# WHB139426/Grounded-Video-LLM

Measured on AMD Instinct MI355X. Metric: clips/sec + grounding tokens/sec, 96-frame Phi3.5-3.8B @1/2/4/8 MI355X, higher is better.
Workload: dtype bf16; 1 GPU; Phi-3.5-3.8B, 96 frames (12 segs x 8), 336^2 spatial + 224^2 temporal, prompts of 60..140 tokens (ragged), 12 greedy tokens, 8 clips per GPU per step (16 clips in flight per GPU: the vision encode of the next 8 overlaps the ragged prefill + batched greedy decode of the current 8; CLIP tower batched over the 96 key frames of a step); prefill_len_max=3559, distinct_clips_resident=16, parallelism=1 GPU

## Files before the change

### grounded-video-llm_amd/csrc/gvl_attn.hip

```cpp
#include "gvl_internal.h"
#include "gvl_attn_plan.h"
#include <cstdlib>

template <int D> struct KSwz;
template <> struct KSwz<64> {
  static __device__ __forceinline__ int phys(int row, int lc) { return lc ^ ((row >> 1) & 7); }
  static __device__ __forceinline__ int logical(int row, int pc) { return pc ^ ((row >> 1) & 7); }
};
template <> struct KSwz<96> {
  static __device__ __forceinline__ int phys(int row, int lc) { int p = lc + 3 * ((row >> 2) & 3); return p >= 12 ? p - 12 : p; }
  static __device__ __forceinline__ int logical(int row, int pc) { int l = pc - 3 * ((row >> 2) & 3); return l < 0 ? l + 12 : l; }
};
template <> struct KSwz<128> {
  static __device__ __forceinline__ int phys(int row, int lc) { return lc ^ (row & 15); }
  static __device__ __forceinline__ int logical(int row, int pc) { return pc ^ (row & 15); }
};

template <int D> struct VSwz;
template <> struct VSwz<64> { static __device__ __forceinline__ int phys(int row, int c) { return c ^ (((row >> 1) & 1) << 2); } };
template <> struct VSwz<96> { static __device__ __forceinline__ int phys(int, int c) { return c; } };
template <> struct VSwz<128> { static __device__ __forceinline__ int phys(int row, int c) { return c ^ ((row & 3) << 2); } };
typedef __attribute__((ext_vector_type(4))) short s16x4_t;
typedef __attribute__((ext_vector_type(8))) short s16x8_t;
__device__ __forceinline__ bf16x8_t lds_tr8(const char* p0, const char* p1) {
  typedef __attribute__((address_space(3))) s16x4_t* lp;
  const s16x4_t lo = __builtin_amdgcn_ds_read_tr16_b64_v4i16((lp)p0), hi = __builtin_amdgcn_ds_read_tr16_b64_v4i16((lp)p1);
  const s16x8_t v = {lo[0], lo[1], lo[2], lo[3], hi[0], hi[1], hi[2], hi[3]};
  return __builtin_bit_cast(bf16x8_t, v);
}
__device__ __forceinline__ void glds16s(const void* sbase, unsigned voff, unsigned lds_dst) {
  unsigned keep;
  asm volatile("s_mov_b32 %0, m0\n\ts_mov_b32 m0, %3\n\ts_nop 0\n\tglobal_load_lds_dwordx4 %1, %2\n\ts_mov_b32 m0, %0"
               : "=&s"(keep) : "v"(voff), "s"(sbase), "s"(lds_dst) : "memory");
}

__device__ __forceinline__ float vmax3(float a, float b, float c) {
  float r;
  asm("v_max3_f32 %0, %1, %2, %3" : "=v"(r) : "v"(a), "v"(b), "v"(c));
  return r;
}

__device__ __forceinline__ int kperm(int i) {
  const int c = i & 3, hh = (i >> 2) & 1, b = i >> 3;
  return (b >> 1) * 16 + 8 * hh + 4 * (b & 1) + c;
}

template <int D, int NWAVES, int NS, int ONES = 0, int VROW = 0, int VL = 0>
__global__ __launch_bounds__(NWAVES * 64) void attn_fwd_kernel(const AttnArgs a) {
  constexpr int NT = NWAVES * 64;
  constexpr int DK = D / 16;
  constexpr int DB = D / 32;
  constexpr int CPR = D / 8;
  constexpr int KCH = 64 * CPR;
  constexpr int NIK = KCH / NT;
  constexpr int TILE_BYTES = 64 * D * 2;
  constexpr int STAGE_BYTES = 2 * TILE_BYTES;
  static_assert(KCH % NT == 0, "tile/threads mismatch");

  extern __shared__ __attribute__((aligned(16))) char smem[];

  const int tid = threadIdx.x, lane = tid & 63;
  const int wave = __builtin_amdgcn_readfirstlane(tid >> 6);
  const int l31 = lane & 31, h = lane >> 5;
  int S_ = a.S;
  const bf16_t* Qp_ = a.Q; bf16_t* Op_ = a.O; const int* tbl_ = a.block_table;
  int nq = (a.S + NWAVES * 32 - 1) / (NWAVES * 32);
  const int rep = a.H / a.KV;
  if constexpr (VL) { nq = 0; for (int u = 0; u < a.vl_n; ++u) nq += (a.vl_rows[u + 1] - a.vl_rows[u] + NWAVES * 32 - 1) / (NWAVES * 32); }
  const int xcd = blockIdx.x & 7, j = blockIdx.x >> 3;
  const int qb_ = j % nq, t_ = j / nq, member = t_ % rep, grp = (t_ / rep) * 8 + xcd;
  int qb = a.causal ? nq - 1 - qb_ : qb_;
  if (grp >= a.KV * a.B) return;
  const int b = grp / a.KV, head = (grp - b * a.KV) * rep + member;
  if constexpr (VL) {
    int u = 0, nqu = (a.vl_rows[1] - a.vl_rows[0] + NWAVES * 32 - 1) / (NWAVES * 32);
    while (qb >= nqu && u + 1 < a.vl_n) { qb -= nqu; ++u; nqu = (a.vl_rows[u + 1] - a.vl_rows[u] + NWAVES * 32 - 1) / (NWAVES * 32); }
    const int r0 = a.vl_rows[u];
    S_ = a.vl_rows[u + 1] - r0;
    Qp_ = a.Q + (size_t)r0 * a.H * D;
    Op_ = a.O + (size_t)r0 * (size_t)(a.H * a.Dout);
    tbl_ = a.vl_tables[u];
  }
  const int hkv = head / (a.H / a.KV);
  const int q0 = qb * (NWAVES * 32);
  const int qw = q0 + wave * 32;
  const int Sk = a.Sk > 0 ? a.Sk : S_, qpos0 = a.qpos0;
  const int n_tiles_all = (Sk + 63) >> 6;
  int last_q = q0 + NWAVES * 32 - 1; if (last_q > S_ - 1) last_q = S_ - 1;
  const int n_tiles = a.causal ? ((qpos0 + last_q) >> 6) + 1 : n_tiles_all;

  unsigned koff[NIK], voff[NIK];
#pragma unroll
  for (int i = 0; i < NIK; ++i) {
    const int pos = i * NT + tid;
    const int kr = pos / CPR, kpc = pos - kr * CPR;
    koff[i] = VROW == 2 ? (unsigned)(kr * a.k_ld + KSwz<D>::logical(kr, kpc) * 8) * 2 : (unsigned)(kr * D + KSwz<D>::logical(kr, kpc) * 8) * 2;
    if constexpr (VROW) {
      const int vr = pos / CPR, lc = VSwz<D>::phys(vr, pos - vr * CPR);
      voff[i] = lc * 8 < a.Dout ? (unsigned)(vr * a.v_ld + lc * 8) * 2 : 0xffffffffu;
    } else {
      const int vr = pos >> 3, vpc = pos & 7;
      voff[i] = (unsigned)(vr * 64 + (vpc ^ ((vr >> 1) & 7)) * 8) * 2;
    }
  }
  const float sc = a.scale * 1.4426950408889634f;
  constexpr bool FOLD = VROW == 3;
  u32x4_t qf[DK];
  u32x4_t qraw[DK], qw_[VROW == 3 ? DK : 1];
  float q_rs = 1.f;
  {
    int qi = qw + l31; if (qi > S_ - 1) qi = S_ - 1;
    if constexpr (VROW == 3) {
      const bf16_t* qp = a.Qrows + ((size_t)b * S_ + qi) * a.q_ld + head * a.Dout + 8 * h;
      const bf16_t* wp = a.q_nw + head * a.Dout + 8 * h;
      q_rs = a.q_rs[(size_t)b * S_ + qi];
#pragma unroll
      for (int kk = 0; kk < DK; ++kk) {
        const bool real = kk * 16 + 8 * h < a.Dout;
        qraw[kk] = real ? *(const u32x4_t*)(qp + kk * 16) : u32x4_t{0u, 0u, 0u, 0u};
        qw_[kk] = real ? *(const u32x4_t*)(wp + kk * 16) : u32x4_t{0u, 0u, 0u, 0u};
      }
    } else {
      const bf16_t* qp = VROW == 2 ? a.Qrows + ((size_t)b * S_ + qi) * a.q_ld + head * D + 8 * h : Qp_ + (((size_t)b * a.H + head) * S_ + qi) * D + 8 * h;
#pragma unroll
      for (int kk = 0; kk < DK; ++kk) qraw[kk] = *(const u32x4_t*)(qp + kk * 16);
    }
  }

  int* pages_s = (int*)(smem + NS * STAGE_BYTES);
  for (int i = tid; i < n_tiles; i += NT) pages_s[i] = tbl_ ? tbl_[b * a.max_pages + i] : b * n_tiles_all + i;
  if constexpr (VROW) {
    const int npc = CPR - (a.Dout >> 3);
    for (int i = tid; i < NS * 64 * npc; i += NT) {
      const int slot = i / (64 * npc), r = (i / npc) & 63, lc = (a.Dout >> 3) + i % npc;
      u32x4_t v = {0u, 0u, 0u, 0u};
      if (ONES && lc * 8 == a.Dout) v[0] = 0x3F80u;
      *(u32x4_t*)(smem + slot * STAGE_BYTES + TILE_BYTES + (r * CPR + VSwz<D>::phys(r, lc)) * 16) = v;
    }
  }
  __syncthreads();
  const unsigned smem_base = __builtin_amdgcn_readfirstlane(lds_addr(smem));
  auto stage = [&](int buf, int t) {
    const int pg = __builtin_amdgcn_readfirstlane(pages_s[t]);
    const size_t pb = ((size_t)pg * a.KV + hkv) * (size_t)(64 * D);
    const bf16_t* kp = a.Kt + pb;
    const bf16_t* vp = a.Vt + pb;
    const unsigned base = smem_base + buf * STAGE_BYTES + wave * 1024;
    if constexpr (VROW) {
      const int rows_left = S_ - t * 64;
      if constexpr (VROW == 2) {
        const bf16_t* kr_ = a.Krows + ((size_t)b * S_ + (size_t)t * 64) * a.k_ld + hkv * D;
        if (rows_left >= 64) {
          if constexpr (NIK == 2 || NIK == 3) glds16xn<NIK>(kr_, koff, base, NT * 16);
          else {
#pragma unroll
            for (int i = 0; i < NIK; ++i) glds16s(kr_, koff[i], base + i * NT * 16);
          }
        } else {
#pragma unroll
          for (int i = 0; i < NIK; ++i) {
            const int r = (i * NT + tid) / CPR;
            glds16s(kr_, r >= rows_left ? koff[i] - (unsigned)((r - rows_left + 1) * a.k_ld * 2) : koff[i], base + i * NT * 16);
          }
        }
      } else {
        glds16xn<NIK>(kp, koff, base, NT * 16);
      }
      const bf16_t* vr_ = a.Vrows + ((size_t)b * S_ + (size_t)t * 64) * a.v_ld + hkv * a.Dout;
      if (rows_left >= 64) {
#pragma unroll
        for (int i = 0; i < NIK; ++i)
          if (voff[i] != 0xffffffffu) glds16s(vr_, voff[i], base + TILE_BYTES + i * NT * 16);
      } else {
#pragma unroll
        for (int i = 0; i < NIK; ++i) {
          const int r = (i * NT + tid) / CPR;
          const unsigned off = r >= rows_left ? voff[i] - (unsigned)((r - rows_left + 1) * a.v_ld * 2) : voff[i];
          if (voff[i] != 0xffffffffu) glds16s(vr_, off, base + TILE_BYTES + i * NT * 16);
        }
      }
    } else if constexpr (NIK == 2 || NIK == 3) {
      glds16xn<NIK>(kp, koff, base, NT * 16);
      glds16xn<NIK>(vp, voff, base + TILE_BYTES, NT * 16);
    } else {
#pragma unroll
      for (int i = 0; i < NIK; ++i) glds16((const char*)kp + koff[i], base + i * NT * 16);
#pragma unroll
      for (int i = 0; i < NIK; ++i) glds16((const char*)vp + voff[i], base + TILE_BYTES + i * NT * 16);
    }
  };

  f32x16_t o[DB];
#pragma unroll
  for (int i = 0; i < DB; ++i)
#pragma unroll
    for (int e = 0; e < 16; ++e) o[i][e] = 0.f;
  float m_run = -1e30f, l_run = 0.f;

  const int krow0 = kperm(l31);
  const int vswz = (l31 >> 1) & 7;
  const int my_q = qw + l31;
  unsigned vtr[DB];
  if constexpr (VROW) {
    const int i16 = lane & 15, g4 = (lane >> 4) & 1, r0 = 8 * h + (i16 >> 2);
#pragma unroll
    for (int db = 0; db < DB; ++db) vtr[db] = (unsigned)(r0 * (D * 2) + VSwz<D>::phys(r0, db * 4 + 2 * g4 + ((i16 & 3) >> 1)) * 16 + (i16 & 1) * 8);
  }

  stage(0, 0);
  if (NS == 3 && n_tiles > 1) stage(1, 1);
#pragma unroll
  for (int kk = 0; kk < DK; ++kk) {
    if constexpr (VROW == 3) {
      u32x4_t o;
#pragma unroll
      for (int e = 0; e < 4; ++e) o[e] = pack2bf(lo_bf(qw_[kk][e]) * rbf(lo_bf(qraw[kk][e]) * q_rs) * sc, hi_bf(qw_[kk][e]) * rbf(hi_bf(qraw[kk][e]) * q_rs) * sc);
      qf[kk] = o;
    } else {
      qf[kk] = qraw[kk];
    }
  }
#pragma unroll
  for (int kk = 0; kk < DK; ++kk) asm volatile("" ::"v"(qf[kk]));
  int cur = 0;
  int first_tile = 1;
  if constexpr (FOLD) m_run = 0.f;
  for (int t = 0; t < n_tiles; ++t) {
    if (NS == 3 && t + 1 < n_tiles) asm volatile("s_waitcnt vmcnt(%0)" ::"n"(2 * NIK) : "memory");
    else asm volatile("s_waitcnt vmcnt(0)" ::: "memory");
    __builtin_amdgcn_s_barrier();
    asm volatile("" ::: "memory");
#ifdef GVL_ATTN_LAB
    if (!(GVL_ATTN_LAB & 1))
#endif
    if (t + NS - 1 < n_tiles) { int nb = cur + NS - 1; if (nb >= NS) nb -= NS; stage(nb, t + NS - 1); }
    const int tb = cur;
    cur = cur + 1 == NS ? 0 : cur + 1;
    if (a.causal && t * 64 > qpos0 + qw + 31) continue;
    const char* kb_ = smem + tb * STAGE_BYTES;
    const char* vb_ = kb_ + TILE_BYTES;

    f32x16_t s[2];
#pragma unroll
    for (int kb = 0; kb < 2; ++kb)
#pragma unroll
      for (int e = 0; e < 16; ++e) s[kb][e] = 0.f;
#ifdef GVL_ATTN_LAB
    if (GVL_ATTN_LAB & 4) { s[0][0] = (float)t; s[1][3] = qf[0][0]; } else
#endif
#ifdef GVL_ATTN_PRIO
    if (GVL_ATTN_PRIO & 1) __builtin_amdgcn_s_setprio(1);
#endif
#pragma unroll
    for (int kk = 0; kk < DK; ++kk) {
#pragma unroll
      for (int kb = 0; kb < 2; ++kb) {
        const int row = kb * 32 + krow0;
        const bf16x8_t kf = *(const bf16x8_t*)(kb_ + row * (D * 2) + (KSwz<D>::phys(row, kk * 2 + h) << 4));
        s[kb] = __builtin_amdgcn_mfma_f32_32x32x16_bf16(kf, __builtin_bit_cast(bf16x8_t, qf[kk]), s[kb], 0, 0, 0);
      }
    }
#ifdef GVL_ATTN_PRIO
    if (GVL_ATTN_PRIO & 1) __builtin_amdgcn_s_setprio(0);
#endif
    const bool need_mask = (t == n_tiles_all - 1 && (Sk & 63)) || (a.causal && t * 64 + 63 > qpos0 + qw);
    if (need_mask) {
#pragma unroll
      for (int kb = 0; kb < 2; ++kb)
#pragma unroll
        for (int r = 0; r < 16; ++r) {
          const int key = t * 64 + kb * 32 + (r >> 3) * 16 + 8 * h + (r & 7);
          const bool dead = key >= Sk || (a.causal && key > qpos0 + my_q);
          s[kb][r] = dead ? -1e30f : s[kb][r];
        }
    }
    float mx;
    {
      asm volatile("s_nop 11" : "+v"(s[0]), "+v"(s[1]));
      float l1[11];
#pragma unroll
      for (int i = 0; i < 5; ++i) { l1[i] = vmax3(s[0][3 * i], s[0][3 * i + 1], s[0][3 * i + 2]); l1[5 + i] = vmax3(s[1][3 * i], s[1][3 * i + 1], s[1][3 * i + 2]); }
      l1[10] = vmax3(s[0][15], s[1][15], l1[0]);
      const float a2 = vmax3(l1[1], l1[2], l1[3]), b2 = vmax3(l1[4], l1[5], l1[6]), c2 = vmax3(l1[7], l1[8], l1[9]);
      mx = vmax3(vmax3(a2, b2, c2), l1[10], l1[10]);
    }
    {
      const auto sw = __builtin_amdgcn_permlane32_swap(__float_as_uint(mx), __float_as_uint(mx), false, false);
      mx = fmaxf(__uint_as_float(sw[0]), __uint_as_float(sw[1]));
    }
    float alpha = 1.f;
    if constexpr (FOLD) {
      if (first_tile || !__all(mx <= a.lazy)) {
        const float m_new = rbf(m_run + (first_tile ? mx : fmaxf(mx, 0.f)));
        const float de = m_new - m_run;
        alpha = first_tile ? 1.f : __builtin_amdgcn_exp2f(-de);
        m_run = m_new;
        first_tile = 0;
#pragma unroll
        for (int i = 0; i < DB; ++i)
#pragma unroll
          for (int e = 0; e < 16; ++e) o[i][e] *= alpha;
#pragma unroll
// ... 421 lines not shown
    if (t + 2 == n_tiles - 1) {
      body(IC<0>{}, IC<0>{}, t, sA, sB);
      body(IC<1>{}, IC<1>{}, t + 1, sB, sA);
    } else if (t + 1 == n_tiles - 1) {
      body(IC<0>{}, IC<1>{}, t, sA, sB);
#pragma unroll
      for (int kb = 0; kb < 2; ++kb) sA[kb] = sB[kb];
    }
    {
      const int tl = n_tiles - 1;
      asm volatile("s_waitcnt vmcnt(0)" ::: "memory");
      __builtin_amdgcn_s_barrier();
      asm volatile("" ::: "memory");
      const int vofs = partial ? VLAST : (tl & 1) * STAGE_BYTES + TILE_BYTES;
      const int nst = (tail_keys + 15) >> 4;
#pragma unroll
      for (int st = 0; st < 4; ++st) {
        if (st < nst) {
          const int kb = st >> 1, r0 = (st & 1) * 8;
          union { bf16x8_t v; unsigned u[4]; } pf;
#pragma unroll
          for (int e = 0; e < 4; ++e) pf.u[e] = pack2bf(__builtin_amdgcn_exp2f(sA[kb][r0 + 2 * e]), __builtin_amdgcn_exp2f(sA[kb][r0 + 2 * e + 1]));
#pragma unroll
          for (int db = 0; db < DB; ++db) o[db] = __builtin_amdgcn_mfma_f32_32x32x16_bf16(vfrag(vofs, st * 3 + db), pf.v, o[db], 0, 0, 0);
        }
      }
    }
  };
  auto row_sum = [&]() -> float {
    const int lr = Dout - 32 * (DB - 1);
    float mine = 0.f;
#pragma unroll
    for (int e = 0; e < 16; ++e) mine = (e == (lr >> 3) * 4 + (lr & 3)) ? o[DB - 1][e] : mine;
    const float other = __shfl_xor(mine, 32, 64);
    return h ? other : mine;
  };
  float l_tot = 0.f;
  bool redo = a.pipe == 2;
  if (!redo) {
    run(IC<0>{});
    l_tot = row_sum();
#ifndef GVL_PIPE_LAB
    redo = __syncthreads_or(!(l_tot > 0.f && l_tot < 1.2676506e30f)) != 0;
#endif
  }
  if (redo) {
#pragma unroll
    for (int i = 0; i < DB; ++i)
#pragma unroll
      for (int e = 0; e < 16; ++e) o[i][e] = 0.f;
    m_run = 0.f;
    qf[DK - 1][0] = h ? 0u : qf[DK - 1][0];
    run(IC<1>{});
    l_tot = row_sum();
  }
  const float inv = 1.f / l_tot;
  {
    const int qs = my_q < q_end ? my_q : q_end - 1;
    char* op = (char*)(a.O + ((size_t)b * S + qs) * (size_t)(a.H * Dout) + head * Dout);
#pragma unroll
    for (int db = 0; db < DB; ++db)
#pragma unroll
      for (int gp = 0; gp < 2; ++gp) {
        const int g0 = 2 * gp;
        unsigned ax = pack2bf(o[db][4 * g0] * inv, o[db][4 * g0 + 1] * inv), ay = pack2bf(o[db][4 * g0 + 2] * inv, o[db][4 * g0 + 3] * inv);
        unsigned bx = pack2bf(o[db][4 * g0 + 4] * inv, o[db][4 * g0 + 5] * inv), by = pack2bf(o[db][4 * g0 + 6] * inv, o[db][4 * g0 + 7] * inv);
        const auto rx = __builtin_amdgcn_permlane32_swap(ax, bx, false, false); ax = rx[0]; bx = rx[1];
        const auto ry = __builtin_amdgcn_permlane32_swap(ay, by, false, false); ay = ry[0]; by = ry[1];
        const int cg = db * 4 + g0 + h;
        if (my_q < q_end && cg * 8 < Dout) {
          const u32x4_t w = {ax, ay, bx, by};
          *(u32x4_t*)(op + cg * 16) = w;
        }
      }
  }
}
template <class Kern>
static int launch_planned(Kern kern, GvlDevOnce& once, const AttnArgs& a, const AttnLaunch& l, hipStream_t st) {
  if (gvl_set_max_lds(once, (const void*)kern, l.lds)) return -3;
  hipLaunchKernelGGL(kern, dim3(l.grid), dim3(l.block), l.lds, st, a);
  return hipGetLastError() == hipSuccess ? 0 : -3;
}
static int launch_attn(const AttnArgs& a, const AttnLaunch& l, hipStream_t st) {
  switch (attn_fwd_key(l.D, l.NWAVES, l.NS, l.ONES, l.VROW, l.VL)) {
#define GVL_CASE(D, NWAVES, NS, ONES, VROW, VL) \
    case attn_fwd_key(D, NWAVES, NS, ONES, VROW, VL): { static GvlDevOnce once; return launch_planned(attn_fwd_kernel<D, NWAVES, NS, ONES, VROW, VL>, once, a, l, st); }
    GVL_ATTN_FWD_LIST(GVL_CASE)
#undef GVL_CASE
    default: return -1;
  }
}
static int launch_attn_iv2_pipe(const AttnArgs& a, const AttnLaunch& l, hipStream_t st) {
  switch (l.NWAVES) {
#define GVL_CASE(NW) \
    case NW: { static GvlDevOnce once; return launch_planned(attn_iv2_pipe_kernel<NW>, once, a, l, st); }
    GVL_ATTN_IV2_PIPE_LIST(GVL_CASE)
#undef GVL_CASE
    default: return -1;
  }
}

double gvl_attn_flops(const AttnArgs& a) {
  const double Sk = a.Sk > 0 ? a.Sk : a.S;
  const double f = 4.0 * (double)a.S * Sk * a.Dout * a.H * a.B;
  return a.causal ? f * (a.qpos0 + 0.5 * a.S) / Sk : f;
}

int gvl_launch_attention(const AttnArgs& a_in, hipStream_t st) {
  static const AttnKnobs knobs = [] {
    AttnKnobs k = GVL_ATTN_KNOBS_DEFAULT;
    if (const char* e = gvl_lab_env("GVL_ATTN_LAZY")) k.lazy = (float)atof(e);
    k.no_ones = gvl_lab_env("GVL_ATTN_NO_ONES") != nullptr;
    return k;
  }();
  AttnArgs a = a_in;
  auto al16 = [](const void* p) { return ((uintptr_t)p & 15) == 0; };
  AttnGeometry g{};
  g.B = a.B; g.H = a.H; g.KV = a.KV; g.S = a.S; g.D = a.D; g.Dout = a.Dout; g.Sk = a.Sk; g.qpos0 = a.qpos0; g.causal = a.causal; g.ones_row = a.ones_row; g.k_ones = a.k_ones;
  g.ring = a.ring; g.pipe = a.pipe; g.pipe_rows = a.pipe_rows; g.v_ld = a.v_ld; g.q_ld = a.q_ld; g.k_ld = a.k_ld; g.max_pages = a.max_pages; g.vl_n = a.vl_n;
  for (int u = 0; u <= GVL_MAX_PREFILL_BATCH; ++u) g.vl_rows[u] = a.vl_rows[u];
  for (int u = 0; u < GVL_MAX_PREFILL_BATCH; ++u) g.vl_tables[u] = a.vl_tables[u] != nullptr;
  g.block_table = a.block_table; g.Vrows = a.Vrows; g.Qrows = a.Qrows; g.Krows = a.Krows; g.q_rs = a.q_rs; g.q_nw = a.q_nw;
  g.O16 = al16(a.O); g.Vrows16 = al16(a.Vrows); g.Qrows16 = al16(a.Qrows); g.Krows16 = al16(a.Krows); g.q_nw16 = al16(a.q_nw);
  AttnLaunch plan[GVL_ATTN_MAX_LAUNCHES];
  const int n = attn_plan(g, knobs, plan);
  if (n < 0) return -1;
  for (int i = 0; i < n; ++i) {
    const AttnLaunch& l = plan[i];
    a.lazy = l.lazy;
    if (l.family == GVL_ATTN_IV2_PIPE) { a.q_begin = l.q_begin; a.q_rows = l.q_rows; }
    const int rc = l.family == GVL_ATTN_IV2_PIPE ? launch_attn_iv2_pipe(a, l, st) : launch_attn(a, l, st);
    if (rc) return rc;
  }
  return 0;
}

template <int D, int G, int PH = 0>
__global__ __launch_bounds__(256, 2) void decode_attn_kernel(const DecodeAttnArgs a) {
  constexpr int CPR = D / 8;
  constexpr int NIT = D / 8;
  constexpr int QP = (64 % CPR == 0) ? 1 : 3;
  static_assert(D == 64 || D == 96 || D == 128, "head dim");
  __shared__ __attribute__((aligned(16))) float part_s[4][64 * (CPR + 1)];
  __shared__ __attribute__((aligned(16))) float p_s[4][64];
  __shared__ float red_s[G][4][D + 2];
  __shared__ int last_s;

  const int tid = threadIdx.x, lane = tid & 63, wave = tid >> 6;
  int split = blockIdx.y, bz = blockIdx.z;
  int hkv = blockIdx.x, head0 = hkv * G;
  if constexpr (PH == 2) { head0 = blockIdx.x; hkv = head0 / (a.H / a.KV); }
  if constexpr (PH == 1) {
    const int Gq = a.H / a.KV, units = a.KV * a.gsplit * a.batch;
    const int unit = ((int)blockIdx.y / Gq) * 8 + (int)blockIdx.x;
    if (unit >= units) return;
    hkv = unit % a.KV; split = (unit / a.KV) % a.gsplit; bz = unit / (a.KV * a.gsplit);
    head0 = hkv * Gq + (int)blockIdx.y % Gq;
  }
  const int* __restrict__ block_table = a.tables[bz];
  const bf16_t* qb = a.q + (size_t)bz * a.q_stride;
  float* part_b = a.part + (size_t)bz * a.H * a.nsplit * (D + 2);
  int* counters_b = a.counters + bz * a.H;
  const int pos = *a.pos_ptrs[bz] + 1;
  const int npages = (pos + 63) >> 6;
  int ns = (npages + 3) >> 2;
  ns = ns > a.nsplit ? a.nsplit : ns;
  const int cpb = a.cpb;
  const int c_begin = split * cpb;
  if (c_begin >= ns) return;
  const int c_end = c_begin + cpb < ns ? c_begin + cpb : ns;
  const int nblk = (ns + cpb - 1) / cpb;
  const int pps = (npages + ns - 1) / ns;

  u32x4_t qv[G][QP];
#pragma unroll
  for (int g = 0; g < G; ++g)
#pragma unroll
    for (int it = 0; it < QP; ++it) qv[g][it] = *(const u32x4_t*)(qb + (head0 + g) * D + ((it * 64 + lane) % CPR) * 8);

  const float sc = a.scale * 1.4426950408889634f;
  for (int chunk = c_begin; chunk < c_end; ++chunk) {
  const int p_begin = chunk * pps;
  int p_end = p_begin + pps; if (p_end > npages) p_end = npages;
  float m_run[G], l_run[G];
  float oacc[G][NIT];
#pragma unroll
  for (int g = 0; g < G; ++g) {
    m_run[g] = -1e30f; l_run[g] = 0.f;
#pragma unroll
    for (int i = 0; i < NIT; ++i) oacc[g][i] = 0.f;
  }

  for (int pg = p_begin + wave; pg < p_end; pg += 4) {
    const size_t pb = ((size_t)block_table[pg] * a.KV + hkv) * (size_t)(64 * D);
    const bf16_t* kp = a.Kt + pb;
    const bf16_t* vp = a.Vt + pb;
    u32x4_t kv[NIT], vv[NIT];
#pragma unroll
    for (int it = 0; it < NIT; ++it) kv[it] = PH == 1 ? *(const u32x4_t*)(kp + (it * 64 + lane) * 8) : __builtin_nontemporal_load((const u32x4_t*)(kp + (it * 64 + lane) * 8));
#pragma unroll
    for (int it = 0; it < NIT; ++it) vv[it] = PH == 1 ? *(const u32x4_t*)(vp + (it * 64 + lane) * 8) : __builtin_nontemporal_load((const u32x4_t*)(vp + (it * 64 + lane) * 8));
#pragma unroll
    for (int g = 0; g < G; ++g) {
#pragma unroll
      for (int it = 0; it < NIT; ++it) {
// ... 381 lines not shown
```

### grounded-video-llm_amd/csrc/gvl_attn_plan.h

```cpp
#pragma once
#include "gvl_limits.h"

enum AttnMode : int {
  GVL_ATTN_PAGED = 0,
  GVL_ATTN_V_ROWS,
  GVL_ATTN_QKV_ROWS,
  GVL_ATTN_QNORM_V_ROWS,
  GVL_ATTN_RAGGED,
};
enum AttnFamily : int { GVL_ATTN_FWD = 0, GVL_ATTN_IV2_PIPE };

#define GVL_ATTN_FWD_LIST(X)                                                                                     \
  X(64, 4, 2, 0, 0, 0) X(64, 4, 2, 0, 1, 0) X(64, 4, 2, 0, 2, 0)                                                 \
  X(96, 4, 2, 0, 0, 0) X(96, 4, 2, 1, 0, 0) X(96, 4, 3, 0, 0, 0) X(96, 4, 2, 0, 1, 0) X(96, 4, 2, 1, 1, 0)       \
  X(96, 4, 2, 0, 3, 0) X(96, 4, 2, 1, 3, 0)                                                                      \
  X(128, 4, 2, 0, 0, 0) X(128, 4, 3, 0, 0, 0)                                                                    \
  X(64, 4, 2, 0, 0, 1) X(96, 4, 2, 0, 0, 1) X(128, 4, 2, 0, 0, 1)
#define GVL_ATTN_IV2_PIPE_LIST(X) X(4) X(8)
constexpr int attn_fwd_key(int D, int NWAVES, int NS, int ONES, int VROW, int VL) { return ((((D * 16 + NWAVES) * 4 + NS) * 2 + ONES) * 4 + VROW) * 2 + VL; }

struct AttnGeometry {
  int B, H, KV, S, D, Dout, Sk, qpos0, causal, ones_row, k_ones, ring, pipe, pipe_rows, v_ld, q_ld, k_ld, max_pages;
  int vl_n, vl_rows[GVL_MAX_PREFILL_BATCH + 1];
  bool block_table, Vrows, Qrows, Krows, q_rs, q_nw, vl_tables[GVL_MAX_PREFILL_BATCH];
  bool O16, Vrows16, Qrows16, Krows16, q_nw16;
};
struct AttnKnobs {
  float lazy;
  bool no_ones;
};
constexpr AttnKnobs GVL_ATTN_KNOBS_DEFAULT = {8.f, false};
struct AttnLaunch {
  int mode;
  int family;
  int D, NWAVES, NS, ONES, VROW, VL;
  unsigned grid; int block, lds;
  int q_begin, q_rows;
  float lazy;
};
constexpr int GVL_ATTN_MAX_LAUNCHES = 2;

inline int attn_mode_of(const AttnGeometry& g) {
  return g.vl_n ? GVL_ATTN_RAGGED : (g.q_rs || g.q_nw) ? GVL_ATTN_QNORM_V_ROWS : (g.Krows || g.Qrows) ? GVL_ATTN_QKV_ROWS : g.Vrows ? GVL_ATTN_V_ROWS : GVL_ATTN_PAGED;
}
inline bool attn_pitch_ok(int ld, long long width, bool ptr16) { return ld >= width && (ld & 7) == 0 && ptr16; }
inline bool attn_tile_below_4g(int ld) { return (unsigned long long)64 * (unsigned long long)ld * 2 < 0xffffffffull; }
inline bool attn_common_ok(const AttnGeometry& g) {
  return g.B > 0 && g.H > 0 && g.KV > 0 && g.S > 0 && g.S <= 256 * 64 && g.Sk <= 256 * 64 && g.H % g.KV == 0 && g.Dout <= g.D && (g.Dout & 7) == 0 && g.O16;
}
inline bool attn_paged_ok(const AttnGeometry& g) {
  return g.Sk >= 0 && g.qpos0 >= 0 && (g.Sk > 0 ? g.Sk >= g.S + g.qpos0 && g.block_table : g.qpos0 == 0);
}
inline bool attn_v_rows_ok(const AttnGeometry& g) {
  return g.Vrows && !g.block_table && g.Sk == 0 && g.qpos0 == 0 && attn_pitch_ok(g.v_ld, (long long)g.KV * g.Dout, g.Vrows16) && attn_tile_below_4g(g.v_ld) && g.D != 128;
}
inline bool attn_qkv_rows_ok(const AttnGeometry& g) {
  return attn_v_rows_ok(g) && g.Qrows && g.Krows && g.D == 64 && g.Dout == g.D && attn_pitch_ok(g.k_ld, (long long)g.KV * g.D, g.Krows16) &&
         attn_pitch_ok(g.q_ld, (long long)g.H * g.D, g.Qrows16) && attn_tile_below_4g(g.k_ld);
}
inline bool attn_qnorm_v_rows_ok(const AttnGeometry& g) {
  return attn_v_rows_ok(g) && g.q_rs && g.q_nw && g.Qrows && !g.Krows && g.D == 96 && g.Dout == 88 && g.k_ones && attn_pitch_ok(g.q_ld, (long long)g.H * g.Dout, g.Qrows16 && g.q_nw16);
}
inline bool attn_ragged_ok(const AttnGeometry& g) {
  if (g.vl_n < 1 || g.vl_n > GVL_MAX_PREFILL_BATCH || g.B != 1 || !g.causal || g.Sk || g.qpos0 || g.Vrows || g.Qrows || g.Krows || g.q_rs || g.q_nw || g.block_table) return false;
  for (int u = 0; u < g.vl_n; ++u)
    if (!g.vl_tables[u] || g.vl_rows[u + 1] <= g.vl_rows[u] || g.vl_rows[u + 1] - g.vl_rows[u] > g.S) return false;
  return true;
}

inline int attn_plan(const AttnGeometry& g, const AttnKnobs& k, AttnLaunch out[GVL_ATTN_MAX_LAUNCHES]) {
  if (g.D != 64 && g.D != 96 && g.D != 128) return -1;
  if (!attn_common_ok(g)) return -1;
  const int mode = attn_mode_of(g);
  switch (mode) {
    case GVL_ATTN_PAGED: if (!attn_paged_ok(g)) return -1; break;
    case GVL_ATTN_V_ROWS: if (!attn_v_rows_ok(g)) return -1; break;
    case GVL_ATTN_QKV_ROWS: if (!attn_qkv_rows_ok(g)) return -1; break;
    case GVL_ATTN_QNORM_V_ROWS: if (!attn_qnorm_v_rows_ok(g)) return -1; break;
    default: if (!attn_ragged_ok(g)) return -1; break;
  }
  const float lazy = k.lazy >= 0.f && k.lazy <= 64.f ? k.lazy : GVL_ATTN_KNOBS_DEFAULT.lazy;
  const long long groups8 = (((long long)g.KV * g.B + 7) / 8) * 8;
  const int vrow = mode == GVL_ATTN_RAGGED ? 0 : mode, vl = mode == GVL_ATTN_RAGGED;
  const int lr = g.Dout - 64;
  const bool ones = g.D == 96 && !vl && g.ones_row && !k.no_ones && g.Dout < 96 && lr >= 0 && (lr & 7) < 4 && !g.causal;

  if (mode == GVL_ATTN_QNORM_V_ROWS && ones && g.pipe && g.H == g.KV) {
    const int lds = 2 * 2 * 64 * 96 * 2 + 64 * 96 * 2;
    const int rows8 = g.pipe_rows == 256 ? (g.S / 256) * 256 : 0;
    int n = 0;
    for (int nw = 8; nw >= 4; nw -= 4) {
      const int q_begin = nw == 8 ? 0 : rows8, q_rows = nw == 8 ? rows8 : g.S - rows8;
      if (q_rows <= 0) continue;
      const long long grid = groups8 * ((q_rows + 32 * nw - 1) / (32 * nw));
      if (grid > 0x7fffffffll) return -1;
      out[n++] = AttnLaunch{mode, GVL_ATTN_IV2_PIPE, 96, nw, 2, 1, 3, 0, (unsigned)grid, 64 * nw, lds, q_begin, q_rows, lazy};
    }
    return n;
  }
  const int ns = g.ring == 3 && mode == GVL_ATTN_PAGED && g.D != 64 && !ones ? 3 : 2;
  const int nwaves = 4, rows = 32 * nwaves;
  long long nq = (g.S + rows - 1) / rows;
  if (vl) { nq = 0; for (int u = 0; u < g.vl_n; ++u) nq += (g.vl_rows[u + 1] - g.vl_rows[u] + rows - 1) / rows; }
  const long long grid = groups8 * (g.H / g.KV) * nq;
  if (grid > 0x7fffffffll) return -1;
  out[0] = AttnLaunch{mode, GVL_ATTN_FWD, g.D, nwaves, ns, ones, vrow, vl, (unsigned)grid, 64 * nwaves, ns * 2 * 64 * g.D * 2 + 1024 ,
                      0, g.S, lazy};
  return 1;
}

enum DecodeAttnFamily : int { GVL_DECODE_ATTN_GQA = 0, GVL_DECODE_ATTN_HEAD };
#define GVL_DECODE_ATTN_GQA_LIST(X) \
  X(64, 4, 1) X(64, 16, 1) X(64, 4, 0) X(64, 16, 0) X(96, 4, 1) X(96, 16, 1) X(96, 4, 0) X(96, 16, 0) X(128, 4, 1) X(128, 16, 1) X(128, 4, 0) X(128, 16, 0)
#define GVL_DECODE_ATTN_HEAD_LIST(X) X(64, 0) X(64, 1) X(64, 2) X(96, 0) X(96, 1) X(96, 2) X(128, 0) X(128, 1) X(128, 2)
constexpr int decode_attn_key(int D, int a, int b) { return (D * 32 + a) * 4 + b; }

struct DecodeAttnGeometry { int H, KV, D, nsplit, batch, hpb, cpb, gsplit; };
struct DecodeAttnKnobs {
  bool no_gqa;
  bool gqa_valu;
  bool gqa_direct;
};
constexpr DecodeAttnKnobs GVL_DECODE_ATTN_KNOBS_DEFAULT = {false, false, false};
struct DecodeAttnLaunch {
  int batch, cpb, gsplit, hpb;
  int family;
  int D, t1, t2;
  unsigned grid_x, grid_y, grid_z;
};

inline int decode_attn_plan(const DecodeAttnGeometry& g, const DecodeAttnKnobs& k, DecodeAttnLaunch* out) {
  DecodeAttnLaunch l{};
  l.batch = g.batch <= 0 ? 1 : g.batch;
  if (l.batch > GVL_MAX_DECODE_BATCH) return -1;
  if (g.H <= 0 || g.KV <= 0 || g.H % g.KV) return -1;
  l.cpb = g.cpb < 1 ? 1 : g.cpb;
  if (g.nsplit < 1 || g.nsplit > 16) return -1;
  l.gsplit = g.gsplit <= 0 || g.gsplit > g.nsplit ? (g.nsplit + l.cpb - 1) / l.cpb : g.gsplit;
  if (g.D != 64 && g.D != 96 && g.D != 128) return -1;
  l.D = g.D; l.hpb = g.hpb;
  const int G = g.H / g.KV;
  long long gx, gy = 1, gz = 1;
  if (G > 1 && G <= 16 && !k.no_gqa && !k.gqa_valu) {
    if (l.hpb < 1 || l.hpb > G || G % l.hpb) l.hpb = G;
    l.family = GVL_DECODE_ATTN_GQA;
    l.t1 = l.hpb <= 4 ? 4 : 16;
    l.t2 = !(k.gqa_direct || (g.D & (g.D - 1)) != 0);
    gx = (long long)(g.H / l.hpb) * l.gsplit * l.batch;
  } else {
    l.family = GVL_DECODE_ATTN_HEAD;
    l.t1 = G == 1 ? 0 : k.no_gqa ? 2 : 1;
    if (l.t1 == 1) { gx = 8; gy = ((long long)g.KV * l.gsplit * l.batch + 7) / 8 * G; }
    else { gx = g.H; gy = l.gsplit; gz = l.batch; }
  }
  if (gx * gy * gz > 0x7fffffffll) return -1;
  l.grid_x = (unsigned)gx; l.grid_y = (unsigned)gy; l.grid_z = (unsigned)gz;
  *out = l;
  return 0;
}

struct DecodeAttnShape { int gsplit, cpb, hpb; };
inline DecodeAttnShape decode_attn_shape(const int* positions, int B, int H, int KV, int nsplit, int force_cpb, int force_hpb, bool capturing) {
  DecodeAttnShape s{nsplit, 1, 0};
  if (capturing) return s;
  if (force_cpb >= 1 && force_cpb <= 16) s.cpb = force_cpb;
  long splits = 0;
  s.gsplit = 1;
  for (int b = 0; b < B; ++b) {
    const int np = (positions[b] + 1 + 63) >> 6, n = (np + 3) >> 2;
    const int ns = n < 1 ? 1 : (n > nsplit ? nsplit : n), blocks = (ns + s.cpb - 1) / s.cpb;
    s.gsplit = blocks > s.gsplit ? blocks : s.gsplit;
    splits += blocks;
  }
  const int G = H / KV;
  if (G > 1) {
    s.hpb = G;
    while (s.hpb > 2 && s.hpb % 2 == 0 && (long)(H / s.hpb) * splits < 400) s.hpb >>= 1;
    if (s.hpb == 2 && (long)(H / 2) * splits < 200) s.hpb = 1;
    if (force_hpb >= 1 && G % force_hpb == 0) s.hpb = force_hpb;
  }
  return s;
}
```

### grounded-video-llm_amd/csrc/gvl_ctx.h

```cpp
#pragma once
#include "gvl_internal.h"
#include "gvl_seq_table.h"
#include "../../include/gvl.h"
#include <dlfcn.h>
#include <fcntl.h>
#include <sys/mman.h>
#include <sys/stat.h>
#include <unistd.h>
#include <algorithm>
#include <cmath>
#include <cstdio>
#include <cstring>
#include <memory>
#include <string>
#include <unordered_map>
#include <vector>

std::string& gvl_create_error();


struct Tensor { void* p = nullptr; int dtype = 0; int64_t numel = 0; std::vector<int64_t> shape; };

struct ClipLayerW { const float *ln1w, *ln1b, *ln2w, *ln2b, *qkvb, *outb, *fc1b, *fc2b; const bf16_t *qkvw, *outw, *fc1w, *fc2w; };
struct Iv2BlockW { const bf16_t *n1, *n2, *qkvw, *qn, *kn, *projw, *fc1w, *fc2w; const float *projb, *ls1, *ls2, *fc1b, *fc2b;
                   const bf16_t *qkvw_f = nullptr, *fc1w_f = nullptr; };
struct LlmLayerW { const bf16_t *ln1, *ln2, *qkvw, *ow, *guw, *downw;
                   const bf16_t *qkvw_f = nullptr, *guw_f = nullptr;
                   const bf16_t *qkvd_f = nullptr, *gud_f = nullptr;
                   const bf16_t *qkvd, *od, *gud, *downd;
                   const float *qkvs, *os, *gus, *downs; };

struct Seq : SeqCore {
  int* d_block_table = nullptr; int* d_pos = nullptr;
  bool table_dirty = false;
  int* d_tok = nullptr;
  int* d_out = nullptr;
  const int* h_out = nullptr;
  int* d_ngen = nullptr;
  unsigned rng_stream = 0;
  int* d_eos = nullptr; volatile int* h_eos = nullptr;
  float* d_lp = nullptr; int* d_top_ids = nullptr; float* d_top_lp = nullptr;
};

struct ProfRec { int cat; hipEvent_t e0, e1; double work; };

struct gvl_ctx : SeqTable<Seq> {
  static constexpr int kMaxSeqs = 256;
  static constexpr int kMaxRuleSets = 1024;
  gvl_ctx() : SeqTable<Seq>(kMaxSeqs, kMaxRuleSets) {}
  gvl_config cfg;
  std::string err;
  std::unordered_map<std::string, Tensor> w;
  bool finalized = false;
  int c_P = 0, c_S = 0, c_Kp = 0, c_Dr = 0, c_D = 0;
  int v_L = 0, v_TL = 0, v_S = 0, v_Kp = 0, v_Dr = 0, v_D = 0;
  int l_Dr = 0, l_D = 0, tok_per_seg = 0, img_tok = 0, seg_tok = 0;
  bool has_clip = false, has_iv2 = false, has_llm = false, has_proj = false;
  const bf16_t* c_patchw = nullptr; const float *c_cls = nullptr, *c_pos = nullptr, *c_prelnw = nullptr, *c_prelnb = nullptr;
  std::vector<ClipLayerW> cl;
  const bf16_t *v_patchw = nullptr, *v_cls = nullptr, *v_pos = nullptr; const float* v_patchb = nullptr;
  std::vector<Iv2BlockW> vb;
  const bf16_t *mm0w = nullptr, *mm1w = nullptr, *vp0w = nullptr, *vp1w = nullptr, *glb_gn = nullptr, *newline = nullptr;
  const float *mm0b = nullptr, *mm1b = nullptr, *vp0b = nullptr, *vp1b = nullptr, *sub_gn = nullptr;
  const bf16_t *l_embed = nullptr, *l_norm = nullptr, *l_headw = nullptr; const float* l_headb = nullptr;
  const float *cos_s = nullptr, *sin_s = nullptr, *cos_l = nullptr, *sin_l = nullptr;
  std::vector<LlmLayerW> ll;
  char* arena = nullptr; size_t arena_bytes = 0, arena_off = 0;
  char* arena_l = nullptr; size_t arena_l_bytes = 0, arena_l_off = 0;
  bf16_t *kpool = nullptr, *vpool = nullptr; size_t layer_stride = 0;
  int* d_seq_tables = nullptr; int* d_seq_pos = nullptr; int seq_table_cap = 0;
  bf16_t *d_x = nullptr, *d_qkv = nullptr, *d_q = nullptr, *d_attn = nullptr, *d_act = nullptr;
  bf16_t* d_xn = nullptr;
  int* d_seq_ngen = nullptr;
  bool decode_mfma = false;
  const bf16_t* l_headd = nullptr;
  const bf16_t* l_headd_f = nullptr;
  bf16_t* d_xt = nullptr;
  float* d_sqpart = nullptr;
  const float* l_heads = nullptr;
  int fp8 = 0;
  std::vector<void*> dw_allocs;
  std::vector<void*> pw_allocs;
  std::vector<void*> nf_allocs;
  const bf16_t *c_patchwt = nullptr, *v_patchwt = nullptr;
  float *d_logits = nullptr, *d_part = nullptr; int* d_counters = nullptr; int *d_seq_tok = nullptr, *d_seq_out = nullptr;
  int* h_seq_out = nullptr;
  int nsplit = 16, outlist_cap = 8192, ids_cap = 16384;
  void* pre_scratch = nullptr; size_t pre_scratch_bytes = 0;
  int kv_total_pages = 0;
  int* h_eos_flags = nullptr; int* d_eos_flags = nullptr; int watch_eos = -1;
  hipEvent_t step_ev[3] = {nullptr, nullptr, nullptr};
  struct { bool on = false; float inv_temp = 1.f, top_p = 0.f; int top_k = 0; unsigned long long seed = 0; unsigned next_stream = 0;
           float min_p = 0.f, typical_p = 0.f, eps = 0.f, eta = 0.f;
           bool warps() const { return on && (min_p > 0.f || (typical_p > 0.f && typical_p < 1.f) || eps > 0.f || eta > 0.f); } } sample;
  float* d_seq_lp = nullptr; int* d_seq_top_ids = nullptr; float* d_seq_top_lp = nullptr;
  struct { int decode_attn_cpb = 0, decode_attn_hpb = 0; bool decode_graph = true; int vision_in_place = 1, prefill_group = 4, attn_ring = 0, attn_pipe = 1, attn_pipe_rows = 128, patch_fused = 1, varlen_attn = 1, norm_fused = 1, last_layer_tail = 1; } dbg;
  void* comm = nullptr; int comm_rank = 0, comm_world = 1;
  bool prof = false; std::vector<ProfRec> recs;
  double prof_ms[GVL_PROF_NCAT] = {0}, prof_work[GVL_PROF_NCAT] = {0}; int64_t prof_n[GVL_PROF_NCAT] = {0};
};

inline int gvl_fail(gvl_ctx* c, int code, const std::string& msg) {
  if (c) c->err = msg; else gvl_create_error() = msg;
  return code;
}
inline int gvl_hipfail(gvl_ctx* c, hipError_t e, const char* what) { return gvl_fail(c, GVL_ERR_HIP, std::string(what) + ": " + hipGetErrorString(e)); }
#define HIPCHK(c, expr) do { hipError_t _e = (expr); if (_e != hipSuccess) return gvl_hipfail(c, _e, #expr); } while (0)
```

### grounded-video-llm_amd/csrc/gvl_elem.hip

```cpp
#include "gvl_internal.h"
#include <cstring>

#define CHECK_LAUNCH() (hipGetLastError() == hipSuccess ? 0 : -3)

template <int MAXV>
__global__ __launch_bounds__(256) void layernorm_f32_kernel(const float* __restrict__ x, const float* __restrict__ w,
                                                            const float* __restrict__ b, bf16_t* __restrict__ y, int rows, int cols, float eps) {
  const int row = blockIdx.x * 4 + (threadIdx.x >> 6), lane = threadIdx.x & 63;
  if (row >= rows) return;
  const float* xr = x + (size_t)row * cols;
  f32x4_t v[MAXV];
  float s = 0.f;
#pragma unroll
  for (int i = 0; i < MAXV; ++i) {
    const int c = (lane + 64 * i) * 4;
    if (c < cols) { v[i] = *(const f32x4_t*)(xr + c); s += v[i][0] + v[i][1] + v[i][2] + v[i][3]; }
  }
  const float mean = wave_sum(s) / cols;
  float q = 0.f;
#pragma unroll
  for (int i = 0; i < MAXV; ++i) {
    const int c = (lane + 64 * i) * 4;
    if (c < cols) {
#pragma unroll
// ... 315 lines not shown
  auto norm_chunk = [&](const u32x4_t& v, int c, float rs, const bf16_t* nw) -> u32x4_t {
    const u32x4_t w = *(const u32x4_t*)(nw + c * 8);
    u32x4_t o;
#pragma unroll
    for (int e = 0; e < 4; ++e) o[e] = pack2bf(lo_bf(w[e]) * rbf(lo_bf(v[e]) * rs), hi_bf(w[e]) * rbf(hi_bf(v[e]) * rs));
    return o;
  };
  bf16_t* Qb = a.Q + ((size_t)b * a.H * S_ + s_in) * a.D + (size_t)row0 * a.H * a.D;
  bf16_t* Kb = a.Kt + ((size_t)page * a.KV) * (64 * a.D) + (size_t)slot * a.D;
  if (in_regs) {
#pragma unroll
    for (int i = 0; i < RC; ++i) {
      const int c = lane + 64 * i;
      if (c < nq && !a.q_rs) { const int hd = c / cpr, dc = c - hd * cpr; *(u32x4_t*)(Qb + (size_t)hd * S_ * a.D + dc * 8) = norm_chunk(qreg[i], c, q_rs, a.qn); }
      if (c < nk) { const int hd = c / cpr, dc = c - hd * cpr; *(u32x4_t*)(Kb + (size_t)hd * (64 * a.D) + dc * 8) = norm_chunk(kreg[i], c, k_rs, a.kn); }
    }
  } else {
    if (!a.q_rs) for (int c = lt; c < nq; c += TEAM) {
      const int hd = c / cpr, dc = c - hd * cpr;
      *(u32x4_t*)(Qb + (size_t)hd * S_ * a.D + dc * 8) = xform(qr, c, q_rs, a.qn);
    }
    for (int c = lt; c < nk; c += TEAM) {
      const int hd = c / cpr, dc = c - hd * cpr;
      *(u32x4_t*)(Kb + (size_t)hd * (64 * a.D) + dc * 8) = xform(kr, c, k_rs, a.kn);
    }
  }
  if (cpd > cpr) {
    const int np = cpd - cpr;
    if (!a.q_rs) for (int c = lt; c < a.H * np; c += TEAM) { const int hd = c / np; *(u32x4_t*)(Qb + (size_t)hd * S_ * a.D + (cpr + c % np) * 8) = zero; }
    for (int c = lt; c < a.KV * np; c += TEAM) {
      const int hd = c / np;
      u32x4_t v = zero; if (a.k_ones && c % np == 0) v[0] = 0x3F80u;
      *(u32x4_t*)(Kb + (size_t)hd * (64 * a.D) + (cpr + c % np) * 8) = v;
    }
  }
  if (a.pos_ptr) {
    bf16_t* Vbase = a.Vt + ((size_t)page * a.KV) * (64 * a.D) + slot;
    for (int i = lt; i < a.KV * a.Dr; i += TEAM) {
      const int hd = i / a.Dr, d = i - hd * a.Dr;
      Vbase[(size_t)hd * (64 * a.D) + d * 64] = vr[i];
    }
  }
}

__global__ __launch_bounds__(256) void v_transpose_kernel(const QkvPostArgs a) {
  __shared__ __attribute__((aligned(16))) bf16_t tile[64][136];
  int t = blockIdx.x, S_ = a.S, row0 = 0;
  const int hkv = blockIdx.y, b = blockIdx.z;
  const int* table = a.block_table;
  if (a.vl_n) {
    int u = 0, t0 = 0;
    for (; u + 1 < a.vl_n; ++u) { const int nt = (a.vl_rows[u + 1] - a.vl_rows[u] + 63) >> 6; if (t < t0 + nt) break; t0 += nt; }
    t -= t0; row0 = a.vl_rows[u]; S_ = a.vl_rows[u + 1] - row0; table = a.vl_tables[u];
  }
  const int tid = threadIdx.x;
  const int s0 = a.pos0 + t * 64;
  const int n_tiles = (S_ + 63) >> 6;
  const int tile_idx = s0 >> 6;
  const int page = table ? table[b * a.max_pages + tile_idx] : b * n_tiles + tile_idx;
  const int voff = (a.H + a.KV) * a.Dr + hkv * a.Dr;
  const int cpr = a.Dr >> 3;
  for (int i = tid; i < 64 * cpr; i += 256) {
    const int r = i / cpr, c = i - r * cpr;
    const int s_in = t * 64 + r;
    u32x4_t v = {0u, 0u, 0u, 0u};
    if (s_in < S_) v = *(const u32x4_t*)(a.qkv + ((size_t)b * S_ + row0 + s_in) * a.ld + voff + c * 8);
    *(u32x4_t*)&tile[r][c * 8] = v;
  }
  __syncthreads();
  bf16_t* dst = a.Vt + ((size_t)page * a.KV + hkv) * (64 * a.D);
  for (int i = tid; i < a.D * 8; i += 256) {
    const int d = i >> 3, k8 = (i & 7) * 8;
    u32x4_t o = {0u, 0u, 0u, 0u};
    if (d < a.Dr) {
#pragma unroll
      for (int e = 0; e < 4; ++e) o[e] = (unsigned)tile[k8 + 2 * e][d] | ((unsigned)tile[k8 + 2 * e + 1][d] << 16);
    } else if (a.ones_row && d == a.Dr) {
      o = u32x4_t{0x3F803F80u, 0x3F803F80u, 0x3F803F80u, 0x3F803F80u};
    }
    *(u32x4_t*)(dst + d * 64 + k8) = o;
  }
}

int gvl_launch_qkv_post(const QkvPostArgs& a, hipStream_t st) {
  if ((a.Dr & 7) || (a.mode == 2 && (a.Dr & 15)) || (a.D & 7) || a.D < a.Dr || a.Dr > 128 || (a.ld & 7)) return -1;
  if (a.vl_n && (a.mode != 2 || a.B != 1 || a.pos0 != 0 || a.pos_ptr || a.vl_n > GVL_MAX_PREFILL_BATCH)) return -1;
  const int rows = a.vl_n ? a.vl_rows[a.vl_n] : a.B * a.S;
  if (a.q_rs && (a.mode != 1 || a.pos_ptr)) return -1;
  if (a.pos_ptr) {
    if (rows != 1 || a.mode != 2) return -1;
    hipLaunchKernelGGL(qkv_post_kernel<4>, dim3(1), dim3(256), 0, st, a);
  } else {
    hipLaunchKernelGGL(qkv_post_kernel<1>, dim3((rows + 3) / 4), dim3(256), 0, st, a);
  }
  if (!a.pos_ptr && a.Vt) {
    int n_tiles = (a.S + 63) >> 6;
    if (a.vl_n) { n_tiles = 0; for (int u = 0; u < a.vl_n; ++u) n_tiles += (a.vl_rows[u + 1] - a.vl_rows[u] + 63) >> 6; }
    hipLaunchKernelGGL(v_transpose_kernel, dim3(n_tiles, a.KV, a.B), dim3(256), 0, st, a);
  }
  return CHECK_LAUNCH();
}

__global__ __launch_bounds__(256) void hd_merge_kernel(const float* __restrict__ f, const float* __restrict__ sub_gn, bf16_t* __restrict__ out, int n, int C) {
  const int c4 = 4 * C, cv = c4 / 4;
  const long total = (long)n * 156 * cv;
  for (long idx = (long)blockIdx.x * blockDim.x + threadIdx.x; idx < total; idx += (long)gridDim.x * blockDim.x) {
    const int c = (int)(idx % cv) * 4;
    const long row = idx / cv;
    const int r = (int)(row % 156), img = (int)(row / 156);
    const int hh = r / 13, ww = r - hh * 13;
    f32x4_t v;
    if (ww == 12) v = *(const f32x4_t*)(sub_gn + c);
    else {
      const int chunk = c / C, cc = c - chunk * C, dy = chunk >> 1, dx = chunk & 1;
      v = *(const f32x4_t*)(f + ((size_t)img * 576 + (2 * hh + dy) * 24 + 2 * ww + dx) * C + cc);
    }
    u32x2_t o = {pack2bf(v[0], v[1]), pack2bf(v[2], v[3])};
    *(u32x2_t*)(out + row * c4 + c) = o;
  }
}
int gvl_launch_hd_merge(const float* f, const float* sub_gn, bf16_t* out, int n, int C, hipStream_t st) {
  if (C % 4) return -1;
  const long total = (long)n * 156 * C;
  int blocks = (int)((total + 255) / 256); if (blocks > 8192) blocks = 8192;
  hipLaunchKernelGGL(hd_merge_kernel, dim3(blocks), dim3(256), 0, st, f, sub_gn, out, n, C);
  return CHECK_LAUNCH();
}

__global__ __launch_bounds__(256) void pool_spatial_kernel(const float* __restrict__ f, bf16_t* __restrict__ out, int n, int C) {
  const int cv = C / 4;
  const long total = (long)n * 64 * cv;
  for (long idx = (long)blockIdx.x * blockDim.x + threadIdx.x; idx < total; idx += (long)gridDim.x * blockDim.x) {
    const int c = (int)(idx % cv) * 4;
    const long row = idx / cv;
    const int r = (int)(row % 64), img = (int)(row / 64);
    const int ph = r >> 3, pw = r & 7;
    f32x4_t acc = {0.f, 0.f, 0.f, 0.f};
    for (int dy = 0; dy < 3; ++dy)
      for (int dx = 0; dx < 3; ++dx) acc += *(const f32x4_t*)(f + ((size_t)img * 576 + (3 * ph + dy) * 24 + 3 * pw + dx) * C + c);
    u32x2_t o = {pack2bf(acc[0] / 9.f, acc[1] / 9.f), pack2bf(acc[2] / 9.f, acc[3] / 9.f)};
    *(u32x2_t*)(out + row * C + c) = o;
  }
}
int gvl_launch_pool_spatial(const float* f, bf16_t* out, int n, int C, hipStream_t st) {
  if (C % 4) return -1;
  const long total = (long)n * 64 * (C / 4);
  int blocks = (int)((total + 255) / 256); if (blocks > 8192) blocks = 8192;
  hipLaunchKernelGGL(pool_spatial_kernel, dim3(blocks), dim3(256), 0, st, f, out, n, C);
  return CHECK_LAUNCH();
}

__global__ __launch_bounds__(256) void pool_temporal_kernel(const bf16_t* __restrict__ f, bf16_t* __restrict__ out, int n, int T, int C) {
  const int cv = C / 8;
  const long total = (long)n * T * 16 * cv;
  for (long idx = (long)blockIdx.x * blockDim.x + threadIdx.x; idx < total; idx += (long)gridDim.x * blockDim.x) {
    const int c = (int)(idx % cv) * 8;
    const long row = idx / cv;
    const int r = (int)(row % 16), t = (int)((row / 16) % T), seg = (int)(row / (16L * T));
    const int ph = r >> 2, pw = r & 3;
    float acc[8] = {0, 0, 0, 0, 0, 0, 0, 0};
    for (int dy = 0; dy < 4; ++dy)
      for (int dx = 0; dx < 4; ++dx) {
        const u32x4_t v = *(const u32x4_t*)(f + ((size_t)seg * T * 256 + t * 256 + (4 * ph + dy) * 16 + 4 * pw + dx) * C + c);
#pragma unroll
        for (int e = 0; e < 4; ++e) { acc[2 * e] += lo_bf(v[e]); acc[2 * e + 1] += hi_bf(v[e]); }
      }
    u32x4_t o;
#pragma unroll
    for (int e = 0; e < 4; ++e) o[e] = pack2bf(acc[2 * e] * 0.0625f, acc[2 * e + 1] * 0.0625f);
    *(u32x4_t*)(out + row * C + c) = o;
  }
}
int gvl_launch_pool_temporal(const bf16_t* f, bf16_t* out, int n, int T, int C, hipStream_t st) {
  if (C % 8) return -1;
  const long total = (long)n * T * 16 * (C / 8);
  int blocks = (int)((total + 255) / 256); if (blocks > 8192) blocks = 8192;
  hipLaunchKernelGGL(pool_temporal_kernel, dim3(blocks), dim3(256), 0, st, f, out, n, T, C);
  return CHECK_LAUNCH();
}

__global__ void f32_to_bf16_kernel(const float* __restrict__ x, bf16_t* __restrict__ y, long n) {
  for (long i = (long)blockIdx.x * blockDim.x + threadIdx.x; i < n; i += (long)gridDim.x * blockDim.x) y[i] = f2bf(x[i]);
// ... 786 lines not shown
```

### grounded-video-llm_amd/csrc/gvl_internal.h

```cpp
#pragma once
#include <hip/hip_runtime.h>
#include <stdint.h>

typedef uint16_t bf16_t;

#include <cstdlib>
#ifdef GVL_LAB
inline const char* gvl_lab_env(const char* name) { return getenv(name); }
#else
inline const char* gvl_lab_env(const char*) { return nullptr; }
#endif

typedef __attribute__((ext_vector_type(8))) __bf16 bf16x8_t;
typedef __attribute__((ext_vector_type(16))) float f32x16_t;
typedef __attribute__((ext_vector_type(4))) float f32x4_t;
typedef __attribute__((ext_vector_type(4))) unsigned int u32x4_t;
typedef __attribute__((ext_vector_type(2))) unsigned int u32x2_t;

#define GVL_KV_PAGE 64
#include "gvl_limits.h"
constexpr int GVL_MAX_VALU_BATCH = 4;
constexpr int GVL_GEMM_ROT_LEN = 64;

#include <atomic>
// ... 58 lines not shown
  static_assert(N == 2 || N == 3, "2 or 3 pieces");
  unsigned keep, d;
  if constexpr (N == 3) {
    asm volatile(
        "s_mov_b32 %0, m0\n\t"
        "s_mov_b32 m0, %6\n\ts_nop 0\n\tglobal_load_lds_dwordx4 %2, %5\n\t"
        "s_add_u32 %1, %6, %7\n\ts_mov_b32 m0, %1\n\ts_nop 0\n\tglobal_load_lds_dwordx4 %3, %5\n\t"
        "s_add_u32 %1, %1, %7\n\ts_mov_b32 m0, %1\n\ts_nop 0\n\tglobal_load_lds_dwordx4 %4, %5\n\t"
        "s_mov_b32 m0, %0"
        : "=&s"(keep), "=&s"(d)
        : "v"(v[0]), "v"(v[1]), "v"(v[N - 1]), "s"(sbase), "s"(lds_dst0), "s"(lds_step)
        : "memory", "scc");
  } else {
    asm volatile(
        "s_mov_b32 %0, m0\n\t"
        "s_mov_b32 m0, %5\n\ts_nop 0\n\tglobal_load_lds_dwordx4 %2, %4\n\t"
        "s_add_u32 %1, %5, %6\n\ts_mov_b32 m0, %1\n\ts_nop 0\n\tglobal_load_lds_dwordx4 %3, %4\n\t"
        "s_mov_b32 m0, %0"
        : "=&s"(keep), "=&s"(d)
        : "v"(v[0]), "v"(v[1]), "s"(sbase), "s"(lds_dst0), "s"(lds_step)
        : "memory", "scc");
  }
}
__device__ __forceinline__ unsigned lds_addr(const void* p) {
  return (unsigned)(unsigned long)(__attribute__((address_space(3))) const void*)p;
}

enum { GVL_ACT_NONE = 0, GVL_ACT_QUICK_GELU = 1, GVL_ACT_GELU = 2, GVL_ACT_SILU_MUL = 3 };

struct GemmArgs {
  const bf16_t* A;  int lda;
  const bf16_t* W;  int ldw;
  void* C;          int ldc;
  int M, N, K;
  const float* bias;
  const float* gamma;
  const void* resid; int ldr;
  int act;
  int out_f32;
  int round_pre_resid;
  int grp_rows, grp_stride, row_off;
  int tile_cfg;
  int band;
  unsigned char rot[64];
  int narrow;
  int m_begin;
  const float* rowscale;
  float* rowsq; int rowsq_ld;
  const float* act_table;
  unsigned long long* dbg;
};
constexpr int GVL_GEMM_BAND = 4;
int gvl_launch_gemm(const GemmArgs& a, hipStream_t st);
int gvl_device_cus();
int gvl_launch_gemm_a4(const GemmArgs& a, int epi, int var, hipStream_t st);
int gvl_launch_gemm_a4p(const GemmArgs& a, int epi, hipStream_t st);
void gvl_gemm_set_a4(int v);
void gvl_gemm_set_narrow(int v);
void gvl_gemm_set_band(int v);
double gvl_gemm_flops(const GemmArgs& a);
template <class Launch, class Report>
inline int gvl_gemm_probe_launch(GemmArgs a, size_t n, hipStream_t st, Launch&& launch, Report&& report) {
  if (hipMalloc((void**)&a.dbg, n * 8) != hipSuccess) return -3;
  hipMemsetAsync(a.dbg, 0, n * 8, st);
  launch(a);
  std::vector<unsigned long long> hbuf(n);
  hipStreamSynchronize(st);
  hipMemcpy(hbuf.data(), a.dbg, n * 8, hipMemcpyDeviceToHost);
  hipFree(a.dbg);
  report(hbuf);
  return hipGetLastError() == hipSuccess ? 0 : -3;
}

struct AttnArgs {
  const bf16_t* Q;
  const bf16_t* Kt;
  const bf16_t* Vt;
  const bf16_t* Vrows;
  int v_ld;
  const bf16_t* Qrows; const bf16_t* Krows;
  int q_ld, k_ld;
  int k_ones;
  const float* q_rs; const bf16_t* q_nw;
  bf16_t* O;
  const int* block_table;
  int max_pages;
  int B, H, KV, S, D, Dout;
  int Sk, qpos0;
  float scale;
  int causal;
  int ones_row;
  int ring;
  int pipe;
  int pipe_rows;
  int q_begin, q_rows;
  float lazy;
  int vl_n;
  int vl_rows[GVL_MAX_PREFILL_BATCH + 1];
  const int* vl_tables[GVL_MAX_PREFILL_BATCH];
};
int gvl_launch_attention(const AttnArgs& a, hipStream_t st);
double gvl_attn_flops(const AttnArgs& a);

struct DecodeAttnArgs {
  const bf16_t* q;
  const bf16_t* Kt; const bf16_t* Vt;
  const int* tables[GVL_MAX_DECODE_BATCH];
  const int* pos_ptrs[GVL_MAX_DECODE_BATCH];
  float* part;
  int* counters;
  bf16_t* out;
  int H, KV, D, Dout, nsplit, batch, q_stride, out_stride, out_tiled;
  float scale;
  int hpb;
  int cpb;
  int gsplit;
};
int gvl_launch_decode_attention(const DecodeAttnArgs& a, hipStream_t st);

int gvl_launch_layernorm_f32(const float* x, const float* w, const float* b, bf16_t* y, int rows, int cols, float eps, hipStream_t st);
int gvl_launch_rmsnorm_bf16(const bf16_t* x, const bf16_t* w, bf16_t* y, int rows, int cols, float eps, hipStream_t st);
int gvl_launch_copy_bytes(const void* src, void* dst, size_t bytes, hipStream_t st);
int gvl_launch_fold_gamma(const bf16_t* W, const bf16_t* gamma, bf16_t* Wo, long rows, int cols, hipStream_t st);
int gvl_launch_rowsq_finish(const float* sq, int ld, int b0, int nblk, float* rs, int rows, int cols, float eps, hipStream_t st);
int gvl_launch_patchify(const float* px, bf16_t* A, int n_img, int T, int image, int patch, int Kp, hipStream_t st);
int gvl_launch_clip_embed_ln(const bf16_t* patch, const float* cls, const float* pos, const float* lnw, const float* lnb,
                             float* x, int n_img, int P, int C, float eps, hipStream_t st);
int gvl_launch_iv2_embed(const bf16_t* patch, const bf16_t* cls, const bf16_t* pos, bf16_t* x, int B, int TL, int C, hipStream_t st);
struct PatchEmbedArgs {
  const float* px;
  const bf16_t* Wt;
  int n_img, T, image, patch, C;
  int M;
  int S;
  int mode;
  const float* bias;
  const float *cls_f32, *pos_f32, *lnw, *lnb; float eps; float* x_f32;
  const bf16_t *cls_bf, *pos_bf; bf16_t* x_bf;
};
int gvl_retile_patch_weight(const bf16_t* W, bf16_t* Wt, int C, int Kp, int p, hipStream_t st);
int gvl_launch_patch_embed(const PatchEmbedArgs& a, hipStream_t st);
struct QkvPostArgs {
  const bf16_t* qkv; int ld;
  bf16_t* Q; bf16_t* Kt; bf16_t* Vt;
  const int* block_table; int max_pages;
  int B, S, H, KV, Dr, D;
  int mode;
  const bf16_t* qn; const bf16_t* kn; float eps;
  const float* cos; const float* sin; int pos0;
  const int* pos_ptr;
  const float* cos_l; const float* sin_l; int rope_switch;
  int ones_row;
  int k_ones;
  float* q_rs;
  int vl_n;
  int vl_rows[GVL_MAX_PREFILL_BATCH + 1];
  const int* vl_tables[GVL_MAX_PREFILL_BATCH];
};
int gvl_launch_qkv_post(const QkvPostArgs& a, hipStream_t st);
int gvl_launch_hd_merge(const float* f, const float* sub_gn, bf16_t* out, int n, int C, hipStream_t st);
int gvl_launch_pool_spatial(const float* f, bf16_t* out, int n, int C, hipStream_t st);
int gvl_launch_pool_temporal(const bf16_t* f, bf16_t* out, int n, int T, int C, hipStream_t st);
int gvl_launch_f32_to_bf16(const float* x, bf16_t* y, int64_t n, hipStream_t st);
int gvl_launch_bcast_row(const bf16_t* row, bf16_t* dst, int n, int stride_rows, int row_off, int cols, hipStream_t st);
int gvl_launch_gather_rows(const bf16_t* table, const int* ids, bf16_t* dst, int n, int cols, hipStream_t st);
int gvl_launch_strip_cls(const void* x, void* y, int n, int S, int C, int elem_bytes, hipStream_t st);
struct GemvArgs {
  const bf16_t* W; int N, K;
  const bf16_t* x;
  const bf16_t* norm_w; float eps;
  const float* bias;
  const bf16_t* resid;
  int act;
  bf16_t* out_bf16;
  float* out_f32;
  int batch, x_stride, out_stride;
  int rope_on; const float *cos_s, *sin_s, *cos_l, *sin_l; int rope_switch;
  const int* pos_ptrs[GVL_MAX_DECODE_BATCH]; const int* tables[GVL_MAX_DECODE_BATCH];
  bf16_t *Q, *Kt, *Vt; int H, KV, Dr, D; int q_stride;
  int variant;
  int w_fp8; const float* wscale;
  int out_tiled;
  const float* sq_in; int sq_n;
  float* sq_out; bf16_t* out_tiled2;
};
__host__ __device__ __forceinline__ size_t gvl_xt_index(int j, int k) { return ((size_t)(k >> 5) * 64 + (size_t)(((k >> 3) & 3) * 16 + j)) * 8 + (k & 7); }
int gvl_retile_decode_weight(const bf16_t* W, bf16_t* Wt, int N, int K, int Dr, int n_qk_heads, hipStream_t st);
int gvl_fp8_quantise_decode_weight(bf16_t* W, unsigned char* Wt8, float* scale, int N, int K, int Dr, int n_qk_heads, hipStream_t st);
int gvl_mxfp4_quantise_decode_weight(bf16_t* W, unsigned char* Wt4, unsigned* scale, int N, int K, int Dr, int n_qk_heads, hipStream_t st);
int gvl_launch_rows_to_tiled(const bf16_t* x, bf16_t* xt, int batch, int cols, int stride, hipStream_t st);
int gvl_launch_gemv(const GemvArgs& a, hipStream_t st);
int gvl_launch_dgemm(const GemvArgs& a, hipStream_t st);
struct IntList { int v[256]; int n; };
int gvl_launch_gather_rows_host_ids(const bf16_t* table, const int* host_ids, int n, bf16_t* dst, int cols, hipStream_t st);
int gvl_launch_ce_rows(const bf16_t* logits, int ld, const int* targets, float* nll, int n, int V, hipStream_t st);
struct ArgmaxArgs { const float* logits; int n, batch; int* tok_ptrs[GVL_MAX_DECODE_BATCH]; int* out_lists[GVL_MAX_DECODE_BATCH];
                    int* ngen_ptrs[GVL_MAX_DECODE_BATCH]; int* pos_ptrs[GVL_MAX_DECODE_BATCH];
                    int eos_id; int* eos_flags[GVL_MAX_DECODE_BATCH];
                    float inv_temp, top_p; int top_k; unsigned seed_lo, seed_hi; unsigned stream[GVL_MAX_DECODE_BATCH];
                    const int* step_override;
                    int top_n[GVL_MAX_DECODE_BATCH]; float* lp_lists[GVL_MAX_DECODE_BATCH]; int* top_ids[GVL_MAX_DECODE_BATCH]; float* top_lp[GVL_MAX_DECODE_BATCH]; };
constexpr int GVL_MAX_TOP_LOGPROBS = 8;
int gvl_launch_argmax(const ArgmaxArgs& a, hipStream_t st);
int gvl_launch_sample(const ArgmaxArgs& a, hipStream_t st);
struct SelRow { int on; float inv_temp; int top_k; float top_p, min_p, typical_p, eps, eta; unsigned seed_lo, seed_hi, stream; };
struct SelRowsArgs { ArgmaxArgs am; SelRow row[GVL_MAX_DECODE_BATCH]; unsigned char* kept; };
int gvl_launch_select_rows(const SelRowsArgs& a, hipStream_t st);
constexpr int GVL_LOGITS_HIST_CAP = 8192;
constexpr int GVL_RULES_MAX_IDS = 1 << 18;
constexpr int GVL_RULES_MAX_SEQS = 1024;
constexpr int GVL_RULES_MAX_SEQ_LEN = 16;
struct TokenRulesDev { int n_suppress, off_suppress, n_begin, off_begin, begin_at, n_force, off_force, force_at, n_multi;
                       int n_tgt[2], off_tgt[2], off_ent[2], off_pre[2]; };
struct LogitsProcArgs { float* logits; int n, ld, batch, cap; const int* hist[GVL_MAX_DECODE_BATCH]; const int* len_ptrs[GVL_MAX_DECODE_BATCH];
                        float penalty[GVL_MAX_DECODE_BATCH]; int ngram[GVL_MAX_DECODE_BATCH], min_new[GVL_MAX_DECODE_BATCH], eos[GVL_MAX_DECODE_BATCH];
                        const TokenRulesDev* rules[GVL_MAX_DECODE_BATCH]; };
int gvl_launch_logits_process(const LogitsProcArgs& a, hipStream_t st);
struct TokPtrs { const int* p[GVL_MAX_DECODE_BATCH]; int n; };
int gvl_launch_gather_tok_rows(const bf16_t* table, const TokPtrs& toks, bf16_t* dst, int cols, hipStream_t st);
int gvl_launch_embed_norm(const bf16_t* table, const TokPtrs& toks, bf16_t* x, bf16_t* xn, const bf16_t* w, int cols, float eps, hipStream_t st);
int gvl_launch_norm_tiled(bf16_t* x, bf16_t* xn, const bf16_t* w, int batch, int cols, float eps, hipStream_t st);
struct IntPtrs { int* p[GVL_MAX_DECODE_BATCH]; int n; };
int gvl_launch_inc_many(const IntPtrs& ptrs, hipStream_t st);
int gvl_launch_inc(int* p, hipStream_t st);
int gvl_launch_kv_page_copy(bf16_t* kpool, bf16_t* vpool, size_t layer_stride, size_t page_elems, int layers, int src_page, int dst_page, hipStream_t st);
int gvl_launch_set_int(int* p, int v, hipStream_t st);

int gvl_launch_preprocess(const unsigned char* frames, int n, int H, int W, int layout, int size, const float* mean, const float* stdv, float* out,
                          void** scratch, size_t* scratch_bytes, hipStream_t st);
```

### grounded-video-llm_amd/csrc/gvl_llm.hip

```cpp
#include "gvl_model.h"
#include "gvl_attn_plan.h"

namespace gvlm {

size_t prefill_bytes(const gvl_ctx* c, int S) {
  const gvl_config& f = c->cfg;
  const size_t qkvw = (size_t)(f.heads + 2 * f.kv_heads) * c->l_Dr;
  size_t b = 0;
  b += 2 * al256((size_t)S * f.hidden * 2) + al256((size_t)S * qkvw * 2) + al256((size_t)S * f.heads * c->l_Dr * 2);
  b += al256((size_t)S * f.inter * 2) + al256((size_t)f.heads * S * c->l_D * 2);
  b += al256((size_t)kLossChunk * f.vocab * 2) + al256((size_t)kLossChunk * f.hidden * 2) + 3 * al256((size_t)S * 4);
  b += al256((size_t)S * ((f.hidden + 63) / 64) * 4) + al256((size_t)S * 4);
  b += (size_t)GVL_MAX_PREFILL_BATCH * (al256((size_t)f.hidden * 2) * 2 + al256((size_t)f.inter * 2) + al256(((f.hidden + 63) / 64) * 4) + 256) + 1024;
  return b + 4096;
}

__global__ void fill_ints_kernel(int* dst, const IntList l) { for (int i = threadIdx.x; i < l.n; i += blockDim.x) dst[i] = l.v[i]; }

int upload_table(gvl_ctx* ctx, Seq& s, hipStream_t st) {
  if (!s.table_dirty) return 0;
  const int np = (int)s.pages.size();
  for (int p0 = 0; p0 < np; p0 += 256) {
    IntList l; l.n = np - p0 < 256 ? np - p0 : 256;
    for (int i = 0; i < l.n; ++i) l.v[i] = s.pages[p0 + i];
// ... 13 lines not shown
    lp.cap = ctx->outlist_cap < GVL_LOGITS_HIST_CAP ? ctx->outlist_cap : GVL_LOGITS_HIST_CAP;
    for (int b = 0; b < am.batch; ++b) {
      const LogitsProc& q = sqs[b]->sel.proc;
      lp.hist[b] = sqs[b]->d_out; lp.len_ptrs[b] = sqs[b]->d_ngen;
      lp.penalty[b] = q.penalty; lp.ngram[b] = q.ngram; lp.min_new[b] = q.eos >= 0 ? q.min_new : 0; lp.eos[b] = q.eos;
      lp.rules[b] = sqs[b]->sel.rules >= 0 ? (const TokenRulesDev*)ctx->rule_sets[sqs[b]->sel.rules].d : nullptr;
    }
    const int rc = gvl_launch_logits_process(lp, st);
    if (rc) return rc;
  }
  for (int b = 0; b < am.batch; ++b) {
    const Seq& q = *sqs[b];
    if (q.sel.top_n < 0 || !q.d_lp) continue;
    am.top_n[b] = q.sel.top_n; am.lp_lists[b] = q.d_lp;
    if (q.sel.top_n > 0) { am.top_ids[b] = q.d_top_ids; am.top_lp[b] = q.d_top_lp; }
  }
  bool per_row = ctx->sample.warps();
  for (int b = 0; b < am.batch; ++b) per_row = per_row || sqs[b]->sel.own_sampling;
  if (per_row) {
    SelRowsArgs sa; memset(&sa, 0, sizeof(sa)); sa.am = am;
    for (int b = 0; b < am.batch; ++b) {
      SelRow& r = sa.row[b];
      if (sqs[b]->sel.own_sampling) {
        const Sampling& q = sqs[b]->sel.sampling;
        r.on = q.on; r.inv_temp = q.inv_temp; r.top_k = q.top_k; r.top_p = q.top_p; r.min_p = q.min_p; r.typical_p = q.typical_p; r.eps = q.eps; r.eta = q.eta;
        r.seed_lo = (unsigned)q.seed; r.seed_hi = (unsigned)(q.seed >> 32); r.stream = q.stream;
      } else {
        const auto& q = ctx->sample;
        r.on = q.on; r.inv_temp = q.inv_temp; r.top_k = q.top_k; r.top_p = q.top_p; r.min_p = q.min_p; r.typical_p = q.typical_p; r.eps = q.eps; r.eta = q.eta;
        r.seed_lo = (unsigned)q.seed; r.seed_hi = (unsigned)(q.seed >> 32); r.stream = sqs[b]->rng_stream;
      }
    }
    return gvl_launch_select_rows(sa, st);
  }
  if (!ctx->sample.on) return gvl_launch_argmax(am, st);
  am.inv_temp = ctx->sample.inv_temp; am.top_p = ctx->sample.top_p; am.top_k = ctx->sample.top_k;
  am.seed_lo = (unsigned)ctx->sample.seed; am.seed_hi = (unsigned)(ctx->sample.seed >> 32);
  for (int b = 0; b < am.batch; ++b) am.stream[b] = sqs[b]->rng_stream;
  return gvl_launch_sample(am, st);
}

int llm_prefill(gvl_ctx* ctx, Seq* const* sqs, int nb, const bf16_t* const* embeds, const int* lens, hipStream_t st, const LossReq* loss, int pos0) {
  const gvl_config& f = ctx->cfg;
  const int Hd = f.hidden, H = f.heads, KV = f.kv_heads, Dr = ctx->l_Dr, D = ctx->l_D, I = f.inter;
  const int qkvw = (H + 2 * KV) * Dr;
  if (nb < 1 || nb > GVL_MAX_PREFILL_BATCH) return fail(ctx, GVL_ERR_ARG, "llm_prefill: batch must be 1 .. 8 sequences");
  if (pos0 != 0 && (nb != 1 || (pos0 & 63) || loss)) return fail(ctx, GVL_ERR_ARG, "llm_prefill: extend takes one sequence whose cached prefix is whole pages");
  for (int b = 0; b < nb; ++b) { const int rc = upload_table(ctx, *sqs[b], st); if (rc) return rc; }
  int off[GVL_MAX_PREFILL_BATCH + 1]; off[0] = 0;
  bool uniform = true;
  for (int b = 0; b < nb; ++b) { off[b + 1] = off[b] + lens[b]; uniform = uniform && lens[b] == lens[0]; }
  const int M = off[nb], S0 = lens[0], P0 = (S0 + 63) / 64;
  if (nb > 1 && uniform && nb * P0 > (int)(sizeof(IntList::v) / sizeof(int))) uniform = false;
  ArenaScope arena_scope(ctx->arena_l_off);
  LALLOC(x, bf16_t, (size_t)M * Hd); LALLOC(h, bf16_t, (size_t)M * Hd); LALLOC(qkv, bf16_t, (size_t)M * qkvw);
  LALLOC(att, bf16_t, (size_t)M * H * Dr); LALLOC(act, bf16_t, (size_t)M * I); LALLOC(Q, bf16_t, (size_t)M * H * D);
  const int* table = sqs[0]->d_block_table;
  int table_stride = sqs[0]->n_pages;
  if (nb > 1 && uniform) {
    LALLOC(tb, int, (size_t)nb * P0);
    IntList l; l.n = nb * P0;
    for (int b = 0; b < nb; ++b) for (int p = 0; p < P0; ++p) l.v[b * P0 + p] = sqs[b]->pages[p];
    hipLaunchKernelGGL(fill_ints_kernel, dim3(1), dim3(256), 0, st, tb, l);
    table = tb; table_stride = P0;
  }
  for (int b = 0; b < nb; ++b) RUN(GVL_PROF_OTHER, 0, gvl_launch_copy_bytes(embeds[b], x + (size_t)off[b] * Hd, (size_t)lens[b] * Hd * 2, st));
  const int NBLK = Hd / 64;
  const bool nf = ctx->dbg.norm_fused && Hd % 64 == 0 && ((f.heads + 2 * f.kv_heads) * ctx->l_Dr) % 16 == 0 && (2 * f.inter) % 16 == 0 && !ctx->ll.empty() && ctx->ll[0].qkvw_f;
  LALLOC(sq, float, (size_t)M * (nf ? NBLK : 1)); LALLOC(nrs, float, (size_t)M);
  const bf16_t* tail_rows = nullptr;
  const int n_att = (nb == 1 || uniform) ? 1 : nb;
  for (int l = 0; l < f.layers; ++l) {
    const LlmLayerW& w = ctx->ll[l];
    bf16_t* Kt = ctx->kpool + (size_t)l * ctx->layer_stride; bf16_t* Vt = ctx->vpool + (size_t)l * ctx->layer_stride;
    if (nf && l > 0) {
      RUN(GVL_PROF_OTHER, 0, gvl_launch_rowsq_finish(sq, NBLK, 0, NBLK, nrs, M, Hd, f.rms_eps, st));
      GemmArgs g = gemm(x, Hd, w.qkvw_f, qkv, qkvw, M, qkvw, Hd); g.rowscale = nrs; RUN(GVL_PROF_GEMM, gvl_gemm_flops(g), gvl_launch_gemm(g, st));
    } else {
      RUN(GVL_PROF_OTHER, 0, gvl_launch_rmsnorm_bf16(x, w.ln1, h, M, Hd, f.rms_eps, st));
      GemmArgs g = gemm(h, Hd, w.qkvw, qkv, qkvw, M, qkvw, Hd); RUN(GVL_PROF_GEMM, gvl_gemm_flops(g), gvl_launch_gemm(g, st));
    }
    const bool vl_attn = n_att > 1 && ctx->dbg.varlen_attn && pos0 == 0;
    bool vl_post = vl_attn && ctx->dbg.varlen_attn == 1;
    if (vl_post && f.rope_orig_max_pos > 0 && ctx->cos_l) {
      const bool l0 = lens[0] > f.rope_orig_max_pos;
      for (int u = 1; u < nb; ++u) vl_post = vl_post && (lens[u] > f.rope_orig_max_pos) == l0;
    }
    if (vl_post) {
      const bool use_long = f.rope_orig_max_pos > 0 && lens[0] > f.rope_orig_max_pos && ctx->cos_l;
      QkvPostArgs q; memset(&q, 0, sizeof(q)); q.qkv = qkv; q.ld = qkvw; q.Q = Q; q.Kt = Kt; q.Vt = Vt; q.B = 1; q.H = H; q.KV = KV; q.Dr = Dr; q.D = D; q.mode = 2;
      q.cos = use_long ? ctx->cos_l : ctx->cos_s; q.sin = use_long ? ctx->sin_l : ctx->sin_s; q.vl_n = nb;
      for (int u = 0; u < nb; ++u) { q.vl_rows[u] = off[u]; q.vl_tables[u] = sqs[u]->d_block_table; q.S = lens[u] > q.S ? lens[u] : q.S; }
      q.vl_rows[nb] = off[nb];
      RUN(GVL_PROF_OTHER, 0, gvl_launch_qkv_post(q, st));
    }
    for (int u = 0; u < n_att && !vl_post; ++u) {
      const int S = lens[u], B = n_att == 1 ? nb : 1;
      const int* tbl = n_att == 1 ? table : sqs[u]->d_block_table;
      const int tstride = n_att == 1 ? table_stride : sqs[u]->n_pages;
      const bool use_long = f.rope_orig_max_pos > 0 && pos0 + S > f.rope_orig_max_pos && ctx->cos_l;
      bf16_t* Qu = Q + (size_t)off[u] * H * D;
      { QkvPostArgs q; memset(&q, 0, sizeof(q)); q.qkv = qkv + (size_t)off[u] * qkvw; q.ld = qkvw; q.Q = Qu; q.Kt = Kt; q.Vt = Vt; q.block_table = tbl; q.max_pages = tstride;
        q.B = B; q.S = S; q.H = H; q.KV = KV; q.Dr = Dr; q.D = D; q.mode = 2; q.cos = use_long ? ctx->cos_l : ctx->cos_s; q.sin = use_long ? ctx->sin_l : ctx->sin_s; q.pos0 = pos0;
        RUN(GVL_PROF_OTHER, 0, gvl_launch_qkv_post(q, st)); }
      if (vl_attn) continue;
      { AttnArgs a; memset(&a, 0, sizeof(a)); a.Q = Qu; a.Kt = Kt; a.Vt = Vt; a.O = att + (size_t)off[u] * H * Dr; a.block_table = tbl; a.max_pages = tstride;
        a.B = B; a.H = H; a.KV = KV; a.S = S; a.D = D; a.Dout = Dr; a.scale = 1.0f / sqrtf((float)Dr); a.causal = 1;
        if (pos0) { a.Sk = pos0 + S; a.qpos0 = pos0; }
        a.ring = ctx->dbg.attn_ring;
        RUN(GVL_PROF_ATTN, gvl_attn_flops(a), gvl_launch_attention(a, st)); }
    }
    if (vl_attn) {
      AttnArgs a; memset(&a, 0, sizeof(a)); a.Q = Q; a.Kt = Kt; a.Vt = Vt; a.O = att; a.B = 1; a.H = H; a.KV = KV; a.D = D; a.Dout = Dr;
      a.scale = 1.0f / sqrtf((float)Dr); a.causal = 1; a.vl_n = nb;
      double fl = 0;
      for (int u = 0; u < nb; ++u) { a.vl_rows[u] = off[u]; a.vl_tables[u] = sqs[u]->d_block_table; a.S = lens[u] > a.S ? lens[u] : a.S;
        AttnArgs one = a; one.S = lens[u]; one.vl_n = 0; fl += gvl_attn_flops(one); }
      a.vl_rows[nb] = off[nb]; a.max_pages = 0;
      RUN(GVL_PROF_ATTN, fl, gvl_launch_attention(a, st));
    }
    { GemmArgs g = gemm(att, H * Dr, w.ow, x, Hd, M, Hd, H * Dr); g.resid = x; g.ldr = Hd; if (nf) { g.rowsq = sq; g.rowsq_ld = NBLK; }
      RUN(GVL_PROF_GEMM, gvl_gemm_flops(g), gvl_launch_gemm(g, st)); }
    if (l == f.layers - 1 && !loss && ctx->dbg.last_layer_tail && (!nf || NBLK % 4 == 0)) {
      int ids[GVL_MAX_PREFILL_BATCH];
      for (int b = 0; b < nb; ++b) ids[b] = off[b + 1] - 1;
      LALLOC(xl, bf16_t, (size_t)nb * Hd); LALLOC(actl, bf16_t, (size_t)nb * I);
      RUN(GVL_PROF_OTHER, 0, gvl_launch_gather_rows_host_ids(x, ids, nb, xl, Hd, st));
      if (nf) {
        LALLOC(sql, float, (size_t)nb * NBLK); LALLOC(rsl, float, nb);
        RUN(GVL_PROF_OTHER, 0, gvl_launch_gather_rows_host_ids((const bf16_t*)sq, ids, nb, (bf16_t*)sql, NBLK * 2, st));
        RUN(GVL_PROF_OTHER, 0, gvl_launch_rowsq_finish(sql, NBLK, 0, NBLK, rsl, nb, Hd, f.rms_eps, st));
        GemmArgs g = gemm(xl, Hd, w.guw_f, actl, I, nb, 2 * I, Hd); g.act = GVL_ACT_SILU_MUL; g.rowscale = rsl; RUN(GVL_PROF_GEMM, gvl_gemm_flops(g), gvl_launch_gemm(g, st));
      } else {
        LALLOC(hl, bf16_t, (size_t)nb * Hd);
        RUN(GVL_PROF_OTHER, 0, gvl_launch_rmsnorm_bf16(xl, w.ln2, hl, nb, Hd, f.rms_eps, st));
        GemmArgs g = gemm(hl, Hd, w.guw, actl, I, nb, 2 * I, Hd); g.act = GVL_ACT_SILU_MUL; RUN(GVL_PROF_GEMM, gvl_gemm_flops(g), gvl_launch_gemm(g, st));
      }
      { GemmArgs g = gemm(actl, I, w.downw, xl, Hd, nb, Hd, I); g.resid = xl; g.ldr = Hd; RUN(GVL_PROF_GEMM, gvl_gemm_flops(g), gvl_launch_gemm(g, st)); }
      tail_rows = xl;
      continue;
    }
    if (nf) {
      RUN(GVL_PROF_OTHER, 0, gvl_launch_rowsq_finish(sq, NBLK, 0, NBLK, nrs, M, Hd, f.rms_eps, st));
      GemmArgs g = gemm(x, Hd, w.guw_f, act, I, M, 2 * I, Hd); g.act = GVL_ACT_SILU_MUL; g.rowscale = nrs; RUN(GVL_PROF_GEMM, gvl_gemm_flops(g), gvl_launch_gemm(g, st));
    } else {
      RUN(GVL_PROF_OTHER, 0, gvl_launch_rmsnorm_bf16(x, w.ln2, h, M, Hd, f.rms_eps, st));
      GemmArgs g = gemm(h, Hd, w.guw, act, I, M, 2 * I, Hd); g.act = GVL_ACT_SILU_MUL; RUN(GVL_PROF_GEMM, gvl_gemm_flops(g), gvl_launch_gemm(g, st));
    }
    { GemmArgs g = gemm(act, I, w.downw, x, Hd, M, Hd, I); g.resid = x; g.ldr = Hd; if (nf && l + 1 < f.layers) { g.rowsq = sq; g.rowsq_ld = NBLK; }
      RUN(GVL_PROF_GEMM, gvl_gemm_flops(g), gvl_launch_gemm(g, st)); }
  }
  if (loss && loss->n > 0) {
    if (nb != 1) return fail(ctx, GVL_ERR_ARG, "llm_prefill: loss tail takes one sequence");
    LALLOC(d_rows, int, loss->n); LALLOC(d_tgt, int, loss->n); LALLOC(d_nll, float, loss->n);
    LALLOC(hs, bf16_t, (size_t)kLossChunk * Hd); LALLOC(lg, bf16_t, (size_t)kLossChunk * f.vocab);
    HIPCHK(ctx, hipMemcpyAsync(d_rows, loss->h_rows, (size_t)loss->n * 4, hipMemcpyHostToDevice, st));
    HIPCHK(ctx, hipMemcpyAsync(d_tgt, loss->h_targets, (size_t)loss->n * 4, hipMemcpyHostToDevice, st));
    for (int r0 = 0; r0 < loss->n; r0 += kLossChunk) {
      const int n = loss->n - r0 < kLossChunk ? loss->n - r0 : kLossChunk;
      RUN(GVL_PROF_OTHER, 0, gvl_launch_gather_rows(x, d_rows + r0, hs, n, Hd, st));
      RUN(GVL_PROF_OTHER, 0, gvl_launch_rmsnorm_bf16(hs, ctx->l_norm, h, n, Hd, f.rms_eps, st));
      { GemmArgs g = gemm(h, Hd, ctx->l_headw, lg, f.vocab, n, f.vocab, Hd); g.bias = ctx->l_headb; RUN(GVL_PROF_GEMM, gvl_gemm_flops(g), gvl_launch_gemm(g, st)); }
      RUN(GVL_PROF_OTHER, 0, gvl_launch_ce_rows(lg, f.vocab, d_tgt + r0, d_nll + r0, n, f.vocab, st));
    }
    HIPCHK(ctx, hipMemcpyAsync(loss->h_nll, d_nll, (size_t)loss->n * 4, hipMemcpyDeviceToHost, st));
  }
  const bf16_t* last = x + (size_t)(S0 - 1) * Hd;
  int last_stride = S0 * Hd;
  if (tail_rows) { last = tail_rows; last_stride = Hd; }
  else if (n_att > 1) {
    for (int b = 0; b < nb; ++b) RUN(GVL_PROF_OTHER, 0, gvl_launch_copy_bytes(x + (size_t)(off[b + 1] - 1) * Hd, h + (size_t)b * Hd, (size_t)Hd * 2, st));
    last = h; last_stride = Hd;
  }
  for (int b0 = 0; b0 < nb;) {
    const int nbc = nb - b0 >= 4 ? 4 : (nb - b0 >= 2 ? 2 : 1);
    GemvArgs g; memset(&g, 0, sizeof(g)); g.W = ctx->l_headw; g.N = f.vocab; g.K = Hd; g.x = last + (size_t)b0 * last_stride; g.norm_w = ctx->l_norm; g.eps = f.rms_eps;
    g.batch = nbc; g.x_stride = last_stride; g.out_stride = f.vocab;
    g.bias = ctx->l_headb; g.out_f32 = ctx->d_logits + (size_t)b0 * f.vocab; RUN(GVL_PROF_GEMV, 2.0 * f.vocab * Hd, gvl_launch_gemv(g, st));
    b0 += nbc;
  }
  for (int b = 0; b < nb; ++b) RUN(GVL_PROF_OTHER, 0, gvl_launch_set_int(sqs[b]->d_ngen, 0, st));
  { ArgmaxArgs am; memset(&am, 0, sizeof(am)); am.logits = ctx->d_logits; am.n = f.vocab; am.batch = nb;
    for (int b = 0; b < nb; ++b) { am.tok_ptrs[b] = sqs[b]->d_tok; am.out_lists[b] = sqs[b]->d_out; am.ngen_ptrs[b] = sqs[b]->d_ngen; }
    for (int b = 0; b < nb; ++b) sqs[b]->rng_stream = ctx->sample.next_stream++;
    RUN(GVL_PROF_OTHER, 0, pick_tokens(ctx, am, sqs, st)); }
  for (int b = 0; b < nb; ++b) {
    RUN(GVL_PROF_OTHER, 0, gvl_launch_set_int(sqs[b]->d_pos, pos0 + lens[b], st));
    sqs[b]->pos = pos0 + lens[b]; sqs[b]->n_gen = 1;
  }
  return 0;
}

int decode_step(gvl_ctx* ctx, Seq* const* sqs, int B, hipStream_t st) {
  const gvl_config& f = ctx->cfg;
  const int Hd = f.hidden, H = f.heads, KV = f.kv_heads, Dr = ctx->l_Dr, D = ctx->l_D, I = f.inter;
  const int qkvw = (H + 2 * KV) * Dr;
  const bool mfma = ctx->decode_mfma;
// ... 155 lines not shown
```

### grounded-video-llm_amd/csrc/gvl_model.hip

```cpp
#include "gvl_model.h"

std::string& gvl_create_error() { static std::string e; return e; }

using namespace gvlm;

namespace {

const Tensor* find(gvl_ctx* c, const std::string& n) { auto it = c->w.find(n); return it == c->w.end() ? nullptr : &it->second; }

template <typename T>
int need(gvl_ctx* c, const std::string& name, int dtype, int64_t numel, const T** out, bool optional = false) {
  const Tensor* t = find(c, name);
  if (!t) { if (optional) { *out = nullptr; return 0; } return fail(c, GVL_ERR_STATE, "missing weight: " + name); }
  if (t->dtype != dtype) return fail(c, GVL_ERR_ARG, "wrong dtype for weight: " + name);
  if (t->numel != numel) return fail(c, GVL_ERR_ARG, "wrong size for weight: " + name + " (have " + std::to_string(t->numel) + ", want " + std::to_string(numel) + ")");
  *out = (const T*)t->p;
  return 0;
}
#define NEED(name, dt, n, outp) do { int _r = need(ctx, name, dt, (int64_t)(n), outp); if (_r) return _r; } while (0)

int alloc_kv_pool(gvl_ctx* ctx, int pages) {
  const gvl_config& f = ctx->cfg;
  ctx->layer_stride = (size_t)pages * f.kv_heads * 64 * ctx->l_D;
  const size_t pool = ctx->layer_stride * f.layers * 2;
// ... 435 lines not shown
  const int id = ctx->open(max_tokens, src_seq, n_tokens);
  if (id < 0) return seq_fail(ctx, "gvl_seq_fork", id);
  bind_slot(ctx, ctx->seqs[id], id);
  *dst_seq = id;
  return 0;
}

int gvl_prefill(gvl_ctx* ctx, int seq_id, const uint16_t* embeds, int S, float* last_logits, void* stream) {
  REQUIRE_READY(ctx->has_llm, "gvl_prefill");
  if (!ctx->lookup(seq_id)) return seq_fail(ctx, "gvl_prefill", SEQ_BAD);
  Seq& sq = ctx->seqs[seq_id];
  if (!embeds || S <= 0 || S > sq.max_tokens || S > ctx->cfg.max_prefill) return fail(ctx, GVL_ERR_ARG, "gvl_prefill: bad length");
  if (sq.pos != 0) return fail(ctx, GVL_ERR_STATE, "gvl_prefill: sequence already holds tokens");
  hipStream_t st = (hipStream_t)stream;
  Seq* one[1] = {&sq}; const bf16_t* e1[1] = {embeds};
  int rc = llm_prefill(ctx, one, 1, e1, &S, st);
  if (rc) return rc;
  if (last_logits) HIPCHK(ctx, hipMemcpyAsync(last_logits, ctx->d_logits, (size_t)ctx->cfg.vocab * 4, hipMemcpyDeviceToDevice, st));
  return 0;
}

int gvl_seq_clone(gvl_ctx* ctx, int src_seq, int max_tokens, int* dst_seq, void* stream) {
  REQUIRE_READY(ctx->has_llm, "gvl_seq_clone");
  if (!dst_seq || !ctx->lookup(src_seq)) return fail(ctx, GVL_ERR_ARG, "gvl_seq_clone: bad arguments");
  const int pos = ctx->seqs[src_seq].pos;
  if (pos <= 0 || max_tokens <= pos || max_tokens > ctx->cfg.max_seq) return fail(ctx, GVL_ERR_ARG, "gvl_seq_clone: the source must hold tokens and max_tokens must exceed them (and fit cfg.max_seq)");
  const int id = ctx->open(max_tokens, src_seq, pos);
  if (id < 0) return seq_fail(ctx, "gvl_seq_clone", id);
  Seq& s = ctx->seqs[id];
  bind_slot(ctx, s, id);
  hipStream_t st = (hipStream_t)stream;
  { const int rc = upload_table(ctx, s, st); if (rc) return rc; }
  if (pos & 63)
    RUN(GVL_PROF_OTHER, 0, gvl_launch_kv_page_copy(ctx->kpool, ctx->vpool, ctx->layer_stride, (size_t)ctx->cfg.kv_heads * 64 * ctx->l_D, ctx->cfg.layers,
                                                   ctx->seqs[src_seq].pages[pos >> 6], s.pages[pos >> 6], st));
  RUN(GVL_PROF_OTHER, 0, gvl_launch_set_int(s.d_pos, pos, st));
  RUN(GVL_PROF_OTHER, 0, gvl_launch_set_int(s.d_ngen, 0, st));
  s.n_gen = 0;
  *dst_seq = id;
  return 0;
}

int gvl_prefill_extend(gvl_ctx* ctx, int seq_id, const uint16_t* embeds, int n_new, float* last_logits, void* stream) {
  REQUIRE_READY(ctx->has_llm, "gvl_prefill_extend");
  if (!ctx->lookup(seq_id)) return seq_fail(ctx, "gvl_prefill_extend", SEQ_BAD);
  Seq& sq = ctx->seqs[seq_id];
  if (sq.pos <= 0 || (sq.pos & 63)) return fail(ctx, GVL_ERR_STATE, "gvl_prefill_extend: the sequence must hold a prefix of whole pages (gvl_seq_fork)");
  if (!embeds || n_new <= 0 || sq.pos + n_new > sq.max_tokens || n_new > ctx->cfg.max_prefill) return fail(ctx, GVL_ERR_ARG, "gvl_prefill_extend: bad length");
  hipStream_t st = (hipStream_t)stream;
  Seq* one[1] = {&sq}; const bf16_t* e1[1] = {embeds};
  int rc = llm_prefill(ctx, one, 1, e1, &n_new, st, nullptr, sq.pos);
  if (rc) return rc;
  if (last_logits) HIPCHK(ctx, hipMemcpyAsync(last_logits, ctx->d_logits, (size_t)ctx->cfg.vocab * 4, hipMemcpyDeviceToDevice, st));
  return 0;
}

int gvl_forward_loss(gvl_ctx* ctx, int seq_id, const uint16_t* embeds, int S, const int64_t* labels, double* nll_sum, int* n_valid, void* stream) {
  REQUIRE_READY(ctx->has_llm, "gvl_forward_loss");
  if (!ctx->lookup(seq_id)) return seq_fail(ctx, "gvl_forward_loss", SEQ_BAD);
  Seq& sq = ctx->seqs[seq_id];
  if (!embeds || !labels || !nll_sum || !n_valid || S <= 0 || S > sq.max_tokens || S > ctx->cfg.max_prefill) return fail(ctx, GVL_ERR_ARG, "gvl_forward_loss: bad arguments / length");
  if (sq.pos != 0) return fail(ctx, GVL_ERR_STATE, "gvl_forward_loss: sequence already holds tokens");
  std::vector<int> rows, tgt;
  for (int t = 0; t + 1 < S; ++t) {
    const int64_t y = labels[t + 1];
    if (y == -100) continue;
    if (y < 0 || y >= ctx->cfg.vocab) return fail(ctx, GVL_ERR_ARG, "gvl_forward_loss: label out of range");
    rows.push_back(t); tgt.push_back((int)y);
  }
  std::vector<float> nll(rows.size());
  LossReq lr{(int)rows.size(), rows.data(), tgt.data(), nll.data()};
  hipStream_t st = (hipStream_t)stream;
  Seq* one[1] = {&sq}; const bf16_t* e1[1] = {embeds};
  const int rc = llm_prefill(ctx, one, 1, e1, &S, st, &lr);
  if (rc) return rc;
  HIPCHK(ctx, hipStreamSynchronize(st));
  double acc = 0;
  for (float v : nll) acc += (double)v;
  *nll_sum = acc; *n_valid = (int)rows.size();
  return 0;
}

int gvl_prefill_varlen(gvl_ctx* ctx, const int* seq_ids, int n_seqs, const uint16_t* const* embeds, const int* seq_lens, void* stream) {
  REQUIRE_READY(ctx->has_llm, "gvl_prefill_varlen");
  if (!seq_ids || !embeds || !seq_lens || n_seqs <= 0 || n_seqs > gvl_ctx::kMaxSeqs) return fail(ctx, GVL_ERR_ARG, "gvl_prefill_varlen: bad arguments");
  for (int i = 0; i < n_seqs; ++i) {
    const int id = seq_ids[i];
    if (!ctx->lookup(id) || !embeds[i]) return fail(ctx, GVL_ERR_ARG, "gvl_prefill_varlen: bad seq / embeds");
    if (seq_lens[i] <= 0 || seq_lens[i] > ctx->seqs[id].max_tokens) return fail(ctx, GVL_ERR_ARG, "gvl_prefill_varlen: bad length");
    if (seq_lens[i] > ctx->cfg.max_prefill) return fail(ctx, GVL_ERR_ARG, "gvl_prefill_varlen: seq_len exceeds cfg.max_prefill");
    if (ctx->seqs[id].pos != 0) return fail(ctx, GVL_ERR_STATE, "gvl_prefill_varlen: sequence already holds tokens");
    if (ctx->repeats(seq_ids, i)) return seq_fail(ctx, "gvl_prefill_varlen", SEQ_DUPLICATE);
  }
  hipStream_t st = (hipStream_t)stream;
  int i = 0;
  while (i < n_seqs) {
    const int left = n_seqs - i;
    int B = left >= ctx->dbg.prefill_group ? ctx->dbg.prefill_group : left;
    for (;;) {
      long rows = 0; for (int b = 0; b < B; ++b) rows += seq_lens[i + b];
      if (B == 1 || rows <= ctx->cfg.max_prefill) break;
      --B;
    }
    Seq* sqs[GVL_MAX_PREFILL_BATCH]; const bf16_t* es[GVL_MAX_PREFILL_BATCH];
    for (int b = 0; b < B; ++b) { sqs[b] = &ctx->seqs[seq_ids[i + b]]; es[b] = embeds[i + b]; }
    const int rc = llm_prefill(ctx, sqs, B, es, seq_lens + i, st);
    if (rc) return rc;
    i += B;
  }
  return 0;
}

int gvl_prefill_batch(gvl_ctx* ctx, const int* seq_ids, int n_seqs, const uint16_t* const* embeds, int S, void* stream) {
  if (!ctx) return GVL_ERR_ARG;
  if (n_seqs <= 0 || n_seqs > gvl_ctx::kMaxSeqs) return fail(ctx, GVL_ERR_ARG, "gvl_prefill_batch: bad arguments");
  int lens[gvl_ctx::kMaxSeqs];
  for (int i = 0; i < n_seqs; ++i) lens[i] = S;
  return gvl_prefill_varlen(ctx, seq_ids, n_seqs, embeds, lens, stream);
}

int gvl_decode_greedy(gvl_ctx* ctx, int seq_id, int max_new, int eos_id, int32_t* out_ids, int* n_out, void* stream) {
  return gvl_decode_greedy_batch(ctx, &seq_id, 1, max_new, eos_id, out_ids, n_out, stream);
}

int gvl_decode_greedy_batch(gvl_ctx* ctx, const int* seq_ids, int n_seqs, int max_new, int eos_id, int32_t* out_ids, int* n_out, void* stream) {
  REQUIRE_READY(ctx->has_llm, "gvl_decode_greedy_batch");
  if (!seq_ids || n_seqs <= 0 || n_seqs > gvl_ctx::kMaxSeqs || !out_ids || !n_out || max_new <= 0 || max_new > ctx->outlist_cap)
    return fail(ctx, GVL_ERR_ARG, "gvl_decode_greedy_batch: bad arguments");
  for (int i = 0; i < n_seqs; ++i) {
    const int id = seq_ids[i];
    if (!ctx->lookup(id)) return seq_fail(ctx, "gvl_decode_greedy_batch", SEQ_BAD);
    if (ctx->seqs[id].n_gen < 1) return fail(ctx, GVL_ERR_STATE, "gvl_decode_greedy: call gvl_prefill first");
    if (ctx->repeats(seq_ids, i)) return seq_fail(ctx, "gvl_decode_greedy_batch", SEQ_DUPLICATE);
  }
  hipStream_t st = (hipStream_t)stream;
  int i = 0;
  while (i < n_seqs) {
    const int left = n_seqs - i, B = decode_group_size(ctx, left);
    Seq* sqs[GVL_MAX_DECODE_BATCH]; int32_t* outs[GVL_MAX_DECODE_BATCH]; int* nouts[GVL_MAX_DECODE_BATCH];
    for (int b = 0; b < B; ++b) { sqs[b] = &ctx->seqs[seq_ids[i + b]]; outs[b] = out_ids + (size_t)(i + b) * max_new; nouts[b] = n_out + i + b; }
    const int rc = decode_group(ctx, sqs, B, max_new, eos_id, outs, nouts, st);
    if (rc) return rc;
    i += B;
  }
  return 0;
}

int gvl_decode_steps(gvl_ctx* ctx, const int* seq_ids, int n_seqs, int n_steps, void* stream) {
  REQUIRE_READY(ctx->has_llm, "gvl_decode_steps");
  if (!seq_ids || n_seqs <= 0 || n_seqs > gvl_ctx::kMaxSeqs || n_steps <= 0) return fail(ctx, GVL_ERR_ARG, "gvl_decode_steps: bad arguments");
  for (int i = 0; i < n_seqs; ++i) {
    const int id = seq_ids[i];
    if (!ctx->lookup(id)) return seq_fail(ctx, "gvl_decode_steps", SEQ_BAD);
    const Seq& sq = ctx->seqs[id];
    if (sq.n_gen < 1) return fail(ctx, GVL_ERR_STATE, "gvl_decode_steps: call gvl_prefill first");
    if (sq.pos + n_steps > sq.max_tokens || sq.n_gen + n_steps > ctx->outlist_cap) return fail(ctx, GVL_ERR_ARG, "gvl_decode_steps: sequence would exceed its capacity");
    if (ctx->repeats(seq_ids, i)) return seq_fail(ctx, "gvl_decode_steps", SEQ_DUPLICATE);
  }
  hipStream_t st = (hipStream_t)stream;
  for (int s = 0; s < n_steps; ++s) {
    int i = 0;
    while (i < n_seqs) {
      const int left = n_seqs - i, B = decode_group_size(ctx, left);
      Seq* sqs[GVL_MAX_DECODE_BATCH];
      for (int b = 0; b < B; ++b) sqs[b] = &ctx->seqs[seq_ids[i + b]];
      const int rc = decode_step(ctx, sqs, B, st);
      if (rc) return rc;
      i += B;
    }
  }
  return 0;
}

int gvl_seq_read(gvl_ctx* ctx, int seq_id, int first, int32_t* out_ids, int cap, int* n_gen, void* stream) {
  REQUIRE_READY(ctx->has_llm, "gvl_seq_read");
  if (!ctx->lookup(seq_id) || !n_gen || first < 0 || cap < 0 || (cap > 0 && !out_ids)) return fail(ctx, GVL_ERR_ARG, "gvl_seq_read: bad arguments");
  const Seq& sq = ctx->seqs[seq_id];
  *n_gen = sq.n_gen;
  int n = sq.n_gen - first; if (n > cap) n = cap;
  if (n > 0) {
    HIPCHK(ctx, hipStreamSynchronize((hipStream_t)stream));
    memcpy(out_ids, sq.h_out + first, (size_t)n * 4);
  }
  return 0;
}

int gvl_decode_step_logits(gvl_ctx* ctx, int seq_id, int tok, float* logits, void* stream) {
  REQUIRE_READY(ctx->has_llm, "gvl_decode_step_logits");
  if (!ctx->lookup(seq_id)) return seq_fail(ctx, "gvl_decode_step_logits", SEQ_BAD);
  Seq& sq = ctx->seqs[seq_id];
  if (tok < 0 || tok >= ctx->cfg.vocab || sq.pos >= sq.max_tokens || sq.pos == 0) return fail(ctx, GVL_ERR_ARG, "gvl_decode_step_logits: bad token / sequence full / not prefilled");
  hipStream_t st = (hipStream_t)stream;
  RUN(GVL_PROF_OTHER, 0, gvl_launch_set_int(sq.d_tok, tok, st));
  Seq* one[1] = {&sq};
  int rc = decode_step(ctx, one, 1, st);
  if (rc) return rc;
  if (logits) HIPCHK(ctx, hipMemcpyAsync(logits, ctx->d_logits, (size_t)ctx->cfg.vocab * 4, hipMemcpyDeviceToDevice, st));
  return 0;
}

int gvl_decode_step_logits_batch(gvl_ctx* ctx, const int* seq_ids, int n_seqs, const int32_t* toks, float* logits, void* stream) {
  REQUIRE_READY(ctx->has_llm, "gvl_decode_step_logits_batch");
  if (!seq_ids || !toks || n_seqs < 1 || n_seqs > decode_group_size(ctx, GVL_MAX_DECODE_BATCH) || (!ctx->decode_mfma && n_seqs == 3))
    return fail(ctx, GVL_ERR_ARG, "gvl_decode_step_logits_batch: 1 .. 16 sequences (VALU fallback geometries: 1, 2 or 4)");
  Seq* sqs[GVL_MAX_DECODE_BATCH];
  for (int i = 0; i < n_seqs; ++i) {
    const int id = seq_ids[i];
    if (!ctx->lookup(id)) return seq_fail(ctx, "gvl_decode_step_logits_batch", SEQ_BAD);
    Seq& sq = ctx->seqs[id];
    if (toks[i] < 0 || toks[i] >= ctx->cfg.vocab || sq.pos >= sq.max_tokens || sq.pos == 0) return fail(ctx, GVL_ERR_ARG, "gvl_decode_step_logits_batch: bad token / sequence full / not prefilled");
    if (ctx->repeats(seq_ids, i)) return seq_fail(ctx, "gvl_decode_step_logits_batch", SEQ_DUPLICATE);
    sqs[i] = &sq;
  }
  hipStream_t st = (hipStream_t)stream;
  for (int i = 0; i < n_seqs; ++i) RUN(GVL_PROF_OTHER, 0, gvl_launch_set_int(sqs[i]->d_tok, toks[i], st));
  const int rc = decode_step(ctx, sqs, n_seqs, st);
  if (rc) return rc;
  if (logits) HIPCHK(ctx, hipMemcpyAsync(logits, ctx->d_logits, (size_t)n_seqs * ctx->cfg.vocab * 4, hipMemcpyDeviceToDevice, st));
  return 0;
}

int gvl_debug_set(gvl_ctx* ctx, const char* key, int value) {
  if (!ctx || !key) return GVL_ERR_ARG;
  const std::string k = key;
  if (k == "decode_attn_cpb") { if (value < 0 || value > 16) return fail(ctx, GVL_ERR_ARG, "gvl_debug_set: decode_attn_cpb must be 0 (default) .. 16"); ctx->dbg.decode_attn_cpb = value; }
  else if (k == "decode_attn_hpb") { if (value < 0) return fail(ctx, GVL_ERR_ARG, "gvl_debug_set: decode_attn_hpb must be >= 0"); ctx->dbg.decode_attn_hpb = value; }
  else if (k == "decode_graph") ctx->dbg.decode_graph = value != 0;
  else if (k == "attn_ring") { if (value != 0 && value != 2 && value != 3) return fail(ctx, GVL_ERR_ARG, "gvl_debug_set: attn_ring must be 0, 2 or 3"); ctx->dbg.attn_ring = value; }
  else if (k == "prefill_group") { if (value < 1 || value > GVL_MAX_PREFILL_BATCH) return fail(ctx, GVL_ERR_ARG, "gvl_debug_set: prefill_group must be 1 .. 8"); ctx->dbg.prefill_group = value; }
  else if (k == "attn_pipe") { if (value < 0 || value > 2) return fail(ctx, GVL_ERR_ARG, "gvl_debug_set: attn_pipe must be 0, 1 or 2"); ctx->dbg.attn_pipe = value; }
  else if (k == "attn_pipe_rows") { if (value != 128 && value != 256) return fail(ctx, GVL_ERR_ARG, "gvl_debug_set: attn_pipe_rows must be 128 (default) or 256"); ctx->dbg.attn_pipe_rows = value; }
  else if (k == "patch_fused") ctx->dbg.patch_fused = value != 0;
  else if (k == "varlen_attn") ctx->dbg.varlen_attn = value < 0 || value > 2 ? 1 : value;
  else if (k == "norm_fused") ctx->dbg.norm_fused = value != 0;
  else if (k == "last_layer_tail") ctx->dbg.last_layer_tail = value != 0;
  else if (k == "gemm_band") { if (value < 0 || value > 64) return fail(ctx, GVL_ERR_ARG, "gvl_debug_set: gemm_band must be 0 (automatic) .. 64"); gvl_gemm_set_band(value); }
  else if (k == "gemm_a4") { if (value < 0 || value > 3) return fail(ctx, GVL_ERR_ARG, "gvl_debug_set: gemm_a4 must be 0 .. 3"); gvl_gemm_set_a4(value); }
  else if (k == "gemm_narrow") gvl_gemm_set_narrow(value < 0 || value > 2 ? 1 : value);
  else if (k == "vision_in_place") { if (value < 0 || value > 2) return fail(ctx, GVL_ERR_ARG, "gvl_debug_set: vision_in_place must be 0, 1 or 2"); ctx->dbg.vision_in_place = value; }
  else return fail(ctx, GVL_ERR_ARG, "gvl_debug_set: unknown key " + k);
  return 0;
}

int gvl_preprocess_frames(gvl_ctx* ctx, const uint8_t* frames, int n, int height, int width, int layout, int size,
                          const float* mean, const float* stdv, float* out, void* stream) {
  if (!ctx) return GVL_ERR_ARG;
  if (!frames || !out || !mean || !stdv || n <= 0 || height <= 0 || width <= 0 || size <= 0 || (layout != 0 && layout != 1))
    return fail(ctx, GVL_ERR_ARG, "gvl_preprocess_frames: bad arguments");
  for (int c = 0; c < 3; ++c) if (!(stdv[c] != 0.f)) return fail(ctx, GVL_ERR_ARG, "gvl_preprocess_frames: zero std");
  const int rc = gvl_launch_preprocess(frames, n, height, width, layout, size, mean, stdv, out, &ctx->pre_scratch, &ctx->pre_scratch_bytes, (hipStream_t)stream);
  if (rc == -2) return fail(ctx, GVL_ERR_OOM, "gvl_preprocess_frames: hipMalloc(scratch) failed");
  if (rc) return fail(ctx, rc == -1 ? GVL_ERR_ARG : GVL_ERR_HIP, "gvl_preprocess_frames: launch failed");
  return 0;
}

int gvl_prof_enable(gvl_ctx* ctx, int on) {
  if (!ctx) return GVL_ERR_ARG;
  hipDeviceSynchronize();
  for (auto& r : ctx->recs) { hipEventDestroy(r.e0); hipEventDestroy(r.e1); }
  ctx->recs.clear();
  for (int i = 0; i < GVL_PROF_NCAT; ++i) { ctx->prof_ms[i] = 0; ctx->prof_work[i] = 0; ctx->prof_n[i] = 0; }
  ctx->prof = on != 0;
  return 0;
}
int gvl_prof_read(gvl_ctx* ctx, int cat, double* total_ms, int64_t* launches, double* work) {
  if (!ctx || cat < 0 || cat >= GVL_PROF_NCAT) return GVL_ERR_ARG;
  hipDeviceSynchronize();
  for (auto& r : ctx->recs) {
    float ms = 0.f;
    if (hipEventElapsedTime(&ms, r.e0, r.e1) == hipSuccess) { ctx->prof_ms[r.cat] += ms; ctx->prof_work[r.cat] += r.work; ctx->prof_n[r.cat] += 1; }
    hipEventDestroy(r.e0); hipEventDestroy(r.e1);
  }
  ctx->recs.clear();
  if (total_ms) *total_ms = ctx->prof_ms[cat];
  if (launches) *launches = ctx->prof_n[cat];
  if (work) *work = ctx->prof_work[cat];
  return 0;
}

int gvl_op_gemm(gvl_ctx* ctx, const uint16_t* A, const uint16_t* W, void* C, int M, int N, int K, const float* bias, const float* gamma,
                const void* resid, int act, int out_f32, int tile_cfg, void* stream) {
  if (!ctx) return GVL_ERR_ARG;
  hipStream_t st = (hipStream_t)stream;
  GemmArgs g = gemm(A, K, W, C, act == GVL_ACT_SILU_MUL ? N / 2 : N, M, N, K);
  g.bias = bias; g.gamma = gamma; g.resid = resid; g.ldr = N; g.act = act; g.out_f32 = out_f32; g.round_pre_resid = 1; g.tile_cfg = tile_cfg;
  if (const char* e = gvl_lab_env("GVL_LAB_LD")) { int la = 0, lw = 0; if (sscanf(e, "%d,%d", &la, &lw) == 2) { g.lda = la; g.ldw = lw; } }
  RUN(GVL_PROF_GEMM, gvl_gemm_flops(g), gvl_launch_gemm(g, st));
  return 0;
}
int gvl_op_gemm_rows(gvl_ctx* ctx, const uint16_t* A, const uint16_t* W, uint16_t* C, int M, int N, int K, const float* bias, const float* gamma,
                     const uint16_t* resid, int act, const float* rowscale, float* rowsq, int rowsq_ld, int tile_cfg, void* stream) {
  if (!ctx) return GVL_ERR_ARG;
  hipStream_t st = (hipStream_t)stream;
  GemmArgs g = gemm(A, K, W, C, act == GVL_ACT_SILU_MUL ? N / 2 : N, M, N, K);
  g.bias = bias; g.gamma = gamma; g.resid = resid; g.ldr = N; g.act = act; g.round_pre_resid = 1; g.tile_cfg = tile_cfg;
  g.rowscale = rowscale; g.rowsq = rowsq; g.rowsq_ld = rowsq_ld;
  RUN(GVL_PROF_GEMM, gvl_gemm_flops(g), gvl_launch_gemm(g, st));
  return 0;
}
int gvl_op_fold_gamma(gvl_ctx* ctx, const uint16_t* W, const uint16_t* gamma, uint16_t* Wo, int64_t rows, int cols, void* stream) {
  if (!ctx) return GVL_ERR_ARG;
  hipStream_t st = (hipStream_t)stream;
  RUN(GVL_PROF_OTHER, 0, gvl_launch_fold_gamma(W, gamma, Wo, (long)rows, cols, st));
  return 0;
}
int gvl_op_rowsq_finish(gvl_ctx* ctx, const float* rowsq, int ld, int b0, int nblk, float* rs, int rows, int cols, float eps, void* stream) {
  if (!ctx) return GVL_ERR_ARG;
  hipStream_t st = (hipStream_t)stream;
  RUN(GVL_PROF_OTHER, 0, gvl_launch_rowsq_finish(rowsq, ld, b0, nblk, rs, rows, cols, eps, st));
  return 0;
}
int gvl_op_attention(gvl_ctx* ctx, const uint16_t* q, const uint16_t* k, const uint16_t* v, uint16_t* out, int B, int S, int H, int KV, int Dr,
                     float scale, int causal, void* stream) {
  if (!ctx) return GVL_ERR_ARG;
  if (k != q + (size_t)H * Dr || v != q + (size_t)(H + KV) * Dr) return fail(ctx, GVL_ERR_ARG, "gvl_op_attention: q,k,v must be the column blocks of one fused qkv tensor");
  const int D = pad_head(Dr);
  if (D < 0 || (Dr & 7)) return fail(ctx, GVL_ERR_ARG, "gvl_op_attention: head dim unsupported");
  hipStream_t st = (hipStream_t)stream;
// ... 80 lines not shown
```

### grounded-video-llm_amd/engine.py

```python
from __future__ import annotations

import ctypes as C
import os
from dataclasses import dataclass
from typing import Dict, List, Optional, Sequence, Tuple

import numpy as np
import torch

from . import lib as L
from . import logits as LP
from . import logprobs as LPR

bf = torch.bfloat16


@dataclass
class TowerGeometry:
    llm: str = "phi3.5"
    clip_hidden: int = 1024
    clip_inter: int = 4096
    clip_layers: int = 24
    clip_heads: int = 16
    clip_image: int = 336
# ... 211 lines not shown
        Lp = (self.geo.iv2_image // self.geo.iv2_patch) ** 2
        out = torch.empty((n, T * Lp, self.geo.iv2_dim), dtype=bf, device=self.device)
        self._chk(self.lib.gvl_iv2_encode(self.ctx, _ptr(px), n, _ptr(out), self.stream), "gvl_iv2_encode")
        return out

    @property
    def tokens_per_seg(self) -> int:
        return int(self.lib.gvl_tokens_per_seg(self.ctx))

    def build_visual(self, clip_feats: torch.Tensor, iv2_feats: torch.Tensor) -> torch.Tensor:
        n = clip_feats.shape[0]
        out = torch.empty((n * self.tokens_per_seg, self.geo.hidden), dtype=bf, device=self.device)
        self._chk(self.lib.gvl_build_visual(self.ctx, _ptr(clip_feats.contiguous()), _ptr(iv2_feats.contiguous()), n, _ptr(out), self.stream),
                  "gvl_build_visual")
        return out

    def encode_segments(self, spatial_px: torch.Tensor, temporal_px: torch.Tensor) -> torch.Tensor:
        sp = spatial_px.to(self.device, torch.float32).contiguous()
        tp = temporal_px.to(self.device, torch.float32).contiguous()
        n = sp.shape[0]
        out = torch.empty((n * self.tokens_per_seg, self.geo.hidden), dtype=bf, device=self.device)
        self._chk(self.lib.gvl_encode_segments(self.ctx, _ptr(sp), _ptr(tp), n, _ptr(out), self.stream), "gvl_encode_segments")
        return out

    def preprocess_frames(self, frames_u8: torch.Tensor, size: int, mean, std) -> torch.Tensor:
        assert frames_u8.dtype == torch.uint8 and frames_u8.dim() == 4
        if frames_u8.shape[-1] == 3 and frames_u8.shape[1] != 3:
            layout, (n, H, W) = 0, (frames_u8.shape[0], frames_u8.shape[1], frames_u8.shape[2])
        else:
            layout, (n, H, W) = 1, (frames_u8.shape[0], frames_u8.shape[2], frames_u8.shape[3])
        fr = frames_u8.to(self.device).contiguous()
        out = torch.empty((n, 3, size, size), dtype=torch.float32, device=self.device)
        m = (C.c_float * 3)(*[float(v) for v in mean]); s = (C.c_float * 3)(*[float(v) for v in std])
        self._chk(self.lib.gvl_preprocess_frames(self.ctx, _ptr(fr), n, H, W, layout, int(size), m, s, _ptr(out), self.stream), "gvl_preprocess_frames")
        return out

    def splice(self, input_ids: Sequence[int], visual: torch.Tensor) -> torch.Tensor:
        ids = (C.c_int64 * len(input_ids))(*[int(i) for i in input_ids])
        nv = visual.shape[0]
        out = torch.empty((len(input_ids) - 1 + nv, self.geo.hidden), dtype=bf, device=self.device)
        S = C.c_int(0)
        self._chk(self.lib.gvl_splice(self.ctx, ids, len(input_ids), _ptr(visual.contiguous()), nv, _ptr(out), C.byref(S), self.stream), "gvl_splice")
        assert S.value == out.shape[0]
        return out

    def seq_alloc(self, max_tokens: int) -> int:
        s = C.c_int(-1)
        self._chk(self.lib.gvl_seq_alloc(self.ctx, int(max_tokens), C.byref(s)), "gvl_seq_alloc")
        return s.value

    def seq_free(self, seq: int):
        self._chk(self.lib.gvl_seq_free(self.ctx, int(seq)), "gvl_seq_free")

    def seq_fork(self, src: int, n_tokens: int, max_tokens: int) -> int:
        sid = C.c_int(-1)
        self._chk(self.lib.gvl_seq_fork(self.ctx, int(src), int(n_tokens), int(max_tokens), C.byref(sid)), "gvl_seq_fork")
        return sid.value

    def seq_clone(self, src: int, max_tokens: int) -> int:
        sid = C.c_int(-1)
        self._chk(self.lib.gvl_seq_clone(self.ctx, int(src), int(max_tokens), C.byref(sid), self.stream), "gvl_seq_clone")
        return sid.value

    def prefill_extend(self, seq: int, embeds_new: torch.Tensor, want_logits: bool = False) -> Optional[torch.Tensor]:
        embeds_new = embeds_new.contiguous()
        assert embeds_new.dtype == bf and embeds_new.dim() == 2
        lg = torch.empty((self.geo.vocab,), dtype=torch.float32, device=self.device) if want_logits else None
        self._chk(self.lib.gvl_prefill_extend(self.ctx, int(seq), _ptr(embeds_new), embeds_new.shape[0], _ptr(lg), self.stream), "gvl_prefill_extend")
        return lg

    def prefill(self, seq: int, embeds: torch.Tensor, want_logits: bool = False) -> Optional[torch.Tensor]:
        embeds = embeds.contiguous()
        logits = torch.empty((self.geo.vocab,), dtype=torch.float32, device=self.device) if want_logits else None
        self._chk(self.lib.gvl_prefill(self.ctx, seq, _ptr(embeds), embeds.shape[0], _ptr(logits), self.stream), "gvl_prefill")
        return logits

    def decode_greedy(self, seq: int, max_new: int, eos_id: Optional[int]) -> List[int]:
        buf = (C.c_int32 * max_new)()
        n = C.c_int(0)
        self._chk(self.lib.gvl_decode_greedy(self.ctx, seq, int(max_new), -1 if eos_id is None else int(eos_id), buf, C.byref(n), self.stream),
                  "gvl_decode_greedy")
        return [int(buf[i]) for i in range(n.value)]

    def prefill_batch(self, seqs: Sequence[int], embeds: Sequence[torch.Tensor]) -> None:
        es = [e.contiguous() for e in embeds]
        n = len(seqs)
        ids = (C.c_int * n)(*[int(s) for s in seqs])
        ptrs = (C.c_void_p * n)(*[e.data_ptr() for e in es])
        lens = (C.c_int * n)(*[int(e.shape[0]) for e in es])
        self._chk(self.lib.gvl_prefill_varlen(self.ctx, ids, n, ptrs, lens, self.stream), "gvl_prefill_varlen")

    def decode_greedy_batch(self, seqs: Sequence[int], max_new: int, eos_id: Optional[int]) -> List[List[int]]:
        n = len(seqs)
        ids = (C.c_int * n)(*[int(s) for s in seqs])
        buf = (C.c_int32 * (n * max_new))()
        nout = (C.c_int * n)()
        self._chk(self.lib.gvl_decode_greedy_batch(self.ctx, ids, n, int(max_new), -1 if eos_id is None else int(eos_id), buf, nout, self.stream),
                  "gvl_decode_greedy_batch")
        return [[int(buf[i * max_new + j]) for j in range(nout[i])] for i in range(n)]

    def forward_loss(self, embeds: torch.Tensor, labels: Sequence[int]) -> Tuple[float, int]:
        embeds = embeds.contiguous()
        S = embeds.shape[0]
        assert len(labels) == S, "labels must cover every row of inputs_embeds"
        lab = (C.c_int64 * S)(*[int(v) for v in labels])
        nll, n = C.c_double(0.0), C.c_int(0)
        seq = self.seq_alloc(S)
        try:
            self._chk(self.lib.gvl_forward_loss(self.ctx, seq, _ptr(embeds), S, lab, C.byref(nll), C.byref(n), self.stream), "gvl_forward_loss")
        finally:
            self.seq_free(seq)
        return nll.value, n.value

    def decode_steps(self, seqs: Sequence[int], n_steps: int) -> None:
        n = len(seqs)
        ids = (C.c_int * n)(*[int(s) for s in seqs])
        self._chk(self.lib.gvl_decode_steps(self.ctx, ids, n, int(n_steps), self.stream), "gvl_decode_steps")

    def seq_read(self, seq: int, first: int = 0, cap: int = 4096) -> List[int]:
        buf = (C.c_int32 * max(cap, 1))()
        n = C.c_int(0)
        self._chk(self.lib.gvl_seq_read(self.ctx, int(seq), int(first), buf, int(cap), C.byref(n), self.stream), "gvl_seq_read")
        return [int(buf[i]) for i in range(max(0, min(n.value - first, cap)))]

    def decode_step_logits(self, seq: int, tok: int) -> torch.Tensor:
        logits = torch.empty((self.geo.vocab,), dtype=torch.float32, device=self.device)
        self._chk(self.lib.gvl_decode_step_logits(self.ctx, seq, int(tok), _ptr(logits), self.stream), "gvl_decode_step_logits")
        return logits

    def decode_step_logits_batch(self, seqs: Sequence[int], toks: Sequence[int]) -> torch.Tensor:
        n = len(seqs)
        logits = torch.empty((n, self.geo.vocab), dtype=torch.float32, device=self.device)
        ids = (C.c_int * n)(*[int(s) for s in seqs]); tk = (C.c_int32 * n)(*[int(t) for t in toks])
        self._chk(self.lib.gvl_decode_step_logits_batch(self.ctx, ids, n, tk, _ptr(logits), self.stream), "gvl_decode_step_logits_batch")
        return logits

    def generate_ids(self, embeds: torch.Tensor, max_new_tokens: int, eos_id: Optional[int], processors=None, logprobs: Optional[int] = None,
                     rules: Optional[int] = None):
        opts = LP.SeqOptions(processors, logprobs, ... if rules is None else rules)
        seq = self.seq_alloc(min(embeds.shape[0] + max_new_tokens, self.geo.max_seq))
        try:
            LP.apply_seq_options(self, seq, opts)
            self.prefill(seq, embeds)
            ids = self.decode_greedy(seq, max_new_tokens, eos_id)
            return ids if logprobs is None else (ids, LP.read_seq_logprobs(self, seq, ids, opts))
        finally:
            self.seq_free(seq)

    def trace_marker(self, tag: int = 0, stream=None):
        st = C.c_void_p(stream.cuda_stream) if stream is not None else self.stream
        self._chk(self.lib.gvl_trace_marker(int(tag), st), "gvl_trace_marker")

    def prof_enable(self, on: bool):
        self._chk(self.lib.gvl_prof_enable(self.ctx, 1 if on else 0), "gvl_prof_enable")

    def prof_read(self, cat: int):
        ms, n, w = C.c_double(0), C.c_int64(0), C.c_double(0)
        self._chk(self.lib.gvl_prof_read(self.ctx, cat, C.byref(ms), C.byref(n), C.byref(w)), "gvl_prof_read")
        return ms.value, n.value, w.value

    def op_gemm(self, A, W, bias=None, gamma=None, resid=None, act=L.ACT_NONE, out_f32=False, tile_cfg=0):
        M, K = A.shape
        N = W.shape[0]
        n_out = N // 2 if act == L.ACT_SILU_MUL else N
        Cc = torch.empty((M, n_out), dtype=torch.float32 if out_f32 else bf, device=self.device)
        self._chk(self.lib.gvl_op_gemm(self.ctx, _ptr(A.contiguous()), _ptr(W.contiguous()), _ptr(Cc), M, N, K, _ptr(bias), _ptr(gamma),
                                       _ptr(resid), act, 1 if out_f32 else 0, tile_cfg, self.stream), "gvl_op_gemm")
        return Cc

    def op_gemm_rows(self, A, W, bias=None, gamma=None, resid=None, act=L.ACT_NONE, rowscale=None, want_rowsq=False, tile_cfg=0):
        M, K = A.shape
        N = W.shape[0]
        n_out = N // 2 if act == L.ACT_SILU_MUL else N
# ... 200 lines not shown
```

### grounded-video-llm_amd/lib.py

```python
from __future__ import annotations

import ctypes as C
import os

_HERE = os.path.dirname(os.path.abspath(__file__))
LIB_PATH = os.environ.get("GVL_LIB_PATH") or os.path.join(_HERE, "libgvl.so")

F32, BF16, I32, I64 = 0, 1, 2, 3
LLM_PHI3, LLM_LLAMA = 0, 1
ACT_NONE, ACT_QUICK_GELU, ACT_GELU, ACT_SILU_MUL = 0, 1, 2, 3
PROF_GEMM, PROF_ATTN, PROF_GEMV, PROF_DECODE_ATTN, PROF_OTHER = 0, 1, 2, 3, 4


class GvlConfig(C.Structure):
    _fields_ = [
        ("llm_kind", C.c_int32),
        ("clip_hidden", C.c_int32), ("clip_inter", C.c_int32), ("clip_layers_run", C.c_int32), ("clip_heads", C.c_int32),
        ("clip_image", C.c_int32), ("clip_patch", C.c_int32),
        ("iv2_dim", C.c_int32), ("iv2_inter", C.c_int32), ("iv2_blocks_run", C.c_int32), ("iv2_heads", C.c_int32),
        ("iv2_image", C.c_int32), ("iv2_patch", C.c_int32), ("iv2_frames_per_seg", C.c_int32),
        ("hidden", C.c_int32), ("inter", C.c_int32), ("layers", C.c_int32), ("heads", C.c_int32), ("kv_heads", C.c_int32),
        ("vocab", C.c_int32),
        ("rms_eps", C.c_float),
        ("lm_head_bias", C.c_int32), ("rope_orig_max_pos", C.c_int32), ("max_seq", C.c_int32),
        ("max_segs", C.c_int32), ("kv_pages", C.c_int32), ("max_prefill", C.c_int32), ("decode_fp8", C.c_int32),
    ]


class GvlBiasTable(C.Structure):
    _fields_ = [("n_targets", C.c_int32), ("targets", C.POINTER(C.c_int32)), ("n_entries", C.c_int32), ("entry_bias", C.POINTER(C.c_float)),
                ("entry_prefix", C.POINTER(C.c_int32)), ("n_prefix", C.c_int32), ("prefix", C.POINTER(C.c_int32))]


class GvlRulesDesc(C.Structure):
    _fields_ = [("n_suppress", C.c_int32), ("suppress", C.POINTER(C.c_int32)), ("n_begin_suppress", C.c_int32), ("begin_suppress", C.POINTER(C.c_int32)),
                ("begin_index", C.c_int32), ("n_force", C.c_int32), ("force_ids", C.POINTER(C.c_int32)), ("force_at", C.c_int32), ("bias", GvlBiasTable * 2)]


class GvlSampling(C.Structure):
    _fields_ = [("do_sample", C.c_int32), ("temperature", C.c_float), ("top_k", C.c_int32), ("top_p", C.c_float), ("min_p", C.c_float),
                ("typical_p", C.c_float), ("epsilon_cutoff", C.c_float), ("eta_cutoff", C.c_float), ("seed", C.c_uint64), ("stream", C.c_uint32)]


_SIGS = {
    "gvl_create": (C.c_int, [C.POINTER(GvlConfig), C.POINTER(C.c_void_p)]),
    "gvl_destroy": (C.c_int, [C.c_void_p]),
    "gvl_last_error": (C.c_char_p, [C.c_void_p]),
    "gvl_device_info": (C.c_int, [C.c_char_p, C.c_int, C.POINTER(C.c_int)]),
    "gvl_load_weight": (C.c_int, [C.c_void_p, C.c_char_p, C.c_void_p, C.c_int, C.POINTER(C.c_int64), C.c_int, C.c_int]),
    "gvl_finalize_weights": (C.c_int, [C.c_void_p]),
    "gvl_load_packed": (C.c_int, [C.c_void_p, C.c_char_p, C.POINTER(C.c_int)]),
    "gvl_kv_info": (C.c_int, [C.c_void_p, C.POINTER(C.c_int), C.POINTER(C.c_int), C.POINTER(C.c_int64), C.POINTER(C.c_int)]),
    "gvl_comm_unique_id": (C.c_int, [C.c_char_p]),
    "gvl_comm_init": (C.c_int, [C.c_void_p, C.c_char_p, C.c_int, C.c_int]),
    "gvl_comm_destroy": (C.c_int, [C.c_void_p]),
    "gvl_decode_group_info": (C.c_int, [C.c_void_p, C.POINTER(C.c_int), C.POINTER(C.c_int)]),
    "gvl_comm_count": (C.c_int, [C.c_void_p, C.POINTER(C.c_int)]),
    "gvl_allgather_visual": (C.c_int, [C.c_void_p, C.c_void_p, C.c_void_p, C.c_int, C.c_int, C.c_void_p, C.c_void_p]),
    "gvl_allgatherv_visual": (C.c_int, [C.c_void_p, C.c_void_p, C.c_void_p, C.POINTER(C.c_int), C.c_int, C.c_void_p, C.c_void_p]),
    "gvl_clip_encode": (C.c_int, [C.c_void_p, C.c_void_p, C.c_int, C.c_void_p, C.c_void_p]),
    "gvl_iv2_encode": (C.c_int, [C.c_void_p, C.c_void_p, C.c_int, C.c_void_p, C.c_void_p]),
    "gvl_build_visual": (C.c_int, [C.c_void_p, C.c_void_p, C.c_void_p, C.c_int, C.c_void_p, C.c_void_p]),
    "gvl_tokens_per_seg": (C.c_int, [C.c_void_p]),
    "gvl_encode_segments": (C.c_int, [C.c_void_p, C.c_void_p, C.c_void_p, C.c_int, C.c_void_p, C.c_void_p]),
    "gvl_splice": (C.c_int, [C.c_void_p, C.POINTER(C.c_int64), C.c_int, C.c_void_p, C.c_int, C.c_void_p, C.POINTER(C.c_int), C.c_void_p]),
    "gvl_seq_alloc": (C.c_int, [C.c_void_p, C.c_int, C.POINTER(C.c_int)]),
    "gvl_seq_free": (C.c_int, [C.c_void_p, C.c_int]),
    "gvl_seq_fork": (C.c_int, [C.c_void_p, C.c_int, C.c_int, C.c_int, C.POINTER(C.c_int)]),
    "gvl_seq_clone": (C.c_int, [C.c_void_p, C.c_int, C.c_int, C.POINTER(C.c_int), C.c_void_p]),
    "gvl_prefill_extend": (C.c_int, [C.c_void_p, C.c_int, C.c_void_p, C.c_int, C.c_void_p, C.c_void_p]),
    "gvl_prefill": (C.c_int, [C.c_void_p, C.c_int, C.c_void_p, C.c_int, C.c_void_p, C.c_void_p]),
    "gvl_decode_greedy": (C.c_int, [C.c_void_p, C.c_int, C.c_int, C.c_int, C.POINTER(C.c_int32), C.POINTER(C.c_int), C.c_void_p]),
    "gvl_preprocess_frames": (C.c_int, [C.c_void_p, C.c_void_p, C.c_int, C.c_int, C.c_int, C.c_int, C.c_int, C.POINTER(C.c_float), C.POINTER(C.c_float), C.c_void_p, C.c_void_p]),
    "gvl_prefill_batch": (C.c_int, [C.c_void_p, C.POINTER(C.c_int), C.c_int, C.POINTER(C.c_void_p), C.c_int, C.c_void_p]),
    "gvl_decode_steps": (C.c_int, [C.c_void_p, C.POINTER(C.c_int), C.c_int, C.c_int, C.c_void_p]),
    "gvl_seq_read": (C.c_int, [C.c_void_p, C.c_int, C.c_int, C.POINTER(C.c_int32), C.c_int, C.POINTER(C.c_int), C.c_void_p]),
    "gvl_forward_loss": (C.c_int, [C.c_void_p, C.c_int, C.c_void_p, C.c_int, C.POINTER(C.c_int64), C.POINTER(C.c_double), C.POINTER(C.c_int), C.c_void_p]),
    "gvl_prefill_varlen": (C.c_int, [C.c_void_p, C.POINTER(C.c_int), C.c_int, C.POINTER(C.c_void_p), C.POINTER(C.c_int), C.c_void_p]),
    "gvl_decode_greedy_batch": (C.c_int, [C.c_void_p, C.POINTER(C.c_int), C.c_int, C.c_int, C.c_int, C.POINTER(C.c_int32), C.POINTER(C.c_int), C.c_void_p]),
    "gvl_decode_step_logits": (C.c_int, [C.c_void_p, C.c_int, C.c_int, C.c_void_p, C.c_void_p]),
    "gvl_decode_step_logits_batch": (C.c_int, [C.c_void_p, C.POINTER(C.c_int), C.c_int, C.POINTER(C.c_int32), C.c_void_p, C.c_void_p]),
    "gvl_prof_enable": (C.c_int, [C.c_void_p, C.c_int]),
    "gvl_prof_read": (C.c_int, [C.c_void_p, C.c_int, C.POINTER(C.c_double), C.POINTER(C.c_int64), C.POINTER(C.c_double)]),
    "gvl_op_gemm": (C.c_int, [C.c_void_p, C.c_void_p, C.c_void_p, C.c_void_p, C.c_int, C.c_int, C.c_int, C.c_void_p, C.c_void_p,
                              C.c_void_p, C.c_int, C.c_int, C.c_int, C.c_void_p]),
    "gvl_op_gemm_rows": (C.c_int, [C.c_void_p, C.c_void_p, C.c_void_p, C.c_void_p, C.c_int, C.c_int, C.c_int, C.c_void_p, C.c_void_p,
                                   C.c_void_p, C.c_int, C.c_void_p, C.c_void_p, C.c_int, C.c_int, C.c_void_p]),
    "gvl_op_fold_gamma": (C.c_int, [C.c_void_p, C.c_void_p, C.c_void_p, C.c_void_p, C.c_int64, C.c_int, C.c_void_p]),
    "gvl_op_rowsq_finish": (C.c_int, [C.c_void_p, C.c_void_p, C.c_int, C.c_int, C.c_int, C.c_void_p, C.c_int, C.c_int, C.c_float, C.c_void_p]),
    "gvl_op_attention": (C.c_int, [C.c_void_p, C.c_void_p, C.c_void_p, C.c_void_p, C.c_void_p, C.c_int, C.c_int, C.c_int, C.c_int,
                                   C.c_int, C.c_float, C.c_int, C.c_void_p]),
    "gvl_op_layernorm": (C.c_int, [C.c_void_p, C.c_void_p, C.c_void_p, C.c_void_p, C.c_void_p, C.c_int, C.c_int, C.c_float, C.c_void_p]),
    "gvl_op_rmsnorm": (C.c_int, [C.c_void_p, C.c_void_p, C.c_void_p, C.c_void_p, C.c_int, C.c_int, C.c_float, C.c_void_p]),
    "gvl_debug_set": (C.c_int, [C.c_void_p, C.c_char_p, C.c_int]),
    "gvl_set_sampling": (C.c_int, [C.c_void_p, C.c_int, C.c_float, C.c_int, C.c_float, C.c_uint64]),
    "gvl_set_sampling_ex": (C.c_int, [C.c_void_p, C.POINTER(GvlSampling)]),
    "gvl_seq_set_sampling": (C.c_int, [C.c_void_p, C.c_int, C.POINTER(GvlSampling)]),
    "gvl_op_select_rows": (C.c_int, [C.c_void_p, C.c_void_p, C.c_int, C.c_int, C.POINTER(GvlSampling), C.c_void_p, C.POINTER(C.c_int), C.c_void_p, C.c_void_p,
                                     C.c_void_p, C.c_void_p, C.c_void_p, C.c_void_p]),
    "gvl_op_sample": (C.c_int, [C.c_void_p, C.c_void_p, C.c_int, C.c_int, C.c_float, C.c_int, C.c_float, C.c_uint64, C.c_void_p, C.c_void_p, C.c_void_p, C.c_void_p]),
    "gvl_set_logits_processors": (C.c_int, [C.c_void_p, C.c_float, C.c_int, C.c_int, C.c_int]),
    "gvl_seq_set_processors": (C.c_int, [C.c_void_p, C.c_int, C.c_float, C.c_int, C.c_int, C.c_int]),
    "gvl_op_logits_process": (C.c_int, [C.c_void_p, C.c_void_p, C.c_int, C.c_int, C.c_void_p, C.c_int, C.c_void_p, C.POINTER(C.c_float),
                                        C.POINTER(C.c_int), C.POINTER(C.c_int), C.POINTER(C.c_int), C.c_void_p]),
    "gvl_rules_create": (C.c_int, [C.c_void_p, C.POINTER(GvlRulesDesc), C.POINTER(C.c_int)]),
    "gvl_rules_destroy": (C.c_int, [C.c_void_p, C.c_int]),
    "gvl_set_token_rules": (C.c_int, [C.c_void_p, C.c_int]),
    "gvl_seq_set_token_rules": (C.c_int, [C.c_void_p, C.c_int, C.c_int]),
    "gvl_op_logits_process_rules": (C.c_int, [C.c_void_p, C.c_void_p, C.c_int, C.c_int, C.c_void_p, C.c_int, C.c_void_p, C.POINTER(C.c_float),
                                              C.POINTER(C.c_int), C.POINTER(C.c_int), C.POINTER(C.c_int), C.POINTER(C.c_int), C.c_void_p]),
    "gvl_set_logprobs": (C.c_int, [C.c_void_p, C.c_int]),
    "gvl_seq_set_logprobs": (C.c_int, [C.c_void_p, C.c_int, C.c_int]),
    "gvl_seq_read_logprobs": (C.c_int, [C.c_void_p, C.c_int, C.c_int, C.c_int, C.c_void_p, C.c_void_p, C.c_void_p, C.POINTER(C.c_int), C.c_void_p]),
    "gvl_op_select_logprobs": (C.c_int, [C.c_void_p, C.c_void_p, C.c_int, C.c_int, C.c_int, C.c_float, C.c_int, C.c_float, C.c_uint64, C.c_void_p,
                                         C.c_void_p, C.POINTER(C.c_int), C.c_void_p, C.c_void_p, C.c_void_p, C.c_void_p, C.c_void_p]),
    "gvl_op_dgemm": (C.c_int, [C.c_void_p, C.c_void_p, C.c_void_p, C.c_void_p, C.c_void_p, C.c_int, C.c_int, C.c_int, C.c_void_p]),
    "gvl_op_decode_bench": (C.c_int, [C.c_void_p, C.c_int, C.c_int, C.c_int, C.c_int, C.c_int, C.c_int, C.c_int, C.POINTER(C.c_double), C.c_void_p]),
    "gvl_probe_mfma": (C.c_int, [C.c_int, C.c_int, C.c_int, C.POINTER(C.c_double), C.POINTER(C.c_double), C.c_void_p]),
    "gvl_trace_marker": (C.c_int, [C.c_int, C.c_void_p]),
    "gvl_op_gemv": (C.c_int, [C.c_void_p, C.c_void_p, C.c_void_p, C.c_void_p, C.c_void_p, C.c_int, C.c_int, C.c_void_p]),
}
EXPORTS = tuple(_SIGS)

_lib = None


def load():
    global _lib
    if _lib is not None:
        return _lib
    if not os.path.exists(LIB_PATH):
        raise RuntimeError(
            f"{LIB_PATH} not found: the HIP extension is required (no CPU / PyTorch fallback exists). "
            "Build it with `python __graft_entry__.py build` (hipcc --offload-arch=gfx950).")
    try:
        lib = C.CDLL(LIB_PATH, mode=C.RTLD_GLOBAL)
    except OSError as e:
        raise RuntimeError(f"cannot load {LIB_PATH}: {e}") from e
    for name, (res, args) in _SIGS.items():
        fn = getattr(lib, name)
        fn.restype = res
        fn.argtypes = args
    _lib = lib
    return lib


ERR_ARG, ERR_STATE, ERR_HIP, ERR_OOM, ERR_NOGPU = -1, -2, -3, -4, -5


class GvlError(RuntimeError):
    status = 0


def check(lib, ctx, rc, what=""):
    if rc != 0:
        msg = lib.gvl_last_error(ctx)
        err = GvlError(f"{what} failed (status {rc}): {msg.decode() if msg else ''}")
        err.status = rc
        raise err
```

### include/gvl.h

```cpp
#ifndef GVL_H
#define GVL_H

#include <stdint.h>

#ifdef __cplusplus
extern "C" {
#endif

typedef struct gvl_ctx gvl_ctx;

typedef enum {
  GVL_OK = 0,
  GVL_ERR_ARG = -1,
  GVL_ERR_STATE = -2,
  GVL_ERR_HIP = -3,
  GVL_ERR_OOM = -4,
  GVL_ERR_NOGPU = -5
} gvl_status;

enum { GVL_F32 = 0, GVL_BF16 = 1, GVL_I32 = 2, GVL_I64 = 3 };
enum { GVL_LLM_PHI3 = 0, GVL_LLM_LLAMA = 1 };

typedef struct {
  int32_t llm_kind;
// ... 2 lines not shown
  int32_t hidden, inter, layers, heads, kv_heads, vocab;
  float rms_eps;
  int32_t lm_head_bias;
  int32_t rope_orig_max_pos;
  int32_t max_seq;
  int32_t max_segs;
  int32_t kv_pages;
  int32_t max_prefill;
  int32_t decode_fp8;
} gvl_config;

int gvl_create(const gvl_config* cfg, gvl_ctx** out);
int gvl_destroy(gvl_ctx* ctx);
const char* gvl_last_error(const gvl_ctx* ctx);
int gvl_device_info(char* arch_out, int arch_len, int* num_cus);

int gvl_load_weight(gvl_ctx* ctx, const char* name, const void* data, int dtype, const int64_t* shape,
                    int ndim, int is_device);
int gvl_finalize_weights(gvl_ctx* ctx);
int gvl_load_packed(gvl_ctx* ctx, const char* path, int* n_loaded);

int gvl_clip_encode(gvl_ctx* ctx, const float* px, int n_images, float* out, void* stream);

int gvl_iv2_encode(gvl_ctx* ctx, const float* px, int n_segs, uint16_t* out, void* stream);

int gvl_build_visual(gvl_ctx* ctx, const float* clip_feats, const uint16_t* iv2_feats, int n_segs,
                     uint16_t* visual, void* stream);
int gvl_tokens_per_seg(const gvl_ctx* ctx);

int gvl_encode_segments(gvl_ctx* ctx, const float* spatial_px, const float* temporal_px, int n_segs,
                        uint16_t* visual, void* stream);

int gvl_splice(gvl_ctx* ctx, const int64_t* ids_host, int n_ids, const uint16_t* visual, int n_visual,
               uint16_t* embeds, int* seq_len_out, void* stream);

int gvl_seq_alloc(gvl_ctx* ctx, int max_tokens, int* seq_id);
int gvl_seq_free(gvl_ctx* ctx, int seq_id);
int gvl_seq_fork(gvl_ctx* ctx, int src_seq, int n_tokens, int max_tokens, int* dst_seq);
int gvl_prefill_extend(gvl_ctx* ctx, int seq_id, const uint16_t* embeds_new, int n_new, float* last_logits, void* stream);
int gvl_seq_clone(gvl_ctx* ctx, int src_seq, int max_tokens, int* dst_seq, void* stream);
int gvl_kv_info(const gvl_ctx* ctx, int* total_pages, int* free_pages, int64_t* pool_bytes, int* max_live_seqs);
int gvl_decode_group_info(const gvl_ctx* ctx, int* max_group, int* any_size);
int gvl_prefill(gvl_ctx* ctx, int seq_id, const uint16_t* embeds, int seq_len, float* last_logits,
                void* stream);
int gvl_decode_greedy(gvl_ctx* ctx, int seq_id, int max_new, int eos_id, int32_t* out_ids_host,
                      int* n_out, void* stream);
int gvl_set_sampling(gvl_ctx* ctx, int do_sample, float temperature, int top_k, float top_p, uint64_t seed);
typedef struct {
  int32_t do_sample;
  float temperature;
  int32_t top_k;
  float top_p;
  float min_p;
  float typical_p;
  float epsilon_cutoff;
  float eta_cutoff;
  uint64_t seed; uint32_t stream;
} gvl_sampling;
int gvl_set_sampling_ex(gvl_ctx* ctx, const gvl_sampling* sampling);
int gvl_seq_set_sampling(gvl_ctx* ctx, int seq_id, const gvl_sampling* sampling);
int gvl_set_logits_processors(gvl_ctx* ctx, float penalty, int ngram, int min_new, int eos_id);
int gvl_seq_set_processors(gvl_ctx* ctx, int seq_id, float penalty, int ngram, int min_new, int eos_id);
typedef struct {
  int32_t n_targets; const int32_t* targets;
  int32_t n_entries; const float* entry_bias; const int32_t* entry_prefix;
  int32_t n_prefix; const int32_t* prefix;
} gvl_bias_table;
typedef struct {
  int32_t n_suppress; const int32_t* suppress;
  int32_t n_begin_suppress; const int32_t* begin_suppress; int32_t begin_index;
  int32_t n_force; const int32_t* force_ids; int32_t force_at;
  gvl_bias_table bias[2];
} gvl_rules_desc;
int gvl_rules_create(gvl_ctx* ctx, const gvl_rules_desc* desc, int* rules_id);
int gvl_rules_destroy(gvl_ctx* ctx, int rules_id);
int gvl_set_token_rules(gvl_ctx* ctx, int rules_id);
int gvl_seq_set_token_rules(gvl_ctx* ctx, int seq_id, int rules_id);
int gvl_set_logprobs(gvl_ctx* ctx, int top_n);
int gvl_seq_set_logprobs(gvl_ctx* ctx, int seq_id, int top_n);
int gvl_seq_read_logprobs(gvl_ctx* ctx, int seq_id, int first, int cap, float* lp_host, int32_t* top_ids_host, float* top_lp_host, int* n_gen,
                          void* stream);
int gvl_prefill_varlen(gvl_ctx* ctx, const int* seq_ids, int n_seqs, const uint16_t* const* embeds,
                       const int* seq_lens, void* stream);
int gvl_prefill_batch(gvl_ctx* ctx, const int* seq_ids, int n_seqs, const uint16_t* const* embeds, int seq_len,
                      void* stream);
int gvl_decode_greedy_batch(gvl_ctx* ctx, const int* seq_ids, int n_seqs, int max_new, int eos_id,
                            int32_t* out_ids_host, int* n_out, void* stream);
int gvl_decode_steps(gvl_ctx* ctx, const int* seq_ids, int n_seqs, int n_steps, void* stream);
int gvl_seq_read(gvl_ctx* ctx, int seq_id, int first, int32_t* out_ids_host, int cap, int* n_gen, void* stream);
int gvl_decode_step_logits(gvl_ctx* ctx, int seq_id, int tok, float* logits, void* stream);
int gvl_decode_step_logits_batch(gvl_ctx* ctx, const int* seq_ids, int n_seqs, const int32_t* toks, float* logits, void* stream);

int gvl_comm_unique_id(char id_out[128]);
int gvl_comm_init(gvl_ctx* ctx, const char id[128], int rank, int world);
int gvl_comm_destroy(gvl_ctx* ctx);
int gvl_comm_count(gvl_ctx* ctx, int* n_ranks);
int gvl_allgather_visual(gvl_ctx* ctx, void* comm, const uint16_t* local, int rows_per_rank, int hidden, uint16_t* all,
                         void* stream);
int gvl_allgatherv_visual(gvl_ctx* ctx, void* comm, const uint16_t* local, const int* rows_per_rank, int hidden, uint16_t* all, void* stream);

int gvl_forward_loss(gvl_ctx* ctx, int seq_id, const uint16_t* embeds, int seq_len, const int64_t* labels_host,
                     double* nll_sum, int* n_valid, void* stream);

int gvl_preprocess_frames(gvl_ctx* ctx, const uint8_t* frames, int n, int height, int width, int layout, int size,
                          const float* mean, const float* std3, float* out, void* stream);

enum { GVL_PROF_GEMM = 0, GVL_PROF_ATTN = 1, GVL_PROF_GEMV = 2, GVL_PROF_DECODE_ATTN = 3, GVL_PROF_OTHER = 4,
       GVL_PROF_NCAT = 5 };
int gvl_prof_enable(gvl_ctx* ctx, int on);
int gvl_prof_read(gvl_ctx* ctx, int category, double* total_ms, int64_t* launches, double* work);

int gvl_debug_set(gvl_ctx* ctx, const char* key, int value);

int gvl_op_gemm(gvl_ctx* ctx, const uint16_t* A, const uint16_t* W, void* C, int M, int N, int K,
                const float* bias, const float* gamma, const void* resid, int act, int out_f32,
                int tile_cfg, void* stream);
int gvl_op_gemm_rows(gvl_ctx* ctx, const uint16_t* A, const uint16_t* W, uint16_t* C, int M, int N, int K, const float* bias, const float* gamma,
                     const uint16_t* resid, int act, const float* rowscale, float* rowsq, int rowsq_ld, int tile_cfg, void* stream);
int gvl_op_fold_gamma(gvl_ctx* ctx, const uint16_t* W, const uint16_t* gamma, uint16_t* Wo, int64_t rows, int cols, void* stream);
int gvl_op_rowsq_finish(gvl_ctx* ctx, const float* rowsq, int ld, int b0, int nblk, float* rs, int rows, int cols, float eps, void* stream);
int gvl_op_attention(gvl_ctx* ctx, const uint16_t* q, const uint16_t* k, const uint16_t* v, uint16_t* out,
                     int B, int S, int H, int KV, int D, float scale, int causal, void* stream);
int gvl_op_layernorm(gvl_ctx* ctx, const float* x, const float* w, const float* b, uint16_t* y, int rows,
                     int cols, float eps, void* stream);
int gvl_op_rmsnorm(gvl_ctx* ctx, const uint16_t* x, const uint16_t* w, uint16_t* y, int rows, int cols,
                   float eps, void* stream);
int gvl_op_gemv(gvl_ctx* ctx, const uint16_t* W, const uint16_t* x, const float* bias, float* y, int N, int K,
                void* stream);
int gvl_op_sample(gvl_ctx* ctx, const float* logits, int n, int batch, float temperature, int top_k, float top_p, uint64_t seed,
                  const uint32_t* streams, const int32_t* steps_dev, int32_t* tokens_dev, void* stream);
int gvl_op_logits_process(gvl_ctx* ctx, float* logits, int n, int batch, const int32_t* hist_dev, int hist_stride, const int32_t* lens_dev,
                          const float* penalty, const int* ngram, const int* min_new, const int* eos_ids, void* stream);
int gvl_op_logits_process_rules(gvl_ctx* ctx, float* logits, int n, int batch, const int32_t* hist_dev, int hist_stride, const int32_t* lens_dev,
                                const float* penalty, const int* ngram, const int* min_new, const int* eos_ids, const int* rules_ids, void* stream);
int gvl_op_select_logprobs(gvl_ctx* ctx, const float* logits, int n, int batch, int do_sample, float temperature, int top_k, float top_p,
                           uint64_t seed, const uint32_t* streams, const int32_t* steps_dev, const int* top_n, int32_t* tokens_dev,
                           float* lp_dev, int32_t* top_ids_dev, float* top_lp_dev, void* stream);
int gvl_op_select_rows(gvl_ctx* ctx, const float* logits, int n, int batch, const gvl_sampling* rows, const int32_t* steps_dev, const int* top_n,
                       int32_t* tokens_dev, float* lp_dev, int32_t* top_ids_dev, float* top_lp_dev, uint8_t* kept_dev, void* stream);
int gvl_op_dgemm(gvl_ctx* ctx, const uint16_t* W, const uint16_t* x, const float* bias, float* y, int N, int K, int batch,
                 void* stream);
int gvl_op_decode_bench(gvl_ctx* ctx, int N, int K, int batch, int mode, int variant, int rounds, int iters, double* us_per_launch,
                        void* stream);

int gvl_probe_mfma(int mode, int waves_per_simd, int iters, double* tflops, double* ghz, void* stream);
int gvl_trace_marker(int tag, void* stream);

#ifdef __cplusplus
}
#endif
#endif
```

Measured before the change: 11.66 clips/s.

## Apply Q RoPE inside prefill attention and write K/V pages directly

Prefill attention now reads Q straight from the fused QKV rows and applies rotary embedding in registers, with new kernel variants for full and partial rotary dims. A new kv_pages kernel applies RoPE to K and writes K plus transposed V into the paged cache in one pass. This removes the separate qkv_post and V-transpose launches and the round trip of a rotated Q buffer through memory. It adds template variants, extra cos/sin loads per attention block, and a new plan mode that falls back when its preconditions fail. It also adds a prefill API that returns the last-position logits, which is new functionality.

```diff
diff --git a/grounded-video-llm_amd/csrc/gvl_attn.hip b/grounded-video-llm_amd/csrc/gvl_attn.hip
--- a/grounded-video-llm_amd/csrc/gvl_attn.hip
+++ b/grounded-video-llm_amd/csrc/gvl_attn.hip
@@ -45,7 +45,7 @@
   return (b >> 1) * 16 + 8 * hh + 4 * (b & 1) + c;
 }
 
-template <int D, int NWAVES, int NS, int ONES = 0, int VROW = 0, int VL = 0>
+template <int D, int NWAVES, int NS, int ONES = 0, int VROW = 0, int VL = 0, int QR = 0>
 __global__ __launch_bounds__(NWAVES * 64) void attn_fwd_kernel(const AttnArgs a) {
   constexpr int NT = NWAVES * 64;
   constexpr int DK = D / 16;
@@ -62,7 +62,9 @@
   const int tid = threadIdx.x, lane = tid & 63;
   const int wave = __builtin_amdgcn_readfirstlane(tid >> 6);
   const int l31 = lane & 31, h = lane >> 5;
+  static_assert(!QR || (VROW == 0 && ONES == 0 && D % 32 == 0 && (QR == 1 || D == 64)), "q in place + RoPE: paged K / V, whole rotate_half pairs per lane");
   int S_ = a.S;
+  int qrow0 = 0;
   const bf16_t* Qp_ = a.Q; bf16_t* Op_ = a.O; const int* tbl_ = a.block_table;
   int nq = (a.S + NWAVES * 32 - 1) / (NWAVES * 32);
   const int rep = a.H / a.KV;
@@ -77,6 +79,7 @@
     while (qb >= nqu && u + 1 < a.vl_n) { qb -= nqu; ++u; nqu = (a.vl_rows[u + 1] - a.vl_rows[u] + NWAVES * 32 - 1) / (NWAVES * 32); }
     const int r0 = a.vl_rows[u];
     S_ = a.vl_rows[u + 1] - r0;
+    qrow0 = r0;
     Qp_ = a.Q + (size_t)r0 * a.H * D;
     Op_ = a.O + (size_t)r0 * (size_t)(a.H * a.Dout);
     tbl_ = a.vl_tables[u];
@@ -107,6 +110,7 @@
   constexpr bool FOLD = VROW == 3;
   u32x4_t qf[DK];
   u32x4_t qraw[DK], qw_[VROW == 3 ? DK : 1];
+  f32x4_t rcos[QR == 1 ? DK / 2 : 1][2], rsin[QR == 1 ? DK / 2 : 1][2];
   float q_rs = 1.f;
   {
     int qi = qw + l31; if (qi > S_ - 1) qi = S_ - 1;
@@ -119,6 +123,18 @@
         const bool real = kk * 16 + 8 * h < a.Dout;
         qraw[kk] = real ? *(const u32x4_t*)(qp + kk * 16) : u32x4_t{0u, 0u, 0u, 0u};
         qw_[kk] = real ? *(const u32x4_t*)(wp + kk * 16) : u32x4_t{0u, 0u, 0u, 0u};
+      }
+    } else if constexpr (QR == 2) {
+    } else if constexpr (QR == 1) {
+      const bf16_t* qp = a.Qrows + ((size_t)qrow0 + (size_t)b * S_ + qi) * a.q_ld + head * D + 8 * h;
+      const float* cp = a.rope_cos + (size_t)qi * (D / 2) + 8 * h;
+      const float* sp = a.rope_sin + (size_t)qi * (D / 2) + 8 * h;
+#pragma unroll
+      for (int kk = 0; kk < DK; ++kk) qraw[kk] = *(const u32x4_t*)(qp + kk * 16);
+#pragma unroll
+      for (int kk = 0; kk < DK / 2; ++kk) {
+        rcos[kk][0] = *(const f32x4_t*)(cp + kk * 16); rcos[kk][1] = *(const f32x4_t*)(cp + kk * 16 + 4);
+        rsin[kk][0] = *(const f32x4_t*)(sp + kk * 16); rsin[kk][1] = *(const f32x4_t*)(sp + kk * 16 + 4);
       }
     } else {
       const bf16_t* qp = VROW == 2 ? a.Qrows + ((size_t)b * S_ + qi) * a.q_ld + head * D + 8 * h : Qp_ + (((size_t)b * a.H + head) * S_ + qi) * D + 8 * h;
@@ -209,15 +225,57 @@
 
   stage(0, 0);
   if (NS == 3 && n_tiles > 1) stage(1, 1);
-#pragma unroll
-  for (int kk = 0; kk < DK; ++kk) {
-    if constexpr (VROW == 3) {
-      u32x4_t o;
-#pragma unroll
-      for (int e = 0; e < 4; ++e) o[e] = pack2bf(lo_bf(qw_[kk][e]) * rbf(lo_bf(qraw[kk][e]) * q_rs) * sc, hi_bf(qw_[kk][e]) * rbf(hi_bf(qraw[kk][e]) * q_rs) * sc);
+  if constexpr (QR == 2) {
+    const int cpr = a.Dout >> 3, hc = cpr >> 1;
+    int qi = qw + l31; if (qi > S_ - 1) qi = S_ - 1;
+    const bf16_t* qp = a.Qrows + ((size_t)qrow0 + (size_t)b * S_ + qi) * a.q_ld + head * a.Dout;
+    const float* cp = a.rope_cos + (size_t)qi * (a.Dout >> 1);
+    const float* sp = a.rope_sin + (size_t)qi * (a.Dout >> 1);
+#pragma unroll
+    for (int kk = 0; kk < DK; ++kk) {
+      const int c = 2 * kk + h;
+      u32x4_t o = {0u, 0u, 0u, 0u};
+      if (c < cpr) {
+        const bool first = c < hc;
+        const u32x4_t v = *(const u32x4_t*)(qp + c * 8), p = *(const u32x4_t*)(qp + (first ? c + hc : c - hc) * 8);
+        const int j0 = (first ? c : c - hc) * 8;
+        const f32x4_t c0 = *(const f32x4_t*)(cp + j0), c1 = *(const f32x4_t*)(cp + j0 + 4), s0 = *(const f32x4_t*)(sp + j0), s1 = *(const f32x4_t*)(sp + j0 + 4);
+        const float sg = first ? -1.f : 1.f;
+        const float cc[8] = {c0[0], c0[1], c0[2], c0[3], c1[0], c1[1], c1[2], c1[3]};
+        const float ss[8] = {s0[0], s0[1], s0[2], s0[3], s1[0], s1[1], s1[2], s1[3]};
+#pragma unroll
+        for (int e = 0; e < 4; ++e) {
+          const float x0 = lo_bf(v[e]), x1 = hi_bf(v[e]), p0 = sg * lo_bf(p[e]), p1 = sg * hi_bf(p[e]);
+          o[e] = pack2bf(rbf(x0 * cc[2 * e]) + rbf(p0 * ss[2 * e]), rbf(x1 * cc[2 * e + 1]) + rbf(p1 * ss[2 * e + 1]));
+        }
+      }
       qf[kk] = o;
-    } else {
-      qf[kk] = qraw[kk];
+    }
+  } else if constexpr (QR == 1) {
+#pragma unroll
+    for (int kk = 0; kk < DK / 2; ++kk) {
+      const u32x4_t x = qraw[kk], y = qraw[kk + DK / 2];
+      u32x4_t lo, hi;
+#pragma unroll
+      for (int e = 0; e < 4; ++e) {
+        const float c0 = rcos[kk][e >> 1][2 * (e & 1)], c1 = rcos[kk][e >> 1][2 * (e & 1) + 1], s0 = rsin[kk][e >> 1][2 * (e & 1)], s1 = rsin[kk][e >> 1][2 * (e & 1) + 1];
+        const float x0 = lo_bf(x[e]), x1 = hi_bf(x[e]), y0 = lo_bf(y[e]), y1 = hi_bf(y[e]);
+        lo[e] = pack2bf(rbf(x0 * c0) + rbf(-y0 * s0), rbf(x1 * c1) + rbf(-y1 * s1));
+        hi[e] = pack2bf(rbf(y0 * c0) + rbf(x0 * s0), rbf(y1 * c1) + rbf(x1 * s1));
+      }
+      qf[kk] = lo; qf[kk + DK / 2] = hi;
+    }
+  } else {
+#pragma unroll
+    for (int kk = 0; kk < DK; ++kk) {
+      if constexpr (VROW == 3) {
+        u32x4_t o;
+#pragma unroll
+        for (int e = 0; e < 4; ++e) o[e] = pack2bf(lo_bf(qw_[kk][e]) * rbf(lo_bf(qraw[kk][e]) * q_rs) * sc, hi_bf(qw_[kk][e]) * rbf(hi_bf(qraw[kk][e]) * q_rs) * sc);
+        qf[kk] = o;
+      } else {
+        qf[kk] = qraw[kk];
+      }
     }
   }
 #pragma unroll
@@ -805,6 +863,16 @@
   return hipGetLastError() == hipSuccess ? 0 : -3;
 }
 static int launch_attn(const AttnArgs& a, const AttnLaunch& l, hipStream_t st) {
+  if (l.QROPE) {
+    if (l.ONES || l.VROW) return -1;
+    switch (attn_fwd_key(l.D, l.NWAVES, l.NS, 0, 0, l.VL) * 4 + l.QROPE) {
+#define GVL_CASE(D, NWAVES, NS, VL, QR) \
+      case attn_fwd_key(D, NWAVES, NS, 0, 0, VL) * 4 + QR: { static GvlDevOnce once; return launch_planned(attn_fwd_kernel<D, NWAVES, NS, 0, 0, VL, QR>, once, a, l, st); }
+      GVL_ATTN_FWD_QROPE_LIST(GVL_CASE)
+#undef GVL_CASE
+      default: return -1;
+    }
+  }
   switch (attn_fwd_key(l.D, l.NWAVES, l.NS, l.ONES, l.VROW, l.VL)) {
 #define GVL_CASE(D, NWAVES, NS, ONES, VROW, VL) \
     case attn_fwd_key(D, NWAVES, NS, ONES, VROW, VL): { static GvlDevOnce once; return launch_planned(attn_fwd_kernel<D, NWAVES, NS, ONES, VROW, VL>, once, a, l, st); }
@@ -844,6 +912,7 @@
   for (int u = 0; u <= GVL_MAX_PREFILL_BATCH; ++u) g.vl_rows[u] = a.vl_rows[u];
   for (int u = 0; u < GVL_MAX_PREFILL_BATCH; ++u) g.vl_tables[u] = a.vl_tables[u] != nullptr;
   g.block_table = a.block_table; g.Vrows = a.Vrows; g.Qrows = a.Qrows; g.Krows = a.Krows; g.q_rs = a.q_rs; g.q_nw = a.q_nw;
+  g.q_rope = a.rope_cos || a.rope_sin; g.rope16 = a.rope_cos && a.rope_sin && al16(a.rope_cos) && al16(a.rope_sin);
   g.O16 = al16(a.O); g.Vrows16 = al16(a.Vrows); g.Qrows16 = al16(a.Qrows); g.Krows16 = al16(a.Krows); g.q_nw16 = al16(a.q_nw);
   AttnLaunch plan[GVL_ATTN_MAX_LAUNCHES];
   const int n = attn_plan(g, knobs, plan);
diff --git a/grounded-video-llm_amd/csrc/gvl_attn_plan.h b/grounded-video-llm_amd/csrc/gvl_attn_plan.h
--- a/grounded-video-llm_amd/csrc/gvl_attn_plan.h
+++ b/grounded-video-llm_amd/csrc/gvl_attn_plan.h
@@ -7,6 +7,7 @@
   GVL_ATTN_QKV_ROWS,
   GVL_ATTN_QNORM_V_ROWS,
   GVL_ATTN_RAGGED,
+  GVL_ATTN_QROPE,
 };
 enum AttnFamily : int { GVL_ATTN_FWD = 0, GVL_ATTN_IV2_PIPE };
 
@@ -17,6 +18,7 @@
   X(128, 4, 2, 0, 0, 0) X(128, 4, 3, 0, 0, 0)                                                                    \
   X(64, 4, 2, 0, 0, 1) X(96, 4, 2, 0, 0, 1) X(128, 4, 2, 0, 0, 1)
 #define GVL_ATTN_IV2_PIPE_LIST(X) X(4) X(8)
+#define GVL_ATTN_FWD_QROPE_LIST(X) X(64, 4, 2, 0, 1) X(64, 4, 2, 1, 1) X(96, 4, 2, 0, 1) X(96, 4, 2, 1, 1) X(128, 4, 2, 0, 1) X(128, 4, 2, 1, 1) X(64, 4, 2, 0, 2) X(64, 4, 2, 1, 2)
 constexpr int attn_fwd_key(int D, int NWAVES, int NS, int ONES, int VROW, int VL) { return ((((D * 16 + NWAVES) * 4 + NS) * 2 + ONES) * 4 + VROW) * 2 + VL; }
 
 struct AttnGeometry {
@@ -24,6 +26,7 @@
   int vl_n, vl_rows[GVL_MAX_PREFILL_BATCH + 1];
   bool block_table, Vrows, Qrows, Krows, q_rs, q_nw, vl_tables[GVL_MAX_PREFILL_BATCH];
   bool O16, Vrows16, Qrows16, Krows16, q_nw16;
+  bool q_rope, rope16;
 };
 struct AttnKnobs {
   float lazy;
@@ -37,11 +40,12 @@
   unsigned grid; int block, lds;
   int q_begin, q_rows;
   float lazy;
+  int QROPE = 0;
 };
 constexpr int GVL_ATTN_MAX_LAUNCHES = 2;
 
 inline int attn_mode_of(const AttnGeometry& g) {
-  return g.vl_n ? GVL_ATTN_RAGGED : (g.q_rs || g.q_nw) ? GVL_ATTN_QNORM_V_ROWS : (g.Krows || g.Qrows) ? GVL_ATTN_QKV_ROWS : g.Vrows ? GVL_ATTN_V_ROWS : GVL_ATTN_PAGED;
+  return g.q_rope ? GVL_ATTN_QROPE : g.vl_n ? GVL_ATTN_RAGGED : (g.q_rs || g.q_nw) ? GVL_ATTN_QNORM_V_ROWS : (g.Krows || g.Qrows) ? GVL_ATTN_QKV_ROWS : g.Vrows ? GVL_ATTN_V_ROWS : GVL_ATTN_PAGED;
 }
 inline bool attn_pitch_ok(int ld, long long width, bool ptr16) { return ld >= width && (ld & 7) == 0 && ptr16; }
 inline bool attn_tile_below_4g(int ld) { return (unsigned long long)64 * (unsigned long long)ld * 2 < 0xffffffffull; }
@@ -61,11 +65,20 @@
 inline bool attn_qnorm_v_rows_ok(const AttnGeometry& g) {
   return attn_v_rows_ok(g) && g.q_rs && g.q_nw && g.Qrows && !g.Krows && g.D == 96 && g.Dout == 88 && g.k_ones && attn_pitch_ok(g.q_ld, (long long)g.H * g.Dout, g.Qrows16 && g.q_nw16);
 }
-inline bool attn_ragged_ok(const AttnGeometry& g) {
-  if (g.vl_n < 1 || g.vl_n > GVL_MAX_PREFILL_BATCH || g.B != 1 || !g.causal || g.Sk || g.qpos0 || g.Vrows || g.Qrows || g.Krows || g.q_rs || g.q_nw || g.block_table) return false;
+inline bool attn_ragged_rows_ok(const AttnGeometry& g) {
+  if (g.vl_n < 1 || g.vl_n > GVL_MAX_PREFILL_BATCH || g.B != 1 || !g.causal || g.Sk || g.qpos0 || g.block_table) return false;
   for (int u = 0; u < g.vl_n; ++u)
     if (!g.vl_tables[u] || g.vl_rows[u + 1] <= g.vl_rows[u] || g.vl_rows[u + 1] - g.vl_rows[u] > g.S) return false;
   return true;
+}
+inline bool attn_ragged_ok(const AttnGeometry& g) {
+  return !(g.Vrows || g.Qrows || g.Krows || g.q_rs || g.q_nw) && attn_ragged_rows_ok(g);
+}
+inline int attn_qrope_form(const AttnGeometry& g) { return g.Dout == g.D ? 1 : g.D == 64 && g.Dout >= 16 && (g.Dout & 15) == 0 ? 2 : 0; }
+inline bool attn_qrope_ok(const AttnGeometry& g) {
+  if (!g.q_rope || !g.rope16 || !g.Qrows || g.Krows || g.Vrows || g.q_rs || g.q_nw || !g.causal || g.Sk || g.qpos0 || !attn_qrope_form(g) || g.ones_row || g.k_ones) return false;
+  if (!attn_pitch_ok(g.q_ld, (long long)g.H * g.Dout, g.Qrows16)) return false;
+  return g.vl_n ? attn_ragged_rows_ok(g) : true;
 }
 
 inline int attn_plan(const AttnGeometry& g, const AttnKnobs& k, AttnLaunch out[GVL_ATTN_MAX_LAUNCHES]) {
@@ -77,11 +90,13 @@
     case GVL_ATTN_V_ROWS: if (!attn_v_rows_ok(g)) return -1; break;
     case GVL_ATTN_QKV_ROWS: if (!attn_qkv_rows_ok(g)) return -1; break;
     case GVL_ATTN_QNORM_V_ROWS: if (!attn_qnorm_v_rows_ok(g)) return -1; break;
+    case GVL_ATTN_QROPE: if (!attn_qrope_ok(g)) return -1; break;
     default: if (!attn_ragged_ok(g)) return -1; break;
   }
   const float lazy = k.lazy >= 0.f && k.lazy <= 64.f ? k.lazy : GVL_ATTN_KNOBS_DEFAULT.lazy;
   const long long groups8 = (((long long)g.KV * g.B + 7) / 8) * 8;
-  const int vrow = mode == GVL_ATTN_RAGGED ? 0 : mode, vl = mode == GVL_ATTN_RAGGED;
+  const int qrope = mode == GVL_ATTN_QROPE ? attn_qrope_form(g) : 0;
+  const int vrow = mode == GVL_ATTN_RAGGED || qrope ? 0 : mode, vl = mode == GVL_ATTN_RAGGED || (qrope && g.vl_n);
   const int lr = g.Dout - 64;
   const bool ones = g.D == 96 && !vl && g.ones_row && !k.no_ones && g.Dout < 96 && lr >= 0 && (lr & 7) < 4 && !g.causal;
 
@@ -105,7 +120,7 @@
   const long long grid = groups8 * (g.H / g.KV) * nq;
   if (grid > 0x7fffffffll) return -1;
   out[0] = AttnLaunch{mode, GVL_ATTN_FWD, g.D, nwaves, ns, ones, vrow, vl, (unsigned)grid, 64 * nwaves, ns * 2 * 64 * g.D * 2 + 1024 ,
-                      0, g.S, lazy};
+                      0, g.S, lazy, qrope};
   return 1;
 }
 
diff --git a/grounded-video-llm_amd/csrc/gvl_ctx.h b/grounded-video-llm_amd/csrc/gvl_ctx.h
--- a/grounded-video-llm_amd/csrc/gvl_ctx.h
+++ b/grounded-video-llm_amd/csrc/gvl_ctx.h
@@ -94,7 +94,7 @@
            float min_p = 0.f, typical_p = 0.f, eps = 0.f, eta = 0.f;
            bool warps() const { return on && (min_p > 0.f || (typical_p > 0.f && typical_p < 1.f) || eps > 0.f || eta > 0.f); } } sample;
   float* d_seq_lp = nullptr; int* d_seq_top_ids = nullptr; float* d_seq_top_lp = nullptr;
-  struct { int decode_attn_cpb = 0, decode_attn_hpb = 0; bool decode_graph = true; int vision_in_place = 1, prefill_group = 4, attn_ring = 0, attn_pipe = 1, attn_pipe_rows = 128, patch_fused = 1, varlen_attn = 1, norm_fused = 1, last_layer_tail = 1; } dbg;
+  struct { int decode_attn_cpb = 0, decode_attn_hpb = 0; bool decode_graph = true; int vision_in_place = 1, prefill_group = 4, attn_ring = 0, attn_pipe = 1, attn_pipe_rows = 128, patch_fused = 1, varlen_attn = 1, norm_fused = 1, last_layer_tail = 1, prefill_q_in_place = 1; } dbg;
   void* comm = nullptr; int comm_rank = 0, comm_world = 1;
   bool prof = false; std::vector<ProfRec> recs;
   double prof_ms[GVL_PROF_NCAT] = {0}, prof_work[GVL_PROF_NCAT] = {0}; int64_t prof_n[GVL_PROF_NCAT] = {0};
diff --git a/grounded-video-llm_amd/csrc/gvl_elem.hip b/grounded-video-llm_amd/csrc/gvl_elem.hip
--- a/grounded-video-llm_amd/csrc/gvl_elem.hip
+++ b/grounded-video-llm_amd/csrc/gvl_elem.hip
@@ -421,9 +421,86 @@
   }
 }
 
+__global__ __launch_bounds__(256) void kv_pages_kernel(const QkvPostArgs a) {
+  __shared__ __attribute__((aligned(16))) bf16_t tile[64][136];
+  int t = blockIdx.x, S_ = a.S, row0 = 0;
+  const int hkv = blockIdx.y, b = blockIdx.z;
+  const int* table = a.block_table;
+  if (a.vl_n) {
+    int u = 0, t0 = 0;
+    for (; u + 1 < a.vl_n; ++u) { const int nt = (a.vl_rows[u + 1] - a.vl_rows[u] + 63) >> 6; if (t < t0 + nt) break; t0 += nt; }
+    t -= t0; row0 = a.vl_rows[u]; S_ = a.vl_rows[u + 1] - row0; table = a.vl_tables[u];
+  }
+  const int tid = threadIdx.x;
+  const int n_tiles = (S_ + 63) >> 6;
+  const int page = table ? table[b * a.max_pages + t] : b * n_tiles + t;
+  const int cpr = a.Dr >> 3, cpd = a.D >> 3, half = a.Dr >> 1, hc = half >> 3;
+  const bf16_t* rows = a.qkv + ((size_t)b * S_ + row0 + (size_t)t * 64) * a.ld;
+  const int koff = a.H * a.Dr + hkv * a.Dr, voff = koff + a.KV * a.Dr;
+  int live = S_ - t * 64; if (live > 64) live = 64;
+  for (int i = tid; i < 64 * cpr; i += 256) {
+    const int r = i / cpr, c = i - r * cpr;
+    u32x4_t v = {0u, 0u, 0u, 0u};
+    if (r < live) v = *(const u32x4_t*)(rows + (size_t)r * a.ld + voff + c * 8);
+    *(u32x4_t*)&tile[r][c * 8] = v;
+  }
+  bf16_t* Kb = a.Kt + ((size_t)page * a.KV + hkv) * (64 * a.D);
+  for (int i = tid; i < 64 * hc; i += 256) {
+    const int r = i / hc, c = i - r * hc;
+    if (r >= live) continue;
+    const bf16_t* kr = rows + (size_t)r * a.ld + koff;
+    const u32x4_t x = *(const u32x4_t*)(kr + c * 8), y = *(const u32x4_t*)(kr + (c + hc) * 8);
+    const float* cp = a.cos + (size_t)(t * 64 + r) * half + c * 8;
+    const float* sp = a.sin + (size_t)(t * 64 + r) * half + c * 8;
+    const f32x4_t c0 = *(const f32x4_t*)cp, c1 = *(const f32x4_t*)(cp + 4), s0 = *(const f32x4_t*)sp, s1 = *(const f32x4_t*)(sp + 4);
+    const float cc[8] = {c0[0], c0[1], c0[2], c0[3], c1[0], c1[1], c1[2], c1[3]};
+    const float ss[8] = {s0[0], s0[1], s0[2], s0[3], s1[0], s1[1], s1[2], s1[3]};
+    u32x4_t lo, hi;
+#pragma unroll
+    for (int e = 0; e < 4; ++e) {
+      const float x0 = lo_bf(x[e]), x1 = hi_bf(x[e]), y0 = lo_bf(y[e]), y1 = hi_bf(y[e]);
+      lo[e] = pack2bf(rbf(x0 * cc[2 * e]) + rbf(-y0 * ss[2 * e]), rbf(x1 * cc[2 * e + 1]) + rbf(-y1 * ss[2 * e + 1]));
+      hi[e] = pack2bf(rbf(y0 * cc[2 * e]) + rbf(x0 * ss[2 * e]), rbf(y1 * cc[2 * e + 1]) + rbf(x1 * ss[2 * e + 1]));
+    }
+    *(u32x4_t*)(Kb + (size_t)r * a.D + c * 8) = lo;
+    *(u32x4_t*)(Kb + (size_t)r * a.D + (c + hc) * 8) = hi;
+  }
+  if (cpd > cpr) {
+    const int np = cpd - cpr;
+    for (int i = tid; i < 64 * np; i += 256) {
+      const int r = i / np, c = i - r * np;
+      if (r >= live) continue;
+      u32x4_t v = {0u, 0u, 0u, 0u}; if (a.k_ones && c == 0) v[0] = 0x3F80u;
+      *(u32x4_t*)(Kb + (size_t)r * a.D + (cpr + c) * 8) = v;
+    }
+  }
+  __syncthreads();
+  bf16_t* dst = a.Vt + ((size_t)page * a.KV + hkv) * (64 * a.D);
+  for (int i = tid; i < a.D * 8; i += 256) {
+    const int d = i >> 3, k8 = (i & 7) * 8;
+    u32x4_t o = {0u, 0u, 0u, 0u};
+    if (d < a.Dr) {
+#pragma unroll
+      for (int e = 0; e < 4; ++e) o[e] = (unsigned)tile[k8 + 2 * e][d] | ((unsigned)tile[k8 + 2 * e + 1][d] << 16);
+    } else if (a.ones_row && d == a.Dr) {
+      o = u32x4_t{0x3F803F80u, 0x3F803F80u, 0x3F803F80u, 0x3F803F80u};
+    }
+    *(u32x4_t*)(dst + d * 64 + k8) = o;
+  }
+}
+
+static bool qkv_post_args_ok(const QkvPostArgs& a) {
+  if ((a.Dr & 7) || (a.mode == 2 && (a.Dr & 15)) || (a.D & 7) || a.D < a.Dr || a.Dr > 128 || (a.ld & 7)) return false;
+  if (a.vl_n && (a.mode != 2 || a.B != 1 || a.pos0 != 0 || a.pos_ptr || a.vl_n > GVL_MAX_PREFILL_BATCH)) return false;
+  return true;
+}
+static dim3 kv_tile_grid(const QkvPostArgs& a) {
+  int n_tiles = (a.S + 63) >> 6;
+  if (a.vl_n) { n_tiles = 0; for (int u = 0; u < a.vl_n; ++u) n_tiles += (a.vl_rows[u + 1] - a.vl_rows[u] + 63) >> 6; }
+  return dim3(n_tiles, a.KV, a.B);
+}
 int gvl_launch_qkv_post(const QkvPostArgs& a, hipStream_t st) {
-  if ((a.Dr & 7) || (a.mode == 2 && (a.Dr & 15)) || (a.D & 7) || a.D < a.Dr || a.Dr > 128 || (a.ld & 7)) return -1;
-  if (a.vl_n && (a.mode != 2 || a.B != 1 || a.pos0 != 0 || a.pos_ptr || a.vl_n > GVL_MAX_PREFILL_BATCH)) return -1;
+  if (!qkv_post_args_ok(a)) return -1;
   const int rows = a.vl_n ? a.vl_rows[a.vl_n] : a.B * a.S;
   if (a.q_rs && (a.mode != 1 || a.pos_ptr)) return -1;
   if (a.pos_ptr) {
@@ -432,11 +509,19 @@
   } else {
     hipLaunchKernelGGL(qkv_post_kernel<1>, dim3((rows + 3) / 4), dim3(256), 0, st, a);
   }
-  if (!a.pos_ptr && a.Vt) {
-    int n_tiles = (a.S + 63) >> 6;
-    if (a.vl_n) { n_tiles = 0; for (int u = 0; u < a.vl_n; ++u) n_tiles += (a.vl_rows[u + 1] - a.vl_rows[u] + 63) >> 6; }
-    hipLaunchKernelGGL(v_transpose_kernel, dim3(n_tiles, a.KV, a.B), dim3(256), 0, st, a);
-  }
+  if (!a.pos_ptr && a.Vt) hipLaunchKernelGGL(v_transpose_kernel, kv_tile_grid(a), dim3(256), 0, st, a);
+  return CHECK_LAUNCH();
+}
+int gvl_launch_v_transpose(const QkvPostArgs& a, hipStream_t st) {
+  if (!qkv_post_args_ok(a) || a.pos_ptr || !a.Vt) return -1;
+  hipLaunchKernelGGL(v_transpose_kernel, kv_tile_grid(a), dim3(256), 0, st, a);
+  return CHECK_LAUNCH();
+}
+int gvl_launch_kv_pages(const QkvPostArgs& a, hipStream_t st) {
+  if (!qkv_post_args_ok(a) || a.mode != 2 || a.pos0 != 0 || a.pos_ptr || !a.Kt || !a.Vt || !a.cos || !a.sin || a.Dr < 16) return -1;
+  if (!a.vl_n && (a.B < 1 || a.S < 1)) return -1;
+  for (int u = 0; u < a.vl_n; ++u) if (a.vl_rows[u + 1] <= a.vl_rows[u] || !a.vl_tables[u]) return -1;
+  hipLaunchKernelGGL(kv_pages_kernel, kv_tile_grid(a), dim3(256), 0, st, a);
   return CHECK_LAUNCH();
 }
 
diff --git a/grounded-video-llm_amd/csrc/gvl_internal.h b/grounded-video-llm_amd/csrc/gvl_internal.h
--- a/grounded-video-llm_amd/csrc/gvl_internal.h
+++ b/grounded-video-llm_amd/csrc/gvl_internal.h
@@ -164,6 +164,7 @@
   int q_ld, k_ld;
   int k_ones;
   const float* q_rs; const bf16_t* q_nw;
+  const float* rope_cos; const float* rope_sin;
   bf16_t* O;
   const int* block_table;
   int max_pages;
@@ -240,6 +241,8 @@
   const int* vl_tables[GVL_MAX_PREFILL_BATCH];
 };
 int gvl_launch_qkv_post(const QkvPostArgs& a, hipStream_t st);
+int gvl_launch_v_transpose(const QkvPostArgs& a, hipStream_t st);
+int gvl_launch_kv_pages(const QkvPostArgs& a, hipStream_t st);
 int gvl_launch_hd_merge(const float* f, const float* sub_gn, bf16_t* out, int n, int C, hipStream_t st);
 int gvl_launch_pool_spatial(const float* f, bf16_t* out, int n, int C, hipStream_t st);
 int gvl_launch_pool_temporal(const bf16_t* f, bf16_t* out, int n, int T, int C, hipStream_t st);
diff --git a/grounded-video-llm_amd/csrc/gvl_llm.hip b/grounded-video-llm_amd/csrc/gvl_llm.hip
--- a/grounded-video-llm_amd/csrc/gvl_llm.hip
+++ b/grounded-video-llm_amd/csrc/gvl_llm.hip
@@ -119,17 +119,28 @@
     }
     const bool vl_attn = n_att > 1 && ctx->dbg.varlen_attn && pos0 == 0;
     bool vl_post = vl_attn && ctx->dbg.varlen_attn == 1;
-    if (vl_post && f.rope_orig_max_pos > 0 && ctx->cos_l) {
+    bool rope_mixed = false;
+    if (n_att > 1 && f.rope_orig_max_pos > 0 && ctx->cos_l) {
       const bool l0 = lens[0] > f.rope_orig_max_pos;
-      for (int u = 1; u < nb; ++u) vl_post = vl_post && (lens[u] > f.rope_orig_max_pos) == l0;
-    }
+      for (int u = 1; u < nb; ++u) rope_mixed = rope_mixed || (lens[u] > f.rope_orig_max_pos) != l0;
+    }
+    vl_post = vl_post && !rope_mixed;
+    const bool qip = ctx->dbg.prefill_q_in_place && pos0 == 0 && (Dr == D || (D == 64 && Dr >= 16 && (Dr & 15) == 0)) && !(vl_attn && rope_mixed);
+    auto kv_append = [&](QkvPostArgs& q) -> int {
+      if (qip) { q.Q = nullptr; RUN(GVL_PROF_OTHER, 0, gvl_launch_kv_pages(q, st)); return 0; }
+      bf16_t* Vt_ = q.Vt; q.Vt = nullptr;
+      RUN(GVL_PROF_OTHER, 0, gvl_launch_qkv_post(q, st));
+      q.Vt = Vt_;
+      RUN(GVL_PROF_OTHER, 0, gvl_launch_v_transpose(q, st));
+      return 0;
+    };
+    const bool group_long = f.rope_orig_max_pos > 0 && lens[0] > f.rope_orig_max_pos && ctx->cos_l;
     if (vl_post) {
-      const bool use_long = f.rope_orig_max_pos > 0 && lens[0] > f.rope_orig_max_pos && ctx->cos_l;
       QkvPostArgs q; memset(&q, 0, sizeof(q)); q.qkv = qkv; q.ld = qkvw; q.Q = Q; q.Kt = Kt; q.Vt = Vt; q.B = 1; q.H = H; q.KV = KV; q.Dr = Dr; q.D = D; q.mode = 2;
-      q.cos = use_long ? ctx->cos_l : ctx->cos_s; q.sin = use_long ? ctx->sin_l : ctx->sin_s; q.vl_n = nb;
+      q.cos = group_long ? ctx->cos_l : ctx->cos_s; q.sin = group_long ? ctx->sin_l : ctx->sin_s; q.vl_n = nb;
       for (int u = 0; u < nb; ++u) { q.vl_rows[u] = off[u]; q.vl_tables[u] = sqs[u]->d_block_table; q.S = lens[u] > q.S ? lens[u] : q.S; }
       q.vl_rows[nb] = off[nb];
-      RUN(GVL_PROF_OTHER, 0, gvl_launch_qkv_post(q, st));
+      if (const int rc = kv_append(q)) return rc;
     }
     for (int u = 0; u < n_att && !vl_post; ++u) {
       const int S = lens[u], B = n_att == 1 ? nb : 1;
@@ -139,17 +150,19 @@
       bf16_t* Qu = Q + (size_t)off[u] * H * D;
       { QkvPostArgs q; memset(&q, 0, sizeof(q)); q.qkv = qkv + (size_t)off[u] * qkvw; q.ld = qkvw; q.Q = Qu; q.Kt = Kt; q.Vt = Vt; q.block_table = tbl; q.max_pages = tstride;
         q.B = B; q.S = S; q.H = H; q.KV = KV; q.Dr = Dr; q.D = D; q.mode = 2; q.cos = use_long ? ctx->cos_l : ctx->cos_s; q.sin = use_long ? ctx->sin_l : ctx->sin_s; q.pos0 = pos0;
-        RUN(GVL_PROF_OTHER, 0, gvl_launch_qkv_post(q, st)); }
+        if (const int rc = kv_append(q)) return rc; }
       if (vl_attn) continue;
       { AttnArgs a; memset(&a, 0, sizeof(a)); a.Q = Qu; a.Kt = Kt; a.Vt = Vt; a.O = att + (size_t)off[u] * H * Dr; a.block_table = tbl; a.max_pages = tstride;
         a.B = B; a.H = H; a.KV = KV; a.S = S; a.D = D; a.Dout = Dr; a.scale = 1.0f / sqrtf((float)Dr); a.causal = 1;
         if (pos0) { a.Sk = pos0 + S; a.qpos0 = pos0; }
+        if (qip) { a.Q = nullptr; a.Qrows = qkv + (size_t)off[u] * qkvw; a.q_ld = qkvw; a.rope_cos = use_long ? ctx->cos_l : ctx->cos_s; a.rope_sin = use_long ? ctx->sin_l : ctx->sin_s; }
         a.ring = ctx->dbg.attn_ring;
         RUN(GVL_PROF_ATTN, gvl_attn_flops(a), gvl_launch_attention(a, st)); }
     }
     if (vl_attn) {
       AttnArgs a; memset(&a, 0, sizeof(a)); a.Q = Q; a.Kt = Kt; a.Vt = Vt; a.O = att; a.B = 1; a.H = H; a.KV = KV; a.D = D; a.Dout = Dr;
       a.scale = 1.0f / sqrtf((float)Dr); a.causal = 1; a.vl_n = nb;
+      if (qip) { a.Q = nullptr; a.Qrows = qkv; a.q_ld = qkvw; a.rope_cos = group_long ? ctx->cos_l : ctx->cos_s; a.rope_sin = group_long ? ctx->sin_l : ctx->sin_s; }
       double fl = 0;
       for (int u = 0; u < nb; ++u) { a.vl_rows[u] = off[u]; a.vl_tables[u] = sqs[u]->d_block_table; a.S = lens[u] > a.S ? lens[u] : a.S;
         AttnArgs one = a; one.S = lens[u]; one.vl_n = 0; fl += gvl_attn_flops(one); }
diff --git a/grounded-video-llm_amd/csrc/gvl_model.hip b/grounded-video-llm_amd/csrc/gvl_model.hip
--- a/grounded-video-llm_amd/csrc/gvl_model.hip
+++ b/grounded-video-llm_amd/csrc/gvl_model.hip
@@ -541,6 +541,10 @@
 }
 
 int gvl_prefill_varlen(gvl_ctx* ctx, const int* seq_ids, int n_seqs, const uint16_t* const* embeds, const int* seq_lens, void* stream) {
+  return gvl_prefill_varlen_logits(ctx, seq_ids, n_seqs, embeds, seq_lens, nullptr, stream);
+}
+
+int gvl_prefill_varlen_logits(gvl_ctx* ctx, const int* seq_ids, int n_seqs, const uint16_t* const* embeds, const int* seq_lens, float* last_logits, void* stream) {
   REQUIRE_READY(ctx->has_llm, "gvl_prefill_varlen");
   if (!seq_ids || !embeds || !seq_lens || n_seqs <= 0 || n_seqs > gvl_ctx::kMaxSeqs) return fail(ctx, GVL_ERR_ARG, "gvl_prefill_varlen: bad arguments");
   for (int i = 0; i < n_seqs; ++i) {
@@ -565,6 +569,7 @@
     for (int b = 0; b < B; ++b) { sqs[b] = &ctx->seqs[seq_ids[i + b]]; es[b] = embeds[i + b]; }
     const int rc = llm_prefill(ctx, sqs, B, es, seq_lens + i, st);
     if (rc) return rc;
+    if (last_logits) HIPCHK(ctx, hipMemcpyAsync(last_logits + (size_t)i * ctx->cfg.vocab, ctx->d_logits, (size_t)B * ctx->cfg.vocab * 4, hipMemcpyDeviceToDevice, st));
     i += B;
   }
   return 0;
@@ -693,6 +698,7 @@
   else if (k == "varlen_attn") ctx->dbg.varlen_attn = value < 0 || value > 2 ? 1 : value;
   else if (k == "norm_fused") ctx->dbg.norm_fused = value != 0;
   else if (k == "last_layer_tail") ctx->dbg.last_layer_tail = value != 0;
+  else if (k == "prefill_q_in_place") ctx->dbg.prefill_q_in_place = value != 0;
   else if (k == "gemm_band") { if (value < 0 || value > 64) return fail(ctx, GVL_ERR_ARG, "gvl_debug_set: gemm_band must be 0 (automatic) .. 64"); gvl_gemm_set_band(value); }
   else if (k == "gemm_a4") { if (value < 0 || value > 3) return fail(ctx, GVL_ERR_ARG, "gvl_debug_set: gemm_a4 must be 0 .. 3"); gvl_gemm_set_a4(value); }
   else if (k == "gemm_narrow") gvl_gemm_set_narrow(value < 0 || value > 2 ? 1 : value);
diff --git a/grounded-video-llm_amd/engine.py b/grounded-video-llm_amd/engine.py
--- a/grounded-video-llm_amd/engine.py
+++ b/grounded-video-llm_amd/engine.py
@@ -317,13 +317,18 @@
                   "gvl_decode_greedy")
         return [int(buf[i]) for i in range(n.value)]
 
-    def prefill_batch(self, seqs: Sequence[int], embeds: Sequence[torch.Tensor]) -> None:
+    def prefill_batch(self, seqs: Sequence[int], embeds: Sequence[torch.Tensor], want_logits: bool = False) -> Optional[torch.Tensor]:
         es = [e.contiguous() for e in embeds]
         n = len(seqs)
         ids = (C.c_int * n)(*[int(s) for s in seqs])
         ptrs = (C.c_void_p * n)(*[e.data_ptr() for e in es])
         lens = (C.c_int * n)(*[int(e.shape[0]) for e in es])
-        self._chk(self.lib.gvl_prefill_varlen(self.ctx, ids, n, ptrs, lens, self.stream), "gvl_prefill_varlen")
+        if not want_logits:
+            self._chk(self.lib.gvl_prefill_varlen(self.ctx, ids, n, ptrs, lens, self.stream), "gvl_prefill_varlen")
+            return None
+        logits = torch.empty((n, self.geo.vocab), dtype=torch.float32, device=self.device)
+        self._chk(self.lib.gvl_prefill_varlen_logits(self.ctx, ids, n, ptrs, lens, _ptr(logits), self.stream), "gvl_prefill_varlen_logits")
+        return logits
 
     def decode_greedy_batch(self, seqs: Sequence[int], max_new: int, eos_id: Optional[int]) -> List[List[int]]:
         n = len(seqs)
diff --git a/grounded-video-llm_amd/lib.py b/grounded-video-llm_amd/lib.py
--- a/grounded-video-llm_amd/lib.py
+++ b/grounded-video-llm_amd/lib.py
@@ -77,6 +77,7 @@
     "gvl_seq_read": (C.c_int, [C.c_void_p, C.c_int, C.c_int, C.POINTER(C.c_int32), C.c_int, C.POINTER(C.c_int), C.c_void_p]),
     "gvl_forward_loss": (C.c_int, [C.c_void_p, C.c_int, C.c_void_p, C.c_int, C.POINTER(C.c_int64), C.POINTER(C.c_double), C.POINTER(C.c_int), C.c_void_p]),
     "gvl_prefill_varlen": (C.c_int, [C.c_void_p, C.POINTER(C.c_int), C.c_int, C.POINTER(C.c_void_p), C.POINTER(C.c_int), C.c_void_p]),
+    "gvl_prefill_varlen_logits": (C.c_int, [C.c_void_p, C.POINTER(C.c_int), C.c_int, C.POINTER(C.c_void_p), C.POINTER(C.c_int), C.c_void_p, C.c_void_p]),
     "gvl_decode_greedy_batch": (C.c_int, [C.c_void_p, C.POINTER(C.c_int), C.c_int, C.c_int, C.c_int, C.POINTER(C.c_int32), C.POINTER(C.c_int), C.c_void_p]),
     "gvl_decode_step_logits": (C.c_int, [C.c_void_p, C.c_int, C.c_int, C.c_void_p, C.c_void_p]),
     "gvl_decode_step_logits_batch": (C.c_int, [C.c_void_p, C.POINTER(C.c_int), C.c_int, C.POINTER(C.c_int32), C.c_void_p, C.c_void_p]),
diff --git a/include/gvl.h b/include/gvl.h
--- a/include/gvl.h
+++ b/include/gvl.h
@@ -108,6 +108,8 @@
                           void* stream);
 int gvl_prefill_varlen(gvl_ctx* ctx, const int* seq_ids, int n_seqs, const uint16_t* const* embeds,
                        const int* seq_lens, void* stream);
+int gvl_prefill_varlen_logits(gvl_ctx* ctx, const int* seq_ids, int n_seqs, const uint16_t* const* embeds,
+                              const int* seq_lens, float* last_logits, void* stream);
 int gvl_prefill_batch(gvl_ctx* ctx, const int* seq_ids, int n_seqs, const uint16_t* const* embeds, int seq_len,
                       void* stream);
 int gvl_decode_greedy_batch(gvl_ctx* ctx, const int* seq_ids, int n_seqs, int max_new, int eos_id,
```

Measured after the change: 11.70 clips/s (median of 6 runs). About the same (+0.3%).
